# av-savchenko/fast-image-recognition

Hardware: AMD Instinct MI355X
Metric: query-vectors/sec brute-force L2 top-1, 1Mx512 gallery (higher is better)
Workload: dtype f32; 1 GPU; 1000000x512 f32 gallery, batched L2 top-1 through the library's default dispatch (the metric's 1Mx512 size; configs[1]'s kernel is the exact-scan loop under `roofline`, --full); query_batch=131072

## Files before the change

### fast-image-recognition_amd/csrc/fir_gemm.hip

```cpp
#include <hip/hip_runtime.h>
#include <stdint.h>

#include <algorithm>
#include <cstdio>
#include <cstdlib>
#include <cstring>
#include <string>
#include <vector>

#include "../../include/fir_amd.h"
#include "fir_internal.h"
#include "fir_common.h"

namespace {

using fir::kKeyNone;

#ifndef FIR_I8_AUTO_MIN_QUERIES
#define FIR_I8_AUTO_MIN_QUERIES 2048
#endif
#ifndef FIR_GEMM_BLOCK
#define FIR_GEMM_BLOCK 512
#endif
constexpr int kGemmBlock = FIR_GEMM_BLOCK;
constexpr int kGemmMinBlocks = kGemmBlock <= 512 ? 2 : 1;
constexpr int kQT = 64;
constexpr int kSlab8 = 64;
constexpr int kSlab16 = 32;
constexpr int kPasses = 128;
constexpr int kCand = 8;
constexpr int kRerankGroup = 8;
constexpr size_t kRerankLdsMax = 144 * 1024;
constexpr int kListCap = 4096;
constexpr int kClassSampleRows = 16384;
constexpr int kMinSampleRows = 8192;

typedef float f32x16 __attribute__((ext_vector_type(16)));


__global__ void __launch_bounds__(256) k_gemm_pack_gallery(const float4* __restrict__ gal4, int64_t n, int dp4, int dq8,
                                                            float4* __restrict__ gm, float* __restrict__ gnorm) {
    const int64_t o = (int64_t)blockIdx.x * 256 + threadIdx.x;
    const int64_t rblocks = (n + 31) / 32;
    if (o >= rblocks * dq8 * 64) return;
    const int l = (int)(o & 63);
    const int64_t t = o >> 6;
    const int kq = (int)(t % dq8);
    const int64_t rb = t / dq8;
    const int64_t row = rb * 32 + (l & 31);
    const int h = l >> 5;
    float v[4] = {0.f, 0.f, 0.f, 0.f};
    if (row < n) {
        const int64_t tile = row >> 6;
        const int r = (int)(row & 63);
#pragma unroll
        for (int i = 0; i < 4; ++i) {
            const int k = 8 * kq + 2 * i + h;
            if (k < dp4 * 4) {
                const float4 g = gal4[(tile * dp4 + (k >> 2)) * 64 + r];
                v[i] = (k & 3) == 0 ? g.x : (k & 3) == 1 ? g.y : (k & 3) == 2 ? g.z : g.w;
            }
        }
    }
    gm[o] = make_float4(v[0], v[1], v[2], v[3]);
    if (kq == 0 && h == 0 && row < n) {
        const int64_t tile = row >> 6;
        const int r = (int)(row & 63);
        float s = 0.f;
        for (int c = 0; c < dp4; ++c) {
            const float4 g = gal4[(tile * dp4 + c) * 64 + r];
            s += g.x * g.x + g.y * g.y + g.z * g.z + g.w * g.w;
        }
        gnorm[row] = s;
    }
}

__global__ void __launch_bounds__(256) k_gemm_pack_queries(const float* q, int nq, int d, int dq8, float4* qm) {
    q += (size_t)blockIdx.y * kQT * d;
    nq -= (int)blockIdx.y * kQT;
    qm += (size_t)blockIdx.y * (kQT / 32) * dq8 * 64;
    const int o = blockIdx.x * 256 + threadIdx.x;
    if (o < (kQT / 32) * dq8 * 64) {
        const int l = o & 63;
        const int t = o >> 6;
        const int kq = t % dq8, jb = t / dq8;
        const int qi = jb * 32 + (l & 31), h = l >> 5;
        float v[4] = {0.f, 0.f, 0.f, 0.f};
        if (qi < nq) {
#pragma unroll
            for (int i = 0; i < 4; ++i) {
                const int k = 8 * kq + 2 * i + h;
                if (k < d) v[i] = q[(size_t)qi * d + k];
            }
        }
        qm[o] = make_float4(v[0], v[1], v[2], v[3]);
    }
}

__global__ void __launch_bounds__(64) k_gemm_qnorm(const float* __restrict__ q, int nq, int d, float* __restrict__ qnorm) {
    const int qi = blockIdx.x;
    float s = 0.f;
    if (qi < nq)
        for (int k = threadIdx.x; k < d; k += 64) s += q[(size_t)qi * d + k] * q[(size_t)qi * d + k];
#pragma unroll
    for (int off = 32; off >= 1; off >>= 1) s += __shfl_xor(s, off, 64);
    if (threadIdx.x == 0) qnorm[qi] = s;
}

template <int MODE>
__global__ void __launch_bounds__(kGemmBlock, kGemmMinBlocks) k_gemm_proxy(const float4* __restrict__ gm, const float* __restrict__ gnorm,
                                                               const float4* qm, int64_t n, int64_t row_begin,
                                                               int64_t row_end, int dq8, const float* tau, unsigned long long* lists, int* counts, float* sample,
                                                               int sample_rows) {
    extern __shared__ __attribute__((aligned(16))) float4 lq[];
    __shared__ float tau_s[kQT];
    {
        const size_t ps = blockIdx.y;
        qm += ps * (kQT / 32) * dq8 * 64;
        tau += ps * kQT;
        lists += ps * kQT * kListCap;
        counts += ps * kQT;
        sample += ps * kQT * sample_rows;
    }
    const int lane = threadIdx.x & 63, wave = threadIdx.x >> 6;
    const int wpb = blockDim.x >> 6;
    const int sq8 = dq8 < kSlab8 ? dq8 : kSlab8;
    const int nslab = (dq8 + sq8 - 1) / sq8;
    if (MODE == 1 && threadIdx.x < kQT) tau_s[threadIdx.x] = tau[threadIdx.x];
    const int64_t rb_begin = row_begin / 32, rb_end = (row_end + 31) / 32;
    const int64_t nrg = (rb_end - rb_begin + wpb - 1) / wpb;
    bool staged = false;
    for (int64_t rg = blockIdx.x; rg < nrg; rg += gridDim.x) {
        const int64_t rb = rb_begin + rg * wpb + wave;
        const bool active = rb < rb_end;
        f32x16 acc0 = {0.f}, acc1 = {0.f};
        for (int sl = 0; sl < nslab; ++sl) {
            const int k0 = sl * sq8;
            const int kw = dq8 - k0 < sq8 ? dq8 - k0 : sq8;
            if (nslab > 1 || !staged) {
                __syncthreads();
                for (int i = threadIdx.x; i < 2 * kw * 64; i += blockDim.x) {
                    const int jb = i / (kw * 64), r = i - jb * kw * 64;
                    lq[(size_t)jb * sq8 * 64 + r] = qm[((size_t)jb * dq8 + k0) * 64 + r];
                }
                __syncthreads();
                staged = true;
            }
            if (!active) continue;
            const float4* a = gm + ((size_t)rb * dq8 + k0) * 64 + lane;
            const int last = kw - 1;
            float4 a0 = a[0], a1 = a[(size_t)(1 < last ? 1 : last) * 64], a2 = a[(size_t)(2 < last ? 2 : last) * 64],
                   a3 = a[(size_t)(3 < last ? 3 : last) * 64], a4 = a[(size_t)(4 < last ? 4 : last) * 64],
                   a5 = a[(size_t)(5 < last ? 5 : last) * 64], a6 = a[(size_t)(6 < last ? 6 : last) * 64],
                   a7 = a[(size_t)(7 < last ? 7 : last) * 64];
            float4 b0 = lq[lane], b1 = lq[(size_t)sq8 * 64 + lane];
#define FIR_GEMM_STEP(AV, KQ)                                                              \
            {                                                                              \
                const int kn = (KQ) + 1 < kw ? (KQ) + 1 : (KQ);                            \
                const float4 n0 = lq[(size_t)kn * 64 + lane];                              \
                const float4 n1 = lq[(size_t)(sq8 + kn) * 64 + lane];                      \
                __builtin_amdgcn_sched_barrier(0);     \
                acc0 = __builtin_amdgcn_mfma_f32_32x32x2f32(AV.x, b0.x, acc0, 0, 0, 0);    \
                acc1 = __builtin_amdgcn_mfma_f32_32x32x2f32(AV.x, b1.x, acc1, 0, 0, 0);    \
                acc0 = __builtin_amdgcn_mfma_f32_32x32x2f32(AV.y, b0.y, acc0, 0, 0, 0);    \
                acc1 = __builtin_amdgcn_mfma_f32_32x32x2f32(AV.y, b1.y, acc1, 0, 0, 0);    \
                acc0 = __builtin_amdgcn_mfma_f32_32x32x2f32(AV.z, b0.z, acc0, 0, 0, 0);    \
                acc1 = __builtin_amdgcn_mfma_f32_32x32x2f32(AV.z, b1.z, acc1, 0, 0, 0);    \
                acc0 = __builtin_amdgcn_mfma_f32_32x32x2f32(AV.w, b0.w, acc0, 0, 0, 0);    \
                acc1 = __builtin_amdgcn_mfma_f32_32x32x2f32(AV.w, b1.w, acc1, 0, 0, 0);    \
                b0 = n0;                                                                   \
                b1 = n1;                                                                   \
            }
            for (int kq = 0; kq < kw; kq += 8) {
#define FIR_GEMM_NEXT(AV, OFF) AV = a[(size_t)(kq + (OFF) + 8 < kw ? kq + (OFF) + 8 : last) * 64];
                FIR_GEMM_STEP(a0, kq)
                FIR_GEMM_NEXT(a0, 0)
                FIR_GEMM_STEP(a1, kq + 1)
                FIR_GEMM_NEXT(a1, 1)
                FIR_GEMM_STEP(a2, kq + 2)
                FIR_GEMM_NEXT(a2, 2)
                FIR_GEMM_STEP(a3, kq + 3)
                FIR_GEMM_NEXT(a3, 3)
                if (kq + 4 < kw) {
                    FIR_GEMM_STEP(a4, kq + 4)
                    FIR_GEMM_NEXT(a4, 4)
                    FIR_GEMM_STEP(a5, kq + 5)
                    FIR_GEMM_NEXT(a5, 5)
                    FIR_GEMM_STEP(a6, kq + 6)
                    FIR_GEMM_NEXT(a6, 6)
                    FIR_GEMM_STEP(a7, kq + 7)
                    FIR_GEMM_NEXT(a7, 7)
                }
#undef FIR_GEMM_NEXT
            }
#undef FIR_GEMM_STEP
        }
        if (!active) continue;
        const int64_t nrow = rb * 32 + (lane & 31);
        const float gn_lane = nrow < n ? gnorm[nrow] : 0.0f;
#pragma unroll
        for (int jb = 0; jb < 2; ++jb) {
            const int q = jb * 32 + (lane & 31);
#pragma unroll
            for (int reg = 0; reg < 16; ++reg) {
                const int roff = (reg & 3) + 8 * (reg >> 2) + 4 * (lane >> 5);
                const int64_t row = rb * 32 + roff;
                const float gn = __shfl(gn_lane, roff, 64);
                if (row >= n || row < row_begin || row >= row_end) continue;
                const float dot = jb == 0 ? acc0[reg] : acc1[reg];
                const float p = gn - 2.0f * dot;
                if (MODE == 0) {
                    if (row < sample_rows) sample[(size_t)q * sample_rows + row] = p;
                } else if (p < tau_s[q]) {
                    const int slot = atomicAdd(&counts[q], 1);
                    if (slot < kListCap) lists[(size_t)q * kListCap + slot] = fir::key_pack(p, (uint32_t)row);
                }
            }
        }
    }
}

typedef __bf16 bf16x8 __attribute__((ext_vector_type(8)));

__device__ __forceinline__ void split_bf16(float x, unsigned short& hi, unsigned short& lo) {
    const __bf16 h = (__bf16)x;
    const __bf16 l = (__bf16)(x - (float)h);
    __builtin_memcpy(&hi, &h, 2);
    __builtin_memcpy(&lo, &l, 2);
}

__global__ void __launch_bounds__(256) k_gemm_pack_gallery_bf16(const float4* __restrict__ gal4, int64_t n, int dp4, int dk16,
                                                                 uint4* __restrict__ gb) {
    const int64_t o = (int64_t)blockIdx.x * 256 + threadIdx.x;
    const int64_t rblocks = (n + 31) / 32;
    if (o >= rblocks * dk16 * 64) return;
    const int l = (int)(o & 63);
    const int64_t t = o >> 6;
    const int kb = (int)(t % dk16);
    const int64_t rb = t / dk16;
    const int64_t row = rb * 32 + (l & 31);
    const int h = l >> 5;
    unsigned short hi[8], lo[8];
#pragma unroll
    for (int j = 0; j < 8; ++j) {
        const int k = 16 * kb + 8 * h + j;
        float x = 0.f;
        if (row < n && k < dp4 * 4) {
            const float4 g = gal4[((row >> 6) * dp4 + (k >> 2)) * 64 + (row & 63)];
            x = (k & 3) == 0 ? g.x : (k & 3) == 1 ? g.y : (k & 3) == 2 ? g.z : g.w;
        }
        split_bf16(x, hi[j], lo[j]);
    }
    uint4 vh, vl;
    __builtin_memcpy(&vh, hi, 16);
    __builtin_memcpy(&vl, lo, 16);
    gb[(size_t)(t * 2) * 64 + l] = vh;
    gb[(size_t)(t * 2 + 1) * 64 + l] = vl;
}

__global__ void __launch_bounds__(256) k_gemm_pack_queries_bf16(const float* q, int nq, int d, int dk16, uint4* qbf) {
    q += (size_t)blockIdx.y * kQT * d;
    nq -= (int)blockIdx.y * kQT;
    qbf += (size_t)blockIdx.y * (kQT / 32) * dk16 * 128;
    const int o = blockIdx.x * 256 + threadIdx.x;
    if (o >= (kQT / 32) * dk16 * 64) return;
    const int l = o & 63;
    const int t = o >> 6;
    const int kb = t % dk16, jb = t / dk16;
    const int qi = jb * 32 + (l & 31), h = l >> 5;
    unsigned short hi[8], lo[8];
#pragma unroll
    for (int j = 0; j < 8; ++j) {
        const int k = 16 * kb + 8 * h + j;
        const float x = (qi < nq && k < d) ? q[(size_t)qi * d + k] : 0.f;
        split_bf16(x, hi[j], lo[j]);
    }
    uint4 vh, vl;
    __builtin_memcpy(&vh, hi, 16);
    __builtin_memcpy(&vl, lo, 16);
    qbf[(size_t)(t * 2) * 64 + l] = vh;
    qbf[(size_t)(t * 2 + 1) * 64 + l] = vl;
}

__device__ __forceinline__ uint4 ld_nt(const uint4* p) {
    typedef unsigned v4u __attribute__((ext_vector_type(4)));
    const v4u v = __builtin_nontemporal_load((const v4u*)p);
    return make_uint4(v.x, v.y, v.z, v.w);
}
__device__ __forceinline__ bf16x8 as_bf16x8(const uint4 v) {
    bf16x8 r;
    __builtin_memcpy(&r, &v, 16);
    return r;
}

template <int MODE>
__global__ void __launch_bounds__(kGemmBlock, kGemmMinBlocks) k_gemm_proxy_bf16(const uint4* __restrict__ gb, const float* __restrict__ gnorm,
                                                                    const uint4* qbf, int64_t n, int64_t row_begin,
                                                                    int64_t row_end, int dk16, const float* tau, unsigned long long* lists, int* counts, float* sample,
                                                                    int sample_rows) {
    extern __shared__ __attribute__((aligned(16))) uint4 lqb[];
    __shared__ float tau_s[kQT];
    {
        const size_t ps = blockIdx.y;
        qbf += ps * (kQT / 32) * dk16 * 128;
        tau += ps * kQT;
        lists += ps * kQT * kListCap;
        counts += ps * kQT;
        sample += ps * kQT * sample_rows;
    }
    const int lane = threadIdx.x & 63, wave = threadIdx.x >> 6;
    const int wpb = blockDim.x >> 6;
    const int sk16 = MODE == 0 ? dk16 : (dk16 < kSlab16 ? dk16 : kSlab16);
    const int nslab = (dk16 + sk16 - 1) / sk16;
    const uint4* bsrc = MODE == 0 ? qbf : lqb;
    if (MODE == 1 && threadIdx.x < kQT) tau_s[threadIdx.x] = tau[threadIdx.x];
    const int64_t rb_begin = row_begin / 32, rb_end = (row_end + 31) / 32;
    const int64_t nrg = (rb_end - rb_begin + wpb - 1) / wpb;
    bool staged = MODE == 0;
    for (int64_t rg = blockIdx.x; rg < nrg; rg += gridDim.x) {
        const int64_t rb = rb_begin + rg * wpb + wave;
        const bool active = rb < rb_end;
        f32x16 acc0 = {0.f}, acc1 = {0.f};
        for (int sl = 0; sl < nslab; ++sl) {
            const int k0 = sl * sk16;
            const int kw = dk16 - k0 < sk16 ? dk16 - k0 : sk16;
            if (MODE == 1 && (nslab > 1 || !staged)) {
                __syncthreads();
                for (int i = threadIdx.x; i < 2 * kw * 128; i += blockDim.x) {
                    const int jb = i / (kw * 128), r = i - jb * kw * 128;
                    lqb[(size_t)jb * sk16 * 128 + r] = qbf[((size_t)jb * dk16 + k0) * 128 + r];
                }
                __syncthreads();
                staged = true;
            }
            if (!active) continue;
            const uint4* a = gb + ((size_t)rb * dk16 + k0) * 128 + lane;
            const int last = kw - 1;
#define FIR_BF_LD(IDX) ld_nt(a + (size_t)((IDX) < last ? (IDX) : last) * 128)
#define FIR_BF_LDL(IDX) ld_nt(a + (size_t)((IDX) < last ? (IDX) : last) * 128 + 64)
            uint4 h0 = FIR_BF_LD(0), l0 = FIR_BF_LDL(0), h1 = FIR_BF_LD(1), l1 = FIR_BF_LDL(1), h2 = FIR_BF_LD(2), l2 = FIR_BF_LDL(2),
                  h3 = FIR_BF_LD(3), l3 = FIR_BF_LDL(3), h4 = FIR_BF_LD(4), l4 = FIR_BF_LDL(4), h5 = FIR_BF_LD(5), l5 = FIR_BF_LDL(5),
                  h6 = FIR_BF_LD(6), l6 = FIR_BF_LDL(6), h7 = FIR_BF_LD(7), l7 = FIR_BF_LDL(7);
            const uint4* bq0 = bsrc + (size_t)(MODE == 0 ? k0 : 0) * 128 + lane;
            const uint4* bq1 = bq0 + (size_t)sk16 * 128;
            uint4 b0h = bq0[0], b0l = bq0[64], b1h = bq1[0], b1l = bq1[64];
#define FIR_BF_STEP(AH, AL, KB)                                                                                  \
            {                                                                                                    \
                const int kn = (KB) + 1 < kw ? (KB) + 1 : (KB);                                                  \
                const uint4 n0h = bq0[(size_t)kn * 128], n0l = bq0[(size_t)kn * 128 + 64];                       \
                const uint4 n1h = bq1[(size_t)kn * 128], n1l = bq1[(size_t)kn * 128 + 64];                       \
                __builtin_amdgcn_sched_barrier(0);                                                               \
                const bf16x8 ah = as_bf16x8(AH), al = as_bf16x8(AL);                                             \
                acc0 = __builtin_amdgcn_mfma_f32_32x32x16_bf16(ah, as_bf16x8(b0h), acc0, 0, 0, 0);               \
                acc1 = __builtin_amdgcn_mfma_f32_32x32x16_bf16(ah, as_bf16x8(b1h), acc1, 0, 0, 0);               \
                acc0 = __builtin_amdgcn_mfma_f32_32x32x16_bf16(ah, as_bf16x8(b0l), acc0, 0, 0, 0);               \
                acc1 = __builtin_amdgcn_mfma_f32_32x32x16_bf16(ah, as_bf16x8(b1l), acc1, 0, 0, 0);               \
                acc0 = __builtin_amdgcn_mfma_f32_32x32x16_bf16(al, as_bf16x8(b0h), acc0, 0, 0, 0);               \
                acc1 = __builtin_amdgcn_mfma_f32_32x32x16_bf16(al, as_bf16x8(b1h), acc1, 0, 0, 0);               \
                b0h = n0h; b0l = n0l; b1h = n1h; b1l = n1l;                                                      \
            }
#define FIR_BF_NEXT(AH, AL, OFF)                \
            {                                   \
                AH = FIR_BF_LD(kb + (OFF) + 8); \
                AL = FIR_BF_LDL(kb + (OFF) + 8);\
            }
            for (int kb = 0; kb < kw; kb += 8) {
                FIR_BF_STEP(h0, l0, kb)
                FIR_BF_NEXT(h0, l0, 0)
                FIR_BF_STEP(h1, l1, kb + 1)
                FIR_BF_NEXT(h1, l1, 1)
                FIR_BF_STEP(h2, l2, kb + 2)
                FIR_BF_NEXT(h2, l2, 2)
                FIR_BF_STEP(h3, l3, kb + 3)
                FIR_BF_NEXT(h3, l3, 3)
                if (kb + 4 < kw) {
                    FIR_BF_STEP(h4, l4, kb + 4)
                    FIR_BF_NEXT(h4, l4, 4)
                    FIR_BF_STEP(h5, l5, kb + 5)
                    FIR_BF_NEXT(h5, l5, 5)
                    FIR_BF_STEP(h6, l6, kb + 6)
                    FIR_BF_NEXT(h6, l6, 6)
                    FIR_BF_STEP(h7, l7, kb + 7)
                    FIR_BF_NEXT(h7, l7, 7)
                }
            }
#undef FIR_BF_NEXT
#undef FIR_BF_STEP
#undef FIR_BF_LD
#undef FIR_BF_LDL
        }
        if (!active) continue;
        const int64_t nrow = rb * 32 + (lane & 31);
        const float gn_lane = nrow < n ? gnorm[nrow] : 0.0f;
#pragma unroll
        for (int jb = 0; jb < 2; ++jb) {
            const int q = jb * 32 + (lane & 31);
#pragma unroll
            for (int reg = 0; reg < 16; ++reg) {
                const int roff = (reg & 3) + 8 * (reg >> 2) + 4 * (lane >> 5);
                const int64_t row = rb * 32 + roff;
                const float gn = __shfl(gn_lane, roff, 64);
                if (row >= n || row < row_begin || row >= row_end) continue;
                const float dot = jb == 0 ? acc0[reg] : acc1[reg];
                const float p = gn - 2.0f * dot;
                if (MODE == 0) {
                    if (row < sample_rows) sample[(size_t)q * sample_rows + row] = p;
                } else if (p < tau_s[q]) {
                    const int slot = atomicAdd(&counts[q], 1);
                    if (slot < kListCap) lists[(size_t)q * kListCap + slot] = fir::key_pack(p, (uint32_t)row);
                }
            }
        }
    }
}

constexpr int kSlabW = 16;
constexpr int kUnitW = kSlabW / 2;
constexpr int kWideLds = 4 * kSlabW * 128 * (int)sizeof(uint4);
__global__ void __launch_bounds__(kGemmBlock, 1) k_gemm_proxy_bf16_wide(const uint4* __restrict__ gb, const float* __restrict__ gnorm,
                                                                         const uint4* qbf, int64_t n, int dk16, const float* tau,
                                                                         unsigned long long* lists, int* counts) {
    extern __shared__ __attribute__((aligned(16))) uint4 lqb[];
    __shared__ float tau_s[2 * kQT];
    {
        const size_t pr = blockIdx.y;
        qbf += pr * 4 * dk16 * 128;
        tau += pr * 2 * kQT;
        lists += pr * 2 * kQT * kListCap;
        counts += pr * 2 * kQT;
    }
    const int lane = threadIdx.x & 63, wave = threadIdx.x >> 6;
    const int wpb = blockDim.x >> 6;
    if (threadIdx.x < 2 * kQT) tau_s[threadIdx.x] = tau[threadIdx.x];
    const int64_t rb_end = (n + 31) / 32;
    const int64_t nrg = (rb_end + wpb - 1) / wpb;
    const int units = dk16 / kUnitW;
    int64_t rg = blockIdx.x;
    if (rg >= nrg) return;
#define FIR_W_BLOCK(RG) (gb + (size_t)(((RG) * wpb + wave) < rb_end ? ((RG) * wpb + wave) : rb_end - 1) * dk16 * 128 + lane)
    const uint4* a_cur = FIR_W_BLOCK(rg);
    uint4 ch[kUnitW], cl[kUnitW], nh[kUnitW], nl[kUnitW];
#pragma unroll
    for (int u = 0; u < kUnitW; ++u) {
        ch[u] = ld_nt(a_cur + (size_t)u * 128);
        cl[u] = ld_nt(a_cur + (size_t)u * 128 + 64);
    }
    for (; rg < nrg; rg += gridDim.x) {
        const int64_t rb = rg * wpb + wave;
        const bool active = rb < rb_end;
        const int64_t rgn = rg + gridDim.x;
        const uint4* a_nxt = FIR_W_BLOCK(rgn < nrg ? rgn : rg);
        f32x16 acc0 = {0.f}, acc1 = {0.f}, acc2 = {0.f}, acc3 = {0.f};
        for (int h = 0; h < units; ++h) {
            const uint4* src = h + 1 < units ? a_cur + (size_t)(h + 1) * kUnitW * 128 : a_nxt;
#pragma unroll
            for (int u = 0; u < kUnitW; ++u) {
                nh[u] = ld_nt(src + (size_t)u * 128);
                nl[u] = ld_nt(src + (size_t)u * 128 + 64);
            }
            if ((h & 1) == 0) {
                const int k0 = h * kUnitW;
                const int kw = dk16 - k0 < kSlabW ? dk16 - k0 : kSlabW;
                __syncthreads();
                for (int i = threadIdx.x; i < 4 * kw * 128; i += blockDim.x) {
                    const int jb = i / (kw * 128), r = i - jb * kw * 128;
                    lqb[(size_t)jb * kSlabW * 128 + r] = qbf[((size_t)jb * dk16 + k0) * 128 + r];
                }
                __syncthreads();
            }
            const uint4* bq = lqb + lane + (size_t)(h & 1) * kUnitW * 128;
#pragma unroll
            for (int u = 0; u < kUnitW; ++u) {
                const uint4* bu = bq + (size_t)u * 128;
                const bf16x8 ah = as_bf16x8(ch[u]), al = as_bf16x8(cl[u]);
#pragma unroll
                for (int jb = 0; jb < 4; ++jb) {
                    const bf16x8 bh = as_bf16x8(bu[(size_t)jb * kSlabW * 128]), bl = as_bf16x8(bu[(size_t)jb * kSlabW * 128 + 64]);
                    f32x16& acc = jb == 0 ? acc0 : jb == 1 ? acc1 : jb == 2 ? acc2 : acc3;
                    acc = __builtin_amdgcn_mfma_f32_32x32x16_bf16(ah, bh, acc, 0, 0, 0);
                    acc = __builtin_amdgcn_mfma_f32_32x32x16_bf16(ah, bl, acc, 0, 0, 0);
                    acc = __builtin_amdgcn_mfma_f32_32x32x16_bf16(al, bh, acc, 0, 0, 0);
                }
            }
#pragma unroll
            for (int u = 0; u < kUnitW; ++u) { ch[u] = nh[u]; cl[u] = nl[u]; }
        }
        a_cur = a_nxt;
        if (!active) continue;
        const int64_t nrow = rb * 32 + (lane & 31);
        const float gn_lane = nrow < n ? gnorm[nrow] : 0.0f;
#pragma unroll
        for (int jb = 0; jb < 4; ++jb) {
            const int q = jb * 32 + (lane & 31);
#pragma unroll
            for (int reg = 0; reg < 16; ++reg) {
                const int roff = (reg & 3) + 8 * (reg >> 2) + 4 * (lane >> 5);
                const int64_t row = rb * 32 + roff;
                const float gn = __shfl(gn_lane, roff, 64);
                if (row >= n) continue;
                const float dot = jb == 0 ? acc0[reg] : jb == 1 ? acc1[reg] : jb == 2 ? acc2[reg] : acc3[reg];
                const float p = gn - 2.0f * dot;
                if (p < tau_s[q]) {
                    const int slot = atomicAdd(&counts[q], 1);
                    if (slot < kListCap) lists[(size_t)q * kListCap + slot] = fir::key_pack(p, (uint32_t)row);
                }
            }
        }
    }
#undef FIR_W_BLOCK
}

typedef _Float16 f16x8 __attribute__((ext_vector_type(8)));
__device__ __forceinline__ f16x8 as_f16x8(const uint4 v) {
    f16x8 r;
    __builtin_memcpy(&r, &v, 16);
    return r;
}
constexpr int kSlabH = 32;
constexpr int kHalfLds = 4 * kSlabH * 64 * (int)sizeof(uint4);
constexpr int kRing = 8;

#include "fir_gemm_rerank.h"

__global__ void __launch_bounds__(256) k_gemm_absmax(const float4* __restrict__ gal4, int64_t count4, float* __restrict__ out) {
    float m = 0.f;
    for (int64_t i = (int64_t)blockIdx.x * 256 + threadIdx.x; i < count4; i += (int64_t)gridDim.x * 256) {
        const float4 g = gal4[i];
        const float a = fmaxf(fmaxf(fabsf(g.x), fabsf(g.y)), fmaxf(fabsf(g.z), fabsf(g.w)));
        const bool bad = !(g.x == g.x && g.y == g.y && g.z == g.z && g.w == g.w);
        m = fmaxf(m, bad ? __builtin_huge_valf() : a);
    }
#pragma unroll
    for (int off = 32; off >= 1; off >>= 1) m = fmaxf(m, __shfl_xor(m, off, 64));
    if ((threadIdx.x & 63) == 0) atomicMax((unsigned int*)out, __float_as_uint(m));
}

__global__ void __launch_bounds__(64) k_gemm_qprep_f16(const float* __restrict__ q, int nq, int d, int gallery_exp, float* __restrict__ qnorm,
                                                        float* __restrict__ qmul, float* __restrict__ qinv, int qstride, int* __restrict__ counts = nullptr,
                                                        float* __restrict__ win = nullptr, unsigned int* __restrict__ t_bits = nullptr,
                                                        const float* __restrict__ gnorm_max_p = nullptr, float e_rel = 0.f, int nslot = 0,
                                                        unsigned int* __restrict__ smin_init = nullptr, int* __restrict__ fb_state = nullptr) {
    const int qi = blockIdx.x;
    if (threadIdx.x == 0) {
        if (smin_init) smin_init[qi] = 0xFF800000u;
        if (fb_state && qi == 0) { fb_state[0] = 0; fb_state[1] = 0; }
    }
    float s = 0.f, m = 0.f;
    bool bad = false;
    if (qi < nq)
        for (int k = threadIdx.x; k < d; k += 64) {
            const float x = q[(size_t)qi * qstride + k];
            s += x * x;
            m = fmaxf(m, fabsf(x));
            bad = bad || !(fabsf(x) < __builtin_huge_valf());
        }
#pragma unroll
    for (int off = 32; off >= 1; off >>= 1) {
        s += __shfl_xor(s, off, 64);
        m = fmaxf(m, __shfl_xor(m, off, 64));
    }
    bad = __any(bad);
    if (threadIdx.x == 0) {
        int ex = 0;
        if (m > 0.f) (void)frexpf(m, &ex);
        int sh = m > 0.f ? 14 - ex : 0;
        if (sh < -100 || sh > 100 || gallery_exp < -100 || gallery_exp > 100) bad = true;
        const float qn = (bad && qi < nq) ? __builtin_nanf("") : s;
        qnorm[qi] = qn;
        qmul[qi] = bad ? 0.f : ldexpf(1.0f, sh);
        qinv[qi] = qi >= nq ? 0.f : bad ? __builtin_nanf("") : ldexpf(1.0f, -sh - gallery_exp);
        if (counts) counts[qi] = 0;
        if (win) {
            const unsigned int start = qi >= nq ? 0u : 0x7F800000u;
            if (qi >= nq) win[qi] = 0.f;
            else {
                win[qi] = nudge_up_(rounding_window_(e_rel, qn, gnorm_max_p[0]));
            }
            if (nslot > 0) { for (int sl = 0; sl < 8; ++sl) atomicExch(&t_bits[(size_t)qi * 8 + sl], start); }
            else atomicExch(&t_bits[qi], start);
        }
    }
}

#include "fir_gemm_f16x.h"

__global__ void __launch_bounds__(256) k_gemm_tau(const float* __restrict__ sample, int sample_rows, float* __restrict__ tau,
                                                   int nq_valid, const float* __restrict__ qnorm, const float* __restrict__ gnorm_max_p, float e_rel,
                                                   int kth_window = 0) {
    __shared__ unsigned long long red[4];
    const int q = blockIdx.x;
    if (q >= nq_valid) {
        if (threadIdx.x == 0) tau[q] = -__builtin_huge_valf();
        return;
    }
    const float* s = sample + (size_t)q * sample_rows;
    unsigned long long best[kCand];
#pragma unroll
    for (int i = 0; i < kCand; ++i) best[i] = kKeyNone;
    for (int i = threadIdx.x; i < sample_rows; i += 256) {
        unsigned long long v = fir::key_pack(s[i], (uint32_t)i);
        if (v < best[kCand - 1]) {
#pragma unroll
            for (int j = 0; j < kCand; ++j) {
                const bool sw = v < best[j];
                const unsigned long long t = best[j];
                best[j] = sw ? v : t;
                v = sw ? t : v;
            }
        }
    }
    unsigned long long m = kKeyNone, smallest = kKeyNone;
    for (int r = 0; r < kCand; ++r) {
        unsigned long long c = fir::wave_min_u64(best[0]);
        __syncthreads();
        if ((threadIdx.x & 63) == 0) red[threadIdx.x >> 6] = c;
        __syncthreads();
        m = red[0];
        for (int i = 1; i < 4; ++i) m = red[i] < m ? red[i] : m;
        if (r == 0) smallest = m;
        if (m == kKeyNone) break;
        if (best[0] == m) {
#pragma unroll
            for (int j = 0; j + 1 < kCand; ++j) best[j] = best[j + 1];
            best[kCand - 1] = kKeyNone;
        }
    }
    if (threadIdx.x == 0) {
        float t = __builtin_huge_valf();
        if (m != kKeyNone) {
            float v = fir::f32_from_orderable((uint32_t)(m >> 32));
            const float v1 = fir::f32_from_orderable((uint32_t)(smallest >> 32));
            const float window = rounding_window_(e_rel, qnorm[q], gnorm_max_p[0]);
            v = kth_window ? v + window : fmaxf(v, v1 + window);
            t = nudge_up_(v);
        }
        tau[q] = t;
    }
}

#include "fir_gemm_fb.h"
#include "fir_gemm_i8.h"

template <int KMAX>
__global__ void __launch_bounds__(64) k_gemm_rerank(const unsigned long long* __restrict__ lists, const int* __restrict__ counts,
                                                     const float* __restrict__ tau, const float4* __restrict__ gal4,
                                                     const float* __restrict__ queries, const float* __restrict__ qnorm,
                                                     const float* __restrict__ gnorm_max_p, int64_t n, int d, int dp4, int64_t row_offset,
                                                     float e_rel, int ngroup, int k_arg, unsigned long long* __restrict__ out_key,
                                                     int* __restrict__ ok, int qstride, const float4* __restrict__ rowmajor, const RerankFb fb,
                                                     const float* __restrict__ eabs = nullptr) {
    const int k = KMAX == 1 ? 1 : k_arg;
    const int q = blockIdx.x, lane = threadIdx.x;
    int qo = q;
    if (fb.qmap) {
        if (q >= fb.state[0] - fb.live_off) return;
        qo = fb.qmap[q];
    }
    const int cnt = counts[q];
    const int have = cnt < kListCap ? cnt : kListCap;
    const unsigned long long* L = lists + (size_t)q * kListCap;
    int found;
    const unsigned long long kth = list_kth_smallest_(L, have, k, lane, found);
    const float qn = qnorm[q], gmax = gnorm_max_p[0];
    const float pk = found == k ? fir::f32_from_orderable((uint32_t)(kth >> 32)) : __builtin_huge_valf();
    const RerankWindow w = eabs ? rerank_window_(e_rel, qn, gmax, d, pk, eabs[q]) : rerank_window_(e_rel, qn, gmax, d, pk);
    extern __shared__ __attribute__((aligned(16))) float4 crow[];
    const RerankLds lds = rerank_lds_f32_(crow, ngroup, dp4, d, queries + (size_t)qo * qstride, lane);
    unsigned long long best[KMAX];
#pragma unroll
    for (int i = 0; i < KMAX; ++i) best[i] = kKeyNone;
    const RerankWalk walk = rerank_walk_(L, have, w.win, lane, [&](int base, unsigned long long v, bool, unsigned long long mask) {
        rerank_gather_f32_(mask, v, base, lane, ngroup, lds, gal4, rowmajor, dp4, d, [&](int, unsigned long long cv, float dist) {
            if (dist < fir::kNotFound) {
                const int64_t row = (int64_t)(uint32_t)(cv & 0xFFFFFFFFull);
                unsigned long long key = fir::key_pack(dist, (uint32_t)(row + row_offset));
#pragma unroll
                for (int j = 0; j < KMAX; ++j) {
                    const bool sw = key < best[j];
                    const unsigned long long t = best[j];
                    best[j] = sw ? key : t;
                    key = sw ? t : key;
                }
            }
        });
    });
    unsigned long long kth_exact = kKeyNone;
    for (int r = 0; r < k; ++r) {
        const unsigned long long m = fir::wave_min_u64(best[0]);
        if (lane == 0) out_key[(size_t)qo * k + r] = m;
        kth_exact = m;
        if (m != kKeyNone && best[0] == m) {
#pragma unroll
            for (int j = 0; j + 1 < KMAX; ++j) best[j] = best[j + 1];
            best[KMAX - 1] = kKeyNone;
        }
    }
    if (lane == 0) {
        const float t = tau[q];
        const bool certified = rerank_certified_<float>(cnt, t, walk.p_out, qn, d, w.E, kth_exact != kKeyNone,
                                                        fir::f32_from_orderable((uint32_t)(kth_exact >> 32)), n, walk.reranked);
        ok[qo] = certified ? 1 : 0;
        if (!certified && fb.list && !fb.qmap) rerank_hand_over_(fb, q, cnt, t, pk, qn, gmax, e_rel, eabs);
    }
}

__global__ void __launch_bounds__(256) k_gemm_select(const float* __restrict__ proxies, int64_t n, const float* __restrict__ tau,
                                                      unsigned long long* __restrict__ lists, int* __restrict__ counts) {
    const int q = blockIdx.y;
    const float tq = tau[q];
    const float* p = proxies + (size_t)q * n;
    for (int64_t row = (int64_t)blockIdx.x * 256 + threadIdx.x; row < n; row += (int64_t)gridDim.x * 256) {
        const float v = p[row];
        if (v < tq) {
            const int slot = atomicAdd(&counts[q], 1);
            if (slot < kListCap) lists[(size_t)q * kListCap + slot] = fir::key_pack(v, (uint32_t)row);
        }
    }
}

__global__ void __launch_bounds__(256) k_gemm_tau_class(float* __restrict__ tau, int nq_total, int nq_valid, int d, const float* __restrict__ qnorm,
                                                         const float* __restrict__ gnorm_max_p, float e_rel) {
    const int q = blockIdx.x * 256 + threadIdx.x;
    if (q >= nq_total) return;
    if (q >= nq_valid) { tau[q] = -__builtin_huge_valf(); return; }
    const float ds = tau[q];
    float t = __builtin_huge_valf();
    if (ds < fir::kNotFound) {
        const float v = (ds * (float)d - qnorm[q]) + rounding_window_(e_rel, qnorm[q], gnorm_max_p[0]);
        t = nudge_up_(v);
    }
    tau[q] = t;
}

__global__ void __launch_bounds__(64) k_gemm_rerank_classes(unsigned long long* lists, const int* __restrict__ counts, const float* __restrict__ tau,
                                                             const float4* __restrict__ gal4, const float* __restrict__ queries,
                                                             const float* __restrict__ qnorm, const float* __restrict__ gnorm_max_p,
                                                             const int32_t* __restrict__ cls, int num_classes, int64_t n, int d, int dp4,
                                                             int64_t row_offset, float e_rel, int ngroup, int k, unsigned long long* __restrict__ out_key,
                                                             int32_t* __restrict__ out_cls, int* __restrict__ ok, int qstride,
                                                             const float4* __restrict__ rowmajor) {
    __shared__ int32_t taken[32];
    const int q = blockIdx.x, lane = threadIdx.x;
    const int cnt = counts[q];
    if (cnt > kListCap) {
        if (lane == 0) ok[q] = 0;
        return;
    }
    const int have = cnt;
    unsigned long long* L = lists + (size_t)q * kListCap;
    auto pick = [&](int r, unsigned long long prev, int64_t roff, int32_t& c_out) -> unsigned long long {
        unsigned long long cand = kKeyNone;
        int32_t cc = -1;
        for (int i = lane; i < have; i += 64) {
            const unsigned long long v = L[i];
            if (v >= cand || (r > 0 && v <= prev)) continue;
            const int32_t c = cls[(int64_t)(uint32_t)(v & 0xFFFFFFFFull) - roff];
            bool skip = (uint32_t)c >= (uint32_t)num_classes;
            for (int j = 0; j < r; ++j) skip = skip || taken[j] == c;
            if (!skip) { cand = v; cc = c; }
        }
        const unsigned long long m = fir::wave_min_u64(cand);
        const unsigned long long who = __ballot(m != kKeyNone && cand == m);
        c_out = who ? __shfl(cc, __ffsll((long long)who) - 1, 64) : -1;
        return m;
    };
    unsigned long long prev = 0;
    int found = 0;
    for (int r = 0; r < k; ++r) {
        int32_t c;
        const unsigned long long m = pick(r, prev, 0, c);
        if (m == kKeyNone) break;
        if (lane == 0) taken[r] = c;
        __syncthreads();
        prev = m;
        ++found;
    }
    const float qn = qnorm[q], gmax = gnorm_max_p[0];
    const float pk = found == k ? fir::f32_from_orderable((uint32_t)(prev >> 32)) : __builtin_huge_valf();
    const RerankWindow w = rerank_window_(e_rel, qn, gmax, d, pk);
    extern __shared__ __attribute__((aligned(16))) float4 crow[];
    const RerankLds lds = rerank_lds_f32_(crow, ngroup, dp4, d, queries + (size_t)q * qstride, lane);
    const RerankWalk walk = rerank_walk_(L, have, w.win, lane, [&](int base, unsigned long long v, bool in, unsigned long long mask) {
        if (base + lane < have && !in) L[base + lane] = kKeyNone;
        rerank_gather_f32_(mask, v, base, lane, ngroup, lds, gal4, rowmajor, dp4, d, [&](int i, unsigned long long cv, float dist) {
            const int64_t row = (int64_t)(uint32_t)(cv & 0xFFFFFFFFull);
            const bool counted = (uint32_t)cls[row] < (uint32_t)num_classes && dist < fir::kNotFound;
            L[i] = counted ? fir::key_pack(dist, (uint32_t)(row + row_offset)) : kKeyNone;
        });
    });
    __threadfence_block();
    __syncthreads();
    unsigned long long kth_exact = kKeyNone;
    prev = 0;
    int r = 0;
    for (; r < k; ++r) {
        int32_t c;
        const unsigned long long m = pick(r, prev, row_offset, c);
        if (m == kKeyNone) break;
        if (lane == 0) {
            taken[r] = c;
            if (out_key) out_key[(size_t)q * k + r] = m;
            if (out_cls) out_cls[(size_t)q * k + r] = c;
        }
        __syncthreads();
        prev = m;
        if (r == k - 1) kth_exact = m;
    }
    for (int i = r + lane; i < k; i += 64) {
        if (out_key) out_key[(size_t)q * k + i] = kKeyNone;
        if (out_cls) out_cls[(size_t)q * k + i] = -1;
    }
    if (lane == 0)
        ok[q] = rerank_certified_<float>(cnt, tau[q], walk.p_out, qn, d, w.E, kth_exact != kKeyNone, fir::f32_from_orderable((uint32_t)(kth_exact >> 32)), n,
                                         walk.reranked) ? 1 : 0;
}

__global__ void k_gemm_fb_count(int* __restrict__ state, int count) {
    unsigned long long* tot = (unsigned long long*)(state + 4);
    tot[0] += (unsigned long long)count;
    tot[1] += (unsigned long long)count;
}

__global__ void __launch_bounds__(256) k_gemm_untile(const float4* __restrict__ gal4, int64_t n, int dp4, int d4, float4* __restrict__ rowmajor) {
    __shared__ float4 t[32][65];
    const int64_t tile = blockIdx.x;
    const int c0 = blockIdx.y * 32;
    for (int i = threadIdx.x; i < 32 * 64; i += 256) {
        const int c = i >> 6, r = i & 63;
        if (c0 + c < d4) t[c][r] = gal4[((size_t)tile * dp4 + c0 + c) * 64 + r];
    }
    __syncthreads();
    for (int i = threadIdx.x; i < 64 * 32; i += 256) {
        const int r = i >> 5, c = i & 31;
        const int64_t row = tile * 64 + r;
        if (row < n && c0 + c < d4) rowmajor[(size_t)row * d4 + c0 + c] = t[c][r];
    }
}

__global__ void __launch_bounds__(256) k_gemm_row_norms(const float4* __restrict__ gal4, int64_t n, int dp4, float* __restrict__ gnorm, int d4) {
    const int64_t row = (int64_t)blockIdx.x * 256 + threadIdx.x;
    if (row >= n) return;
    float s = 0.f;
    for (int c = 0; c < d4; ++c) {
        const float4 g = gal4[((row >> 6) * dp4 + c) * 64 + (row & 63)];
        s += g.x * g.x + g.y * g.y + g.z * g.z + g.w * g.w;
    }
    gnorm[row] = s;
}

__global__ void k_gemm_max(const float* __restrict__ gnorm, int64_t n, float* __restrict__ out) {
    __shared__ float red[4];
    float m = 0.f;
    for (int64_t i = threadIdx.x; i < n; i += 256) m = fmaxf(m, gnorm[i]);
#pragma unroll
    for (int off = 32; off >= 1; off >>= 1) m = fmaxf(m, __shfl_xor(m, off, 64));
    if ((threadIdx.x & 63) == 0) red[threadIdx.x >> 6] = m;
    __syncthreads();
    if (threadIdx.x == 0) out[0] = fmaxf(fmaxf(red[0], red[1]), fmaxf(red[2], red[3]));
}

__global__ void __launch_bounds__(256) k_gemm_adapt_init(float* __restrict__ win, unsigned int* __restrict__ t_bits, int nq_total, int nq_valid,
                                                          const float* __restrict__ qnorm, const float* __restrict__ gnorm_max_p, float e_rel) {
    const int q = blockIdx.x * 256 + threadIdx.x;
    if (q >= nq_total) return;
    if (q >= nq_valid) { win[q] = 0.f; t_bits[q] = 0u; return; }
    win[q] = nudge_up_(rounding_window_(e_rel, qnorm[q], gnorm_max_p[0]));
    t_bits[q] = 0x7F800000u;
}
__global__ void __launch_bounds__(256) k_gemm_adapt_final(unsigned int* __restrict__ t_bits, const float* __restrict__ qnorm, float* __restrict__ tau,
                                                           int nq_total, int nq_valid, int nslot = 0) {
    const int q = blockIdx.x * 256 + threadIdx.x;
    if (q >= nq_total) return;
    unsigned int t;
    if (nslot > 0) {
        unsigned int v[8];
        for (int sl = 0; sl < 8; ++sl) v[sl] = atomicMin(&t_bits[(size_t)q * 8 + sl], 0xFFFFFFFFu);
        t = 0xFFFFFFFFu;
        for (int i = 0; i < 8; ++i) {
            int rank = 0;
            for (int j = 0; j < 8; ++j) rank += (v[j] < v[i] || (v[j] == v[i] && j < i)) ? 1 : 0;
            if (rank == nslot - 1) t = v[i];
        }
    } else t = atomicMin(&t_bits[q], 0xFFFFFFFFu);
    tau[q] = q < nq_valid ? __uint_as_float(t) - qnorm[q] : -__builtin_huge_valf();
}

}

struct fir_gemm {
    fir_gallery* g = nullptr;
    fir_gallery_view v;
    const float4* gal4 = nullptr;
    int dp4 = 0, dq8 = 0;
    int feat = 0;
    int precision = 0;
    uint4* gh = nullptr;
    float* proxies = nullptr;
    int proxies_nq = 0;
    int lists_cap = 0;
    float4* rowmajor = nullptr;
    int gallery_exp = 0;
    float* qmul[2] = {nullptr, nullptr};
    float* qinv[2] = {nullptr, nullptr};
    int dk16 = 0;
    float4* gm = nullptr;
    uint4* gb = nullptr;
    uint4* qbf[2] = {nullptr, nullptr};
    float* gnorm = nullptr;
    float* gmax = nullptr;
    float4* qm[2] = {nullptr, nullptr};
    float* qnorm[2] = {nullptr, nullptr};
    float* tau[2] = {nullptr, nullptr};
    float* sample = nullptr;
    unsigned long long* lists[2] = {nullptr, nullptr};
    int* counts[2] = {nullptr, nullptr};
    hipStream_t side = nullptr;
    hipEvent_t main_done[2] = {nullptr, nullptr}, rerank_done[2] = {nullptr, nullptr}, prep_done[2] = {nullptr, nullptr};
    hipEvent_t queries_ready = nullptr;
    hipStream_t copy = nullptr;
    hipEvent_t copy_done[2] = {nullptr, nullptr};
    int* ok = nullptr; size_t ok_cap = 0;
    int sample_rows = 0;
    int* fb_state = nullptr;
    int* fb_list = nullptr;
    int* fb_list2 = nullptr;
    float* fb_tau2 = nullptr;
    float* sc_qnorm = nullptr; float* sc_qmul = nullptr; float* sc_qinv = nullptr; float* sc_tau = nullptr;
    int* sc_counts = nullptr;
    unsigned long long* sc_lists = nullptr;
    uint4* sc_qbf = nullptr;
    size_t fb_lds = 0;
    int fb_grid = 0;
    int64_t passes = 0;
    int rerank_group = kRerankGroup;
    bool wide = true;
    unsigned int* smin[2] = {nullptr, nullptr};
    int rt_sample_rows = 0;
    bool f64 = false;
    const double2* gal2 = nullptr; int dp2 = 0;
    int adaptive = 1;
    int class_sample_div = 64;
    int adaptive_topk = 1;
    float* awin[2] = {nullptr, nullptr};
    unsigned int* aT[2] = {nullptr, nullptr};
    float erel_scale = 1.0f;
    int dbg_block = kGemmBlock;
    int dbg_skip = 0;
    int adapt_dbg = 0;
    bool debug_counts = false;
    hipEvent_t phase_ev[4] = {nullptr, nullptr, nullptr, nullptr};
    std::string dump_phases;
    int last_kind = 0;
    int last_b = 0, last_nq = 0;
    int last_sc_rounds = 0;
    bool last_i8 = false;
    int i8_mode = 0;
    bool i8_built = false, i8_off = false;
    const char* i8_off_why = "";
    std::string i8_note;
    int dk8 = 0;
    uint4* g8 = nullptr;
    float* i8_mu = nullptr;
    float* i8_gnorm = nullptr;
    float* i8_par = nullptr;
    float* i8_eabs[2] = {nullptr, nullptr};
    float* sc_eabs = nullptr;
    float i8_R = 0.f, i8_G = 0.f;
    int* i8_pin = nullptr;
    hipEvent_t i8_ev = nullptr;
    bool i8_pending = false;
    int i8_pending_qb = 0;
};

static void gemm_read_knobs_(fir_gemm* m) {
    if (const char* w = fir_knob_("FIR_GEMM_ADAPTIVE")) m->adaptive = std::atoi(w);
    if (const char* w = fir_knob_("FIR_GEMM_ADAPTIVE_TOPK")) m->adaptive_topk = std::atoi(w) != 0;
    if (const char* w = fir_knob_("FIR_GEMM_CLASS_SAMPLE_DIV")) m->class_sample_div = std::max(1, std::atoi(w));
#ifdef FIR_AUDIT
    if (const char* w = fir_knob_("FIR_GEMM_DBG_SKIP")) m->dbg_skip = std::atoi(w) & 1023;
    if (const char* w = fir_knob_("FIR_GEMM_DBG_BLOCK")) m->dbg_block = std::atoi(w) == 256 ? 256 : kGemmBlock;
    if (const char* w = fir_knob_("FIR_GEMM_EREL_SCALE")) m->erel_scale = (float)std::atof(w);
    if (const char* w = fir_knob_("FIR_GEMM_ADAPT_DBG")) m->adapt_dbg = (std::atoi(w) & 3) << 2;
    if (fir_knob_("FIR_GEMM_DEBUG_COUNTS")) m->debug_counts = true;
    if (const char* w = fir_knob_("FIR_GEMM_DUMP_PHASES")) m->dump_phases = w;
#endif
}

struct RerankSlot {
    const unsigned long long* lists;
    const int* counts;
    const float* tau;
    const float* qnorm;
    const float* eabs = nullptr;
    const float* gmax = nullptr;
};
static size_t gemm_rerank_lds_(const fir_gemm* m) { return (size_t)(m->rerank_group + 1) * (m->dp4 + 1) * sizeof(float4); }
static void gemm_launch_rerank_(fir_gemm* m, hipStream_t st, int nq, const RerankSlot& s, const float* d_queries, float e_rel, int k, uint64_t* out_key, int* ok,
                                const RerankFb& fb) {
    hipLaunchKernelGGL(k == 1 ? k_gemm_rerank<1> : k_gemm_rerank<kTopKMax>, dim3(nq), dim3(64), gemm_rerank_lds_(m), st, s.lists, s.counts, s.tau, m->gal4, d_queries,
                       s.qnorm, s.gmax ? s.gmax : (const float*)m->gmax, m->v.n, m->feat, m->dp4, m->v.row_offset, e_rel, m->rerank_group, k, (unsigned long long*)out_key,
                       ok, m->v.d, (const float4*)m->rowmajor, fb, s.eabs);
}

constexpr int kShareMax = 16, kShareStreamed = 8;
static bool gemm_streamed_(const fir_gemm* m) { return m->dk16 > kSlabH; }
static int gemm_odd_(const fir_gemm* m) { return m->dk16 == kRing ? 2 : (m->dk16 / kRing) & 1; }
static int gemm_odd8_(const fir_gemm* m) { return m->dk8 == kRing ? 2 : (m->dk8 / kRing) & 1; }
static int launch_pairs_(int left, int cap) {
    int P = 1;
    while (P * 2 <= left && P * 2 <= cap) P *= 2;
    return P;
}

typedef void (*fir_x_fn)(const uint4*, const float*, const uint4*, const float*, int64_t, int64_t, int64_t, int, const float*, unsigned long long*, int*, float*,
                         int, int, int, int, unsigned int*, int);
struct fir_x_entry {
    int mode, streamed, odd, njb;
    fir_x_fn fn;
    const char* name;
};
#define FIR_X(M, S, O) {M, S, O, 8, k_gemm_proxy_f16x<M, S, O>, "fir::k_gemm_proxy_f16x<" #M ", " #S ", " #O ">"}
#define FIR_X_FEW(S, J) {3, S, 0, J, k_gemm_proxy_f16x<3, S, 0, 0, J>, "fir::k_gemm_proxy_f16x<3, " #S ", 0, 0, " #J ">"}
static const fir_x_entry kXTable[] = {
    FIR_X(1, 0, 0), FIR_X(1, 0, 1), FIR_X(1, 1, 0), FIR_X(1, 1, 1), FIR_X(2, 0, 0), FIR_X(2, 0, 1), FIR_X(2, 1, 0), FIR_X(2, 1, 1),
    FIR_X(3, 0, 0), FIR_X(3, 0, 1), FIR_X(3, 1, 0), FIR_X(3, 1, 1), FIR_X(4, 0, 0), FIR_X(4, 0, 1), FIR_X(4, 1, 0), FIR_X(4, 1, 1),
    FIR_X_FEW(0, 1), FIR_X_FEW(1, 1), FIR_X_FEW(0, 2), FIR_X_FEW(1, 2),
    FIR_X(1, 0, 2), FIR_X(2, 0, 2), FIR_X(3, 0, 2), FIR_X(4, 0, 2),
};
#undef FIR_X
#undef FIR_X_FEW
static const fir_x_entry* lookup_x(int mode, bool streamed, int odd, int njb) {
    for (const fir_x_entry& e : kXTable)
        if (e.mode == mode && e.streamed == (int)streamed && e.odd == odd && e.njb == njb) return &e;
    return nullptr;
}
static const fir_x_entry& find_x(int mode, bool streamed, int odd, int njb = 8) {
    if (!(mode == 3 && !odd && (njb == 1 || njb == 2))) njb = 8;
    if (const fir_x_entry* e = lookup_x(mode, streamed, odd, njb)) return *e;
    if (const fir_x_entry* e = lookup_x(2, streamed, odd, 8)) return *e;
    return *lookup_x(2, false, 0, 8);
}
static fir_x_fn pick_x(int mode, bool streamed, int odd, int dbg = 0, int njb = 8) {
#ifdef FIR_AUDIT
    if (dbg && mode == 3 && !streamed && !odd) {
        switch (dbg & 1023) {
            case 1: return k_gemm_proxy_f16x<3, 0, 0, 1>;
            case 2: return k_gemm_proxy_f16x<3, 0, 0, 2>;
            case 3: return k_gemm_proxy_f16x<3, 0, 0, 3>;
            case 5: return k_gemm_proxy_f16x<3, 0, 0, 5>;
            case 7: return k_gemm_proxy_f16x<3, 0, 0, 7>;
            case 512: return k_gemm_proxy_f16x<3, 0, 0, 512>;
            case 256: return k_gemm_proxy_f16x<3, 0, 0, 256>;
            case 128: return k_gemm_proxy_f16x<3, 0, 0, 128>;
            case 384: return k_gemm_proxy_f16x<3, 0, 0, 384>;
            case 64: return k_gemm_proxy_f16x<3, 0, 0, 64>;
            case 33: return k_gemm_proxy_f16x<3, 0, 0, 33>;
            case 37: return k_gemm_proxy_f16x<3, 0, 0, 37>;
            case 35: return k_gemm_proxy_f16x<3, 0, 0, 35>;
            case 16: return k_gemm_proxy_f16x<3, 0, 0, 16>;
            case 8: return k_gemm_proxy_f16x<3, 0, 0, 8>;
            default: break;
        }
    }
#endif
    return find_x(mode, streamed, odd, dbg ? 8 : njb).fn;
}
struct fir_x8_entry {
    int mode, odd;
    fir_x_fn fn;
    const char* name;
};
#define FIR_X8(M, O) {M, O, k_gemm_proxy_f16x<M, 0, O, 0, 8, 1>, "fir::k_gemm_proxy_i8x<" #M ", " #O ">"}
static const fir_x8_entry kX8Table[] = {FIR_X8(3, 0), FIR_X8(3, 1), FIR_X8(3, 2), FIR_X8(1, 0), FIR_X8(1, 1), FIR_X8(1, 2)};
#undef FIR_X8
static const fir_x8_entry& find_x8(int mode, int odd) {
    for (const fir_x8_entry& e : kX8Table)
        if (e.mode == mode && e.odd == odd) return e;
    return kX8Table[0];
}
static hipError_t gemm_x_lds_attr_() {
    for (const fir_x_entry& e : kXTable) {
        const hipError_t err = hipFuncSetAttribute((const void*)e.fn, hipFuncAttributeMaxDynamicSharedMemorySize, kHalfLds);
        if (err != hipSuccess) return err;
    }
    for (const fir_x8_entry& e : kX8Table) {
        const hipError_t err = hipFuncSetAttribute((const void*)e.fn, hipFuncAttributeMaxDynamicSharedMemorySize, kHalfLds);
        if (err != hipSuccess) return err;
    }
    return hipSuccess;
}

static void gemm_free_i8_(fir_gemm* m) {
    (void)hipFree(m->g8); (void)hipFree(m->i8_mu); (void)hipFree(m->i8_gnorm); (void)hipFree(m->i8_par); (void)hipFree(m->i8_eabs[0]); (void)hipFree(m->i8_eabs[1]);
    (void)hipFree(m->sc_eabs);
    if (m->i8_pin) (void)hipHostFree(m->i8_pin);
    if (m->i8_ev) (void)hipEventDestroy(m->i8_ev);
    m->g8 = nullptr; m->i8_mu = m->i8_gnorm = m->i8_par = m->i8_eabs[0] = m->i8_eabs[1] = m->sc_eabs = nullptr;
    m->i8_pin = nullptr; m->i8_ev = nullptr;
    m->i8_built = false;
}

extern "C" {

int fir_gemm_create(fir_gallery* g, fir_gemm** out) { return fir_gemm_create_range(g, FIR_GEMM_F16, 0, out); }

int fir_gemm_create_ex(fir_gallery* g, int32_t precision, fir_gemm** out) { return fir_gemm_create_range(g, precision, 0, out); }

int fir_gemm_create_range(fir_gallery* g, int32_t precision, int32_t end_pos, fir_gemm** out) { return fir_gemm_create_range_ex_(g, precision, end_pos, -1, out); }

void fir_gemm_memory_bytes_(const fir_gemm* m, int64_t* fragments, int64_t* rowmajor, int64_t* scratch) {
    const int64_t rblocks = (std::max<int64_t>(m->v.n, 1) + 31) / 32, np = std::max<int64_t>(m->v.n, 1);
    const int64_t fr = m->gh ? rblocks * m->dk16 * 1024 : m->gb ? rblocks * m->dk16 * 2048 : m->gm ? rblocks * m->dq8 * 1024 : 0;
    const int64_t rm = m->rowmajor ? m->v.n * (int64_t)((m->feat + 3) / 4) * 16 : 0;
    int64_t sc = np * 4 + 16;
    sc += 2 * ((int64_t)m->lists_cap * kListCap * 8 + (int64_t)m->lists_cap * 4);
    sc += 2 * (m->precision == FIR_GEMM_F32 ? (int64_t)kPasses * (kQT / 32) * m->dq8 * 1024
                                            : (int64_t)kPasses * (kQT / 32) * m->dk16 * (m->precision == FIR_GEMM_BF16_SPLIT ? 2048 : 1024));
    sc += 2 * (int64_t)kPasses * kQT * 4 * 4 + 2 * (int64_t)kRtSubsets * kPasses * kQT * 4;
    sc += (int64_t)m->ok_cap * 16 + 32;
    if (m->sc_lists) sc += (int64_t)kScQueries * kListCap * 8 + (int64_t)4 * m->dk16 * 1024 + (int64_t)kScQueries * 20;
    if (m->proxies) sc += (int64_t)m->proxies_nq * np * 4;
    int64_t fr8 = 0;
    if (m->g8) {
        fr8 = rblocks * m->dk8 * 1024;
        sc += np * 4 + (int64_t)((m->feat + 3) / 4) * 16 + 32 + 2 * (int64_t)kPasses * kQT * 4 + (int64_t)kScQueries * 4;
    }
    if (fragments) *fragments = fr + fr8;
    if (rowmajor) *rowmajor = rm;
    if (scratch) *scratch = sc;
}

int fir_gemm_create_range_ex_(fir_gallery* g, int32_t precision, int32_t end_pos, int32_t rowmajor_mode, fir_gemm** out) {
    if (!g || !out) return fir_fail_(FIR_ERR_ARG, "NULL argument");
    if (precision != FIR_GEMM_F32 && precision != FIR_GEMM_BF16_SPLIT && precision != FIR_GEMM_F16)
        return fir_fail_(FIR_ERR_ARG, "bad precision %d", precision);
    *out = nullptr;
    fir_gemm* m = new (std::nothrow) fir_gemm();
    if (!m) return fir_fail_(FIR_ERR_NOMEM, "host allocation failed");
    m->g = g;
    const void* gp = nullptr;
    if (fir_gallery_view_(g, &m->v) != FIR_OK || fir_gallery_tiled_(g, &gp, &m->dp4) != FIR_OK) { delete m; return fir_fail_(FIR_ERR_ARG, "bad gallery"); }
    m->gal4 = (const float4*)gp;
    m->precision = precision;
    if (precision == FIR_GEMM_F16 && !(m->v.cus >= 8 && (m->v.cus & 7) == 0)) {
        const int cus = m->v.cus;
        delete m;
        return fir_fail_(FIR_ERR_ARG, "the 16-row kernels want CUs in eights (%d)", cus);
    }
    m->feat = end_pos > 0 && end_pos < m->v.d ? end_pos : m->v.d;
    if (end_pos < 0 || end_pos > m->v.d || (m->feat != m->v.d && (m->feat % 16 != 0 || precision != FIR_GEMM_F16))) {
        const int dd = m->v.d;
        delete m;
        return fir_fail_(FIR_ERR_ARG, "feature prefix [0,%d) of %d: multiples of 16 inside the row, fp16 form only", end_pos, dd);
    }
    if (const char* w = fir_knob_("FIR_GEMM_WIDE")) m->wide = std::atoi(w) != 0;
    m->dq8 = (m->feat + 31) / 32 * 4;
    m->dk16 = (m->feat + 127) / 128 * 8;
    if (precision == FIR_GEMM_F16) m->dk16 = (m->feat + 16 * kRing - 1) / (16 * kRing) * kRing;
    hipError_t e = hipSetDevice(m->v.device);
    const int64_t rblocks = (std::max<int64_t>(m->v.n, 1) + 31) / 32;
    const int64_t np = std::max<int64_t>(m->v.n, 1);
    if (e == hipSuccess && precision == FIR_GEMM_F32) e = hipMalloc((void**)&m->gm, (size_t)rblocks * m->dq8 * 64 * sizeof(float4));
    if (e == hipSuccess && precision == FIR_GEMM_BF16_SPLIT) e = hipMalloc((void**)&m->gb, (size_t)rblocks * m->dk16 * 128 * sizeof(uint4));
    if (e == hipSuccess && precision == FIR_GEMM_F16) e = hipMalloc((void**)&m->gh, (size_t)rblocks * m->dk16 * 64 * sizeof(uint4));
    if (e == hipSuccess) e = hipMalloc((void**)&m->gnorm, (size_t)np * sizeof(float));
    if (e == hipSuccess) e = hipMalloc((void**)&m->gmax, 16);
    for (int b = 0; b < 2; ++b) {
        if (e == hipSuccess && precision == FIR_GEMM_F32) e = hipMalloc((void**)&m->qm[b], (size_t)kPasses * (kQT / 32) * m->dq8 * 64 * sizeof(float4));
        if (e == hipSuccess && precision != FIR_GEMM_F32)
            e = hipMalloc((void**)&m->qbf[b], (size_t)kPasses * (kQT / 32) * m->dk16 * (precision == FIR_GEMM_BF16_SPLIT ? 128 : 64) * sizeof(uint4));
        if (e == hipSuccess) e = hipMalloc((void**)&m->qnorm[b], kPasses * kQT * sizeof(float));
        if (e == hipSuccess) e = hipMalloc((void**)&m->qmul[b], kPasses * kQT * sizeof(float));
        if (e == hipSuccess) e = hipMalloc((void**)&m->qinv[b], kPasses * kQT * sizeof(float));
        if (e == hipSuccess) e = hipMalloc((void**)&m->smin[b], (size_t)kRtSubsets * kPasses * kQT * sizeof(unsigned int));
        if (e == hipSuccess) e = hipMalloc((void**)&m->tau[b], kPasses * kQT * sizeof(float));
        if (e == hipSuccess) e = hipMalloc((void**)&m->awin[b], kPasses * kQT * sizeof(float));
        if (e == hipSuccess) e = hipMalloc((void**)&m->aT[b], (size_t)8 * kPasses * kQT * sizeof(unsigned int));
        if (e == hipSuccess) e = hipEventCreateWithFlags(&m->main_done[b], hipEventDisableTiming);
        if (e == hipSuccess) e = hipEventCreateWithFlags(&m->rerank_done[b], hipEventDisableTiming);
        if (e == hipSuccess) e = hipEventCreateWithFlags(&m->prep_done[b], hipEventDisableTiming);
    }
    if (e == hipSuccess) e = hipEventCreateWithFlags(&m->queries_ready, hipEventDisableTiming);
    if (e == hipSuccess) e = hipStreamCreateWithFlags(&m->side, hipStreamNonBlocking);
    if (e == hipSuccess) e = hipStreamCreateWithFlags(&m->copy, hipStreamNonBlocking);
    for (int b = 0; b < 2 && e == hipSuccess; ++b) e = hipEventCreateWithFlags(&m->copy_done[b], hipEventDisableTiming);
    m->sample_rows = (int)std::min<int64_t>(np, std::max<int64_t>(kMinSampleRows, np / 64));
    m->rt_sample_rows = (int)std::min<int64_t>(np, std::max<int64_t>(kMinSampleRows, np / 32));
    if (const char* w = fir_knob_("FIR_GEMM_SAMPLE_DIV"))
        m->rt_sample_rows = (int)std::min<int64_t>(np, std::max<int64_t>(kMinSampleRows, np / std::max(1, std::atoi(w))));
    if (e == hipSuccess) e = hipMalloc((void**)&m->fb_state, kFbStateWords * sizeof(int));
    if (e == hipSuccess) e = hipMemset(m->fb_state, 0, kFbStateWords * sizeof(int));
    if (e == hipSuccess) e = hipMalloc((void**)&m->sc_qnorm, kScQueries * sizeof(float));
    if (e == hipSuccess) e = hipMalloc((void**)&m->sc_qmul, kScQueries * sizeof(float));
    if (e == hipSuccess) e = hipMalloc((void**)&m->sc_qinv, kScQueries * sizeof(float));
    if (e == hipSuccess) e = hipMalloc((void**)&m->sc_tau, kScQueries * sizeof(float));
    if (e == hipSuccess) e = hipMalloc((void**)&m->sc_counts, kScQueries * sizeof(int));
    if (e == hipSuccess && precision == FIR_GEMM_F16) e = hipMalloc((void**)&m->sc_lists, (size_t)kScQueries * kListCap * sizeof(unsigned long long));
    if (e == hipSuccess && precision == FIR_GEMM_F16) e = hipMalloc((void**)&m->sc_qbf, (size_t)4 * m->dk16 * 64 * sizeof(uint4));
    {
        m->fb_lds = (size_t)m->dp4 * 4 * 8 * sizeof(float);
        if (m->fb_lds > kRerankLdsMax) {
            const int dd = m->v.d;
            fir_gemm_destroy(m);
            return fir_fail_(FIR_ERR_ARG, "rows of %d features are too long for the matrix-core path's exact fallback", dd);
        }
        if (e == hipSuccess && m->fb_lds > 48 * 1024)
            e = hipFuncSetAttribute((const void*)k_gemm_exact_fb, hipFuncAttributeMaxDynamicSharedMemorySize, (int)kRerankLdsMax);
        const int per_cu = (int)std::max<size_t>(1, std::min<size_t>(4, (size_t)(160 * 1024) / std::max<size_t>(m->fb_lds, 1)));
        m->fb_grid = std::max(1, m->v.cus) * per_cu;
    }
    const int lds_bytes = precision == FIR_GEMM_F32 ? (kQT / 32) * std::min(m->dq8, kSlab8) * 64 * (int)sizeof(float4)
                                                    : (kQT / 32) * std::min(m->dk16, kSlab16) * 128 * (int)sizeof(uint4);
    if (e == hipSuccess) e = hipFuncSetAttribute((const void*)k_gemm_proxy<0>, hipFuncAttributeMaxDynamicSharedMemorySize, lds_bytes);
    if (e == hipSuccess) e = hipFuncSetAttribute((const void*)k_gemm_proxy<1>, hipFuncAttributeMaxDynamicSharedMemorySize, lds_bytes);
    if (e == hipSuccess) e = hipFuncSetAttribute((const void*)k_gemm_proxy_bf16<0>, hipFuncAttributeMaxDynamicSharedMemorySize, lds_bytes);
    if (e == hipSuccess) e = hipFuncSetAttribute((const void*)k_gemm_proxy_bf16<1>, hipFuncAttributeMaxDynamicSharedMemorySize, lds_bytes);
    if (e == hipSuccess) e = hipFuncSetAttribute((const void*)k_gemm_proxy_bf16_wide, hipFuncAttributeMaxDynamicSharedMemorySize, kWideLds);
    {
        const size_t row_bytes = (size_t)(m->dp4 + 1) * sizeof(float4);
        m->rerank_group = (int)std::min<size_t>(kRerankGroup, kRerankLdsMax / row_bytes > 1 ? kRerankLdsMax / row_bytes - 1 : 0);
        if (m->rerank_group < 1) { delete m; return fir_fail_(FIR_ERR_ARG, "rows of %d features are too long for the matrix-core path's re-rank", m->v.d); }
        if (gemm_rerank_lds_(m) > 48 * 1024)
            for (const void* fn : {(const void*)k_gemm_rerank<1>, (const void*)k_gemm_rerank<kTopKMax>, (const void*)k_gemm_rerank_classes})
                if (e == hipSuccess) e = hipFuncSetAttribute(fn, hipFuncAttributeMaxDynamicSharedMemorySize, (int)kRerankLdsMax);
    }
    if (e == hipSuccess && precision == FIR_GEMM_F16) e = gemm_x_lds_attr_();
    gemm_read_knobs_(m);
    if (e == hipSuccess && m->v.n > 0) {
        if (precision == FIR_GEMM_BF16_SPLIT) {
            const int64_t totalb = rblocks * m->dk16 * 64;
            hipLaunchKernelGGL(k_gemm_pack_gallery_bf16, dim3((unsigned)((totalb + 255) / 256)), dim3(256), 0, m->v.stream, m->gal4, m->v.n, m->dp4,
                               m->dk16, m->gb);
            hipLaunchKernelGGL(k_gemm_row_norms, dim3((unsigned)((m->v.n + 255) / 256)), dim3(256), 0, m->v.stream, m->gal4, m->v.n, m->dp4, m->gnorm, (m->feat + 3) / 4);
        }
        if (precision == FIR_GEMM_F16) {
            float h_max = 0.f;
            e = hipMemsetAsync(m->gmax, 0, 16, m->v.stream);
            const int64_t count4 = (int64_t)((m->v.n + 63) / 64) * m->dp4 * 64;
            hipLaunchKernelGGL(k_gemm_absmax, dim3((unsigned)std::min<int64_t>((count4 + 255) / 256, 4096)), dim3(256), 0, m->v.stream, m->gal4, count4, m->gmax);
            if (e == hipSuccess) e = hipMemcpyAsync(&h_max, m->gmax, sizeof(float), hipMemcpyDeviceToHost, m->v.stream);
            if (e == hipSuccess) e = hipStreamSynchronize(m->v.stream);
            int ex = 0;
            if (h_max > 0.f && h_max < __builtin_huge_valf()) { (void)std::frexp(h_max, &ex); m->gallery_exp = 14 - ex; }
            else m->gallery_exp = h_max > 0.f ? 1000 : 0;
            const float scale = (m->gallery_exp >= -100 && m->gallery_exp <= 100) ? std::ldexp(1.0f, m->gallery_exp) : 0.f;
            const int64_t totalh = rblocks * m->dk16 * 64;
            hipLaunchKernelGGL(k_gemm_pack_gallery_f16x, dim3((unsigned)((totalh + 255) / 256)), dim3(256), 0, m->v.stream, m->gal4, m->v.n, m->dp4,
                               m->dk16, scale, m->gh, m->feat == m->v.d ? m->dp4 * 4 : m->feat);
            hipLaunchKernelGGL(k_gemm_row_norms, dim3((unsigned)((m->v.n + 255) / 256)), dim3(256), 0, m->v.stream, m->gal4, m->v.n, m->dp4, m->gnorm, (m->feat + 3) / 4);
        }
        const int64_t total = precision == FIR_GEMM_F32 ? rblocks * m->dq8 * 64 : 0;
        if (total > 0)
        hipLaunchKernelGGL(k_gemm_pack_gallery, dim3((unsigned)((total + 255) / 256)), dim3(256), 0, m->v.stream, m->gal4, m->v.n, m->dp4, m->dq8,
                           m->gm, m->gnorm);
        hipLaunchKernelGGL(k_gemm_max, dim3(1), dim3(256), 0, m->v.stream, m->gnorm, m->v.n, m->gmax);
        {
            const int d4 = (m->feat + 3) / 4;
            const size_t want = (size_t)m->v.n * d4 * sizeof(float4);
            size_t free_b = 0, total_b = 0;
            int mode = rowmajor_mode;
            if (const char* w = fir_knob_("FIR_GEMM_ROWMAJOR")) { if (mode < 0) mode = std::atoi(w); }
            const bool room = hipMemGetInfo(&free_b, &total_b) == hipSuccess && free_b >= 4 * want;
            if (mode != 0 && (room || mode > 0) && hipMalloc((void**)&m->rowmajor, want) == hipSuccess) {
                const int64_t tiles = (m->v.n + 63) / 64;
                for (int64_t t0 = 0; t0 < tiles; t0 += 65535 * 16) {
                    const int64_t nt = std::min<int64_t>(tiles - t0, 65535 * 16);
                    hipLaunchKernelGGL(k_gemm_untile, dim3((unsigned)nt, (unsigned)((d4 + 31) / 32)), dim3(256), 0, m->v.stream, m->gal4 + (size_t)t0 * m->dp4 * 64,
                                       m->v.n - t0 * 64, m->dp4, d4, m->rowmajor + (size_t)t0 * 64 * d4);
                }
            } else {
                (void)hipGetLastError();
                m->rowmajor = nullptr;
            }
        }
        e = hipGetLastError();
        if (e == hipSuccess) e = hipStreamSynchronize(m->v.stream);
    }
    if (e != hipSuccess) {
        const int rc = fir_fail_(e == hipErrorOutOfMemory ? FIR_ERR_NOMEM : FIR_ERR_HIP, "GEMM-path setup: %s", hipGetErrorString(e));
        fir_gemm_destroy(m);
        return rc;
    }
    *out = m;
    return FIR_OK;
}

int fir_gemm_destroy(fir_gemm* m) {
    if (!m) return FIR_OK;
    (void)hipSetDevice(m->v.device);
    (void)fir_gallery_wait_calls_(m->g);
    if (m->v.stream || !m->f64) (void)hipStreamSynchronize(m->v.stream);
    if (m->side) { (void)hipStreamSynchronize(m->side); (void)hipStreamDestroy(m->side); }
    for (int b = 0; b < 2; ++b) {
        (void)hipFree(m->qm[b]); (void)hipFree(m->qbf[b]); (void)hipFree(m->qnorm[b]); (void)hipFree(m->qmul[b]); (void)hipFree(m->qinv[b]); (void)hipFree(m->smin[b]); (void)hipFree(m->tau[b]); (void)hipFree(m->awin[b]); (void)hipFree(m->aT[b]); (void)hipFree(m->lists[b]); (void)hipFree(m->counts[b]);
        if (m->main_done[b]) (void)hipEventDestroy(m->main_done[b]);
        if (m->rerank_done[b]) (void)hipEventDestroy(m->rerank_done[b]);
        if (m->prep_done[b]) (void)hipEventDestroy(m->prep_done[b]);
    }
    if (m->queries_ready) (void)hipEventDestroy(m->queries_ready);
    for (hipEvent_t ev : m->phase_ev) if (ev) (void)hipEventDestroy(ev);
    (void)hipFree(m->gm); (void)hipFree(m->gb); (void)hipFree(m->gh); (void)hipFree(m->rowmajor); (void)hipFree(m->proxies); (void)hipFree(m->gnorm); (void)hipFree(m->gmax); (void)hipFree(m->sample); (void)hipFree(m->ok);
    (void)hipFree(m->fb_state); (void)hipFree(m->fb_list); (void)hipFree(m->fb_list2); (void)hipFree(m->fb_tau2);
    (void)hipFree(m->sc_qnorm); (void)hipFree(m->sc_qmul); (void)hipFree(m->sc_qinv); (void)hipFree(m->sc_tau); (void)hipFree(m->sc_counts);
    (void)hipFree(m->sc_lists); (void)hipFree(m->sc_qbf);
    gemm_free_i8_(m);
        if (m->copy) { (void)hipStreamSynchronize(m->copy); (void)hipStreamDestroy(m->copy); }
    for (int b = 0; b < 2; ++b) if (m->copy_done[b]) (void)hipEventDestroy(m->copy_done[b]);
    delete m;
    return FIR_OK;
}

int fir_gemm_stats_ex(const fir_gemm* m, int64_t out[3]) {
    if (!m || !out) return fir_fail_(FIR_ERR_ARG, "NULL argument");
    FIR_HIP(hipSetDevice(m->v.device));
    FIR_HIP(hipDeviceSynchronize());
    unsigned long long tot[2] = {0, 0};
    FIR_HIP(hipMemcpy(tot, m->fb_state + 4, sizeof tot, hipMemcpyDeviceToHost));
    out[0] = m->passes;
    out[1] = (int64_t)tot[0];
    out[2] = (int64_t)tot[1];
    return FIR_OK;
}

int fir_gemm_uncertified_notes(const fir_gemm* m, float out[32], int32_t* count) {
    if (!m || !out || !count) return fir_fail_(FIR_ERR_ARG, "NULL argument");
    FIR_HIP(hipSetDevice(m->v.device));
    FIR_HIP(hipDeviceSynchronize());
    int h[kFbStateWords];
    FIR_HIP(hipMemcpy(h, m->fb_state, sizeof h, hipMemcpyDeviceToHost));
    *count = h[2] < 8 ? h[2] : 8;
    std::memcpy(out, h + 8, 32 * sizeof(float));
    return FIR_OK;
}

int fir_gemm_stats(const fir_gemm* m, int64_t* passes, int64_t* fallback_queries) {
    int64_t o[3];
    const int rc = fir_gemm_stats_ex(m, o);
    if (rc) return rc;
    if (passes) *passes = o[0];
    if (fallback_queries) *fallback_queries = o[2];
    return FIR_OK;
}

}

static int gemm_finish_(fir_gemm* m, const float* d_queries, int k, uint64_t* d_keys, hipStream_t st, float e_rel, int sc_rounds, bool streamed, bool i8 = false) {
    const int d = m->feat, qs = m->v.d;
    const int64_t n = m->v.n;
    for (int r = 0; r < sc_rounds; ++r) {
        const int off = r * kScQueries;
        if (i8) {
            hipLaunchKernelGGL(k_gemm_qprep_i8, dim3(kScQueries), dim3(64), 0, st, d_queries, kScQueries, d, qs, (const float*)m->i8_mu, (const float*)m->i8_par, e_rel,
                               m->erel_scale, m->sc_qnorm, m->sc_qmul, m->sc_qinv, m->sc_eabs, m->sc_counts, (float*)nullptr, (unsigned int*)nullptr, (int*)nullptr,
                               (const int*)m->fb_state, (const int*)m->fb_list, off, (const float*)m->fb_tau2, m->sc_tau);
            hipLaunchKernelGGL(k_gemm_pack_queries_i8, dim3((4 * m->dk8 * 64 + 255) / 256, 1), dim3(256), 0, st, d_queries, kScQueries, d, m->dk8, (const float*)m->i8_mu,
                               (const float*)m->sc_qmul, m->sc_qbf, qs, (const int*)m->fb_list + off, (const int*)m->fb_state, off);
            hipLaunchKernelGGL(find_x8(1, gemm_odd8_(m)).fn, dim3(m->v.cus, 1), dim3(kGemmBlock), kHalfLds, st, m->g8, m->i8_gnorm, m->sc_qbf, (const float*)m->sc_qinv, n,
                               (int64_t)0, n, m->dk8, (const float*)m->sc_tau, m->sc_lists, m->sc_counts, (float*)nullptr, 0, 1, 1, 1,
                               (unsigned int*)m->fb_state, off);
            gemm_launch_rerank_(m, st, kScQueries, {m->sc_lists, m->sc_counts, m->sc_tau, m->sc_qnorm, m->sc_eabs, m->i8_par + 2}, d_queries, e_rel, k, d_keys, m->ok,
                                {m->fb_state, nullptr, nullptr, 0, (const int*)m->fb_list + off, off});
            continue;
        }
        hipLaunchKernelGGL(k_gemm_sc_prep, dim3(kScQueries), dim3(64), 0, st, d_queries, d, qs, m->gallery_exp, (const int*)m->fb_state, (const int*)m->fb_list, off,
                           (const float*)m->fb_tau2, m->sc_qnorm, m->sc_qmul, m->sc_qinv, m->sc_tau, m->sc_counts);
        hipLaunchKernelGGL(k_gemm_pack_queries_f16x, dim3((4 * m->dk16 * 64 + 255) / 256, 1), dim3(256), 0, st, d_queries, kScQueries, d, m->dk16, (const float*)m->sc_qmul,
                           m->sc_qbf, qs, (const int*)m->fb_list + off, (const int*)m->fb_state, off);
        hipLaunchKernelGGL(pick_x(1, streamed, gemm_odd_(m)), dim3(m->v.cus, 1), dim3(kGemmBlock), kHalfLds, st, m->gh, m->gnorm, m->sc_qbf, (const float*)m->sc_qinv, n,
                           (int64_t)0, n, m->dk16, (const float*)m->sc_tau, m->sc_lists, m->sc_counts, (float*)nullptr, 0, 1, 1, 1,
                           (unsigned int*)m->fb_state, off);
        gemm_launch_rerank_(m, st, kScQueries, {m->sc_lists, m->sc_counts, m->sc_tau, m->sc_qnorm}, d_queries, e_rel, k, d_keys, m->ok,
                            {m->fb_state, nullptr, nullptr, 0, (const int*)m->fb_list + off, off});
    }
    hipLaunchKernelGGL(k_gemm_fb_collect, dim3(1), dim3(256), 0, st, m->fb_state, (const int*)m->fb_list, (const int*)m->ok, m->fb_list2, (unsigned long long*)d_keys, k);
    for (int r = 0; r < k; ++r)
        hipLaunchKernelGGL(k_gemm_exact_fb, dim3(m->fb_grid), dim3(256), m->fb_lds, st, m->gal4, n, m->dp4, d, m->v.row_offset, d_queries, qs, (const int*)m->fb_state,
                           (const int*)m->fb_list2, (unsigned long long*)d_keys, k, r);
    FIR_HIP(hipGetLastError());
    return FIR_OK;
}

struct GemmCall {
    const float* d_queries;
    const float* h_queries;
    int32_t qb;
    int k;
    uint64_t* d_keys;
    int32_t num_classes;
    int32_t* d_classes;
    hipStream_t st;
    int d, qs;
    int64_t n;
    float e_rel;
    int grid;
    int sbq, nsb;
    bool serial_prep;
    bool one_stream;
    bool streamed;
    int odd;
    size_t lds;
    bool i8 = false;
    bool i8_went_back = false;

    int sb_queries(int sb) const { return std::min(sbq, qb - sb * sbq); }
    const float* sb_first(int sb) const { return d_queries + (size_t)sb * sbq * qs; }
};

constexpr int kI8AutoMinQueries = FIR_I8_AUTO_MIN_QUERIES;
constexpr float kI8AutoMaxRG = 0.0125f;
static int gemm_build_i8_(fir_gemm* m, hipStream_t st) {
    const int64_t n = m->v.n, rblocks = (std::max<int64_t>(n, 1) + 31) / 32, tiles = (n + 63) / 64;
    const int d4 = (m->feat + 3) / 4;
    m->dk8 = (m->feat + 32 * kRing - 1) / (32 * kRing) * kRing;
    double* partial = nullptr;
    FIR_HIP(hipMalloc((void**)&m->g8, (size_t)rblocks * m->dk8 * 64 * sizeof(uint4)));
    FIR_HIP(hipMalloc((void**)&m->i8_mu, (size_t)d4 * 4 * sizeof(float)));
    FIR_HIP(hipMalloc((void**)&m->i8_gnorm, (size_t)std::max<int64_t>(n, 1) * sizeof(float)));
    FIR_HIP(hipMalloc((void**)&m->i8_par, 8 * sizeof(float)));
    for (int b = 0; b < 2; ++b) FIR_HIP(hipMalloc((void**)&m->i8_eabs[b], kPasses * kQT * sizeof(float)));
    FIR_HIP(hipMalloc((void**)&m->sc_eabs, kScQueries * sizeof(float)));
    FIR_HIP(hipHostMalloc((void**)&m->i8_pin, 64, hipHostMallocDefault));
    FIR_HIP(hipEventCreateWithFlags(&m->i8_ev, hipEventDisableTiming));
    FIR_HIP(hipMalloc((void**)&partial, (size_t)kI8Slices * d4 * 4 * sizeof(double)));
    hipLaunchKernelGGL(k_i8_colsum, dim3(d4, kI8Slices), dim3(256), 0, st, m->gal4, tiles, m->dp4, partial);
    hipLaunchKernelGGL(k_i8_mean, dim3((d4 * 4 + 255) / 256), dim3(256), 0, st, (const double*)partial, d4, m->feat, n, m->i8_mu, m->i8_par);
    hipLaunchKernelGGL(k_i8_rows<0>, dim3((unsigned)((n + 255) / 256)), dim3(256), 0, st, m->gal4, n, m->dp4, m->feat, (const float*)m->i8_mu, m->i8_gnorm, m->i8_par);
    hipLaunchKernelGGL(k_i8_scale, dim3(1), dim3(1), 0, st, m->i8_par);
    hipLaunchKernelGGL(k_i8_rows<1>, dim3((unsigned)((n + 255) / 256)), dim3(256), 0, st, m->gal4, n, m->dp4, m->feat, (const float*)m->i8_mu, m->i8_gnorm, m->i8_par);
    const int64_t total = rblocks * m->dk8 * 64;
    hipLaunchKernelGGL(k_i8_pack_gallery, dim3((unsigned)((total + 255) / 256)), dim3(256), 0, st, m->gal4, n, m->dp4, m->dk8, m->feat, (const float*)m->i8_mu,
                       (const float*)m->i8_par, m->g8);
    float h[4] = {0.f, 0.f, 0.f, 0.f};
    hipError_t e = hipGetLastError();
    if (e == hipSuccess) e = hipMemcpyAsync(h, m->i8_par, sizeof h, hipMemcpyDeviceToHost, st);
    if (e == hipSuccess) e = hipStreamSynchronize(st);
    (void)hipFree(partial);
    FIR_HIP(e);
    m->i8_G = std::sqrt(h[2]);
    m->i8_R = h[3];
    m->i8_built = true;
    return FIR_OK;
}
static int gemm_wants_i8_(fir_gemm* m, GemmCall& c, bool* out) {
    *out = false;
    if (m->i8_pending) {
        const hipError_t eq = hipEventQuery(m->i8_ev);
        if (eq == hipSuccess) {
            m->i8_pending = false;
            if ((int64_t)m->i8_pin[0] * 16 > (int64_t)m->i8_pending_qb) { m->i8_off = true; m->i8_off_why = "second passes"; }
        } else if (eq == hipErrorNotReady) (void)hipGetLastError();
    }
    if (m->i8_mode == 0 || m->precision != FIR_GEMM_F16 || m->f64 || c.k != 1 || c.num_classes > 0 || m->feat != m->v.d || m->feat > 1024 || m->feat < 8 ||
        c.qb <= 32 || m->dbg_skip)
        return FIR_OK;
    if (m->i8_mode < 0 && (kI8AutoMinQueries <= 0 || c.qb < kI8AutoMinQueries)) return FIR_OK;
    if (m->i8_mode < 0 && m->i8_off) { c.i8_went_back = true; return FIR_OK; }
    if (!m->i8_built && m->i8_off) { c.i8_went_back = true; return FIR_OK; }
    if (!m->i8_built) {
        const int rc = gemm_build_i8_(m, c.st);
        if (rc) {
            (void)hipGetLastError();
            gemm_free_i8_(m);
            if (rc != FIR_ERR_NOMEM) return rc;
            m->i8_off = true; m->i8_off_why = "no memory";
            c.i8_went_back = true;
            return FIR_OK;
        }
        if (!(m->i8_R <= kI8AutoMaxRG * m->i8_G)) { m->i8_off = true; m->i8_off_why = "R / G"; }
    }
    if (m->i8_mode < 0 && m->i8_off) { c.i8_went_back = true; return FIR_OK; }
    if (!m->i8_built) return FIR_OK;
    *out = true;
    return FIR_OK;
}

static bool adaptive_for_(const fir_gemm* m, const GemmCall& c, int nq_sb) {
    if (m->precision != FIR_GEMM_F16 || m->adaptive <= 0 || (c.k > 1 && !m->adaptive_topk)) return false;
    if (c.num_classes > 0) return false;
    if (m->adaptive > 1 || c.k == 1) return true;
    const int pairs_sb = ((nq_sb + kQT - 1) / kQT + 1) / 2;
    const int P = launch_pairs_(pairs_sb, c.streamed ? kShareStreamed : kShareMax);
    const int64_t row_groups = ((c.n + 31) / 32 + kGemmBlock / 64 - 1) / (kGemmBlock / 64);
    return P >= 8 || c.n <= 65536 || row_groups * P / std::max(c.grid, 1) >= 100;
}

static int gemm_fb_reserve_(fir_gemm* m, int32_t qb) {
    if ((size_t)qb <= m->ok_cap) return FIR_OK;
    FIR_HIP(hipDeviceSynchronize());
    (void)hipFree(m->ok); (void)hipFree(m->fb_list); (void)hipFree(m->fb_list2); (void)hipFree(m->fb_tau2);
    m->ok = nullptr; m->fb_list = nullptr; m->fb_list2 = nullptr; m->fb_tau2 = nullptr;
    m->ok_cap = 0;
    const size_t cap = (size_t)std::max(qb, 1024);
    FIR_HIP(hipMalloc((void**)&m->ok, cap * sizeof(int)));
    FIR_HIP(hipMalloc((void**)&m->fb_list, cap * sizeof(int)));
    FIR_HIP(hipMalloc((void**)&m->fb_list2, cap * sizeof(int)));
    FIR_HIP(hipMalloc((void**)&m->fb_tau2, cap * sizeof(float)));
    m->ok_cap = cap;
    return FIR_OK;
}

static int gemm_reserve_(fir_gemm* m, const GemmCall& c) {
    const int rcr = gemm_fb_reserve_(m, c.qb);
    if (rcr) return rcr;
    const int need = (std::min(c.sbq, c.qb) + 2 * kQT - 1) / (2 * kQT) * (2 * kQT);
    if (need > m->lists_cap) {
        FIR_HIP(hipStreamSynchronize(c.st));
        FIR_HIP(hipStreamSynchronize(m->side));
        for (int b = 0; b < 2; ++b) {
            (void)hipFree(m->lists[b]); (void)hipFree(m->counts[b]);
            m->lists[b] = nullptr; m->counts[b] = nullptr;
        }
        m->lists_cap = 0;
        for (int b = 0; b < 2; ++b) {
            FIR_HIP(hipMalloc((void**)&m->lists[b], (size_t)need * kListCap * sizeof(unsigned long long)));
            FIR_HIP(hipMalloc((void**)&m->counts[b], (size_t)need * sizeof(int)));
        }
        m->lists_cap = need;
    }
    if (m->precision != FIR_GEMM_F16 && !m->sample)
        FIR_HIP(hipMalloc((void**)&m->sample, (size_t)kPasses * kQT * m->sample_rows * sizeof(float)));
    return FIR_OK;
}

static int gemm_prep_f16_(fir_gemm* m, const GemmCall& c, hipStream_t ps, int sb) {
    const int b = sb & 1, nq = c.sb_queries(sb), k = c.k;
    const int pairs = ((nq + kQT - 1) / kQT + 1) / 2;
    const float* dq = c.sb_first(sb);
    if (c.i8) {
        hipLaunchKernelGGL(k_gemm_qprep_i8, dim3(pairs * 2 * kQT), dim3(64), 0, ps, dq, nq, c.d, c.qs, (const float*)m->i8_mu, (const float*)m->i8_par, c.e_rel,
                           m->erel_scale, m->qnorm[b], m->qmul[b], m->qinv[b], m->i8_eabs[b], m->counts[b], m->awin[b], m->aT[b], sb == 0 ? m->fb_state : (int*)nullptr,
                           (const int*)nullptr, (const int*)nullptr, 0, (const float*)nullptr, (float*)nullptr);
        hipLaunchKernelGGL(k_gemm_pack_queries_i8, dim3((4 * m->dk8 * 64 + 255) / 256, pairs), dim3(256), 0, ps, dq, nq, c.d, m->dk8, (const float*)m->i8_mu,
                           (const float*)m->qmul[b], m->qbf[b], c.qs);
        return FIR_OK;
    }
    const bool adaptive = adaptive_for_(m, c, nq);
    hipLaunchKernelGGL(k_gemm_qprep_f16, dim3(pairs * 2 * kQT), dim3(64), 0, ps, dq, nq, c.d, m->gallery_exp, m->qnorm[b], m->qmul[b], m->qinv[b], c.qs,
                       m->counts[b], adaptive ? m->awin[b] : (float*)nullptr, adaptive ? m->aT[b] : (unsigned int*)nullptr,
                       (const float*)m->gmax, c.e_rel, k > 1 ? k : 0, (unsigned int*)nullptr, sb == 0 ? m->fb_state : (int*)nullptr);
    hipLaunchKernelGGL(k_gemm_pack_queries_f16x, dim3((4 * m->dk16 * 64 + 255) / 256, pairs), dim3(256), 0, ps, dq, nq, c.d, m->dk16, m->qmul[b],
                       m->qbf[b], c.qs);
    if (adaptive) return FIR_OK;
    if (c.num_classes > 0) {
        const int64_t rows = std::min<int64_t>(c.n, std::max<int64_t>(kClassSampleRows, c.n * k / m->class_sample_div));
        const int rc = fir_class_scan_dev_(m->g, dq, nq, c.d, c.num_classes, k, rows, nullptr, nullptr, m->tau[b], ps);
        if (rc) return rc;
        hipLaunchKernelGGL(k_gemm_tau_class, dim3((pairs * 2 * kQT + 255) / 256), dim3(256), 0, ps, m->tau[b], pairs * 2 * kQT, nq, c.d, m->qnorm[b], m->gmax, c.e_rel);
        return FIR_OK;
    }
    const int sub_stride = k > 1 ? kPasses * kQT : 0;
    FIR_HIP(hipMemsetD32Async((hipDeviceptr_t)m->smin[b], (int)0xFF800000u, sub_stride ? (size_t)kRtSubsets * sub_stride : (size_t)pairs * 2 * kQT, ps));
    const int64_t sample_blocks = ((int64_t)m->rt_sample_rows + 31) / 32;
    const int rb_stride = (int)std::max<int64_t>(1, ((c.n + 31) / 32) / sample_blocks);
    for (int p0 = 0; p0 < pairs;) {
        const int P = launch_pairs_(pairs - p0, kShareMax);
        const size_t qo = (size_t)p0;
        hipLaunchKernelGGL(pick_x(2, c.streamed, c.odd), dim3(c.grid), dim3(kGemmBlock), kHalfLds, ps, m->gh, m->gnorm, m->qbf[b] + qo * 4 * m->dk16 * 64,
                           m->qinv[b] + qo * 2 * kQT, c.n, (int64_t)0, sample_blocks * 32, m->dk16, m->tau[b], m->lists[b], m->counts[b], (float*)nullptr,
                           0, P, P <= 1 ? 1 : 0, rb_stride, m->smin[b] + qo * 2 * kQT, sub_stride);
        p0 += P;
    }
    if (sub_stride)
        hipLaunchKernelGGL(k_gemm_tau_kmin, dim3((pairs * 2 * kQT + 255) / 256), dim3(256), 0, ps, m->smin[b], sub_stride, k, m->tau[b], pairs * 2 * kQT, nq,
                           m->qnorm[b], m->gmax, c.e_rel);
    else
        hipLaunchKernelGGL(k_gemm_tau_min, dim3((pairs * 2 * kQT + 255) / 256), dim3(256), 0, ps, m->smin[b], m->tau[b], pairs * 2 * kQT, nq, m->qnorm[b], m->gmax, c.e_rel);
    return FIR_OK;
}

static int gemm_prep_f32_bf16_(fir_gemm* m, const GemmCall& c, hipStream_t ps, int sb) {
    const int b = sb & 1, nq = c.sb_queries(sb), np = (nq + kQT - 1) / kQT;
    const float* dq = c.sb_first(sb);
    const int sample_rows = m->sample_rows, sample_grid = (sample_rows + 63) / 64;
    hipLaunchKernelGGL(k_gemm_qnorm, dim3(np * kQT), dim3(64), 0, ps, dq, nq, c.d, m->qnorm[b]);
    FIR_HIP(hipMemsetAsync(m->counts[b], 0, (size_t)np * kQT * sizeof(int), ps));
    if (m->precision == FIR_GEMM_F32) {
        hipLaunchKernelGGL(k_gemm_pack_queries, dim3(((kQT / 32) * m->dq8 * 64 + 255) / 256, np), dim3(256), 0, ps, dq, nq, c.d, m->dq8, m->qm[b]);
        hipLaunchKernelGGL(k_gemm_proxy<0>, dim3(sample_grid, np), dim3(128), c.lds, ps, m->gm, m->gnorm, m->qm[b], c.n, (int64_t)0,
                           (int64_t)sample_rows, m->dq8, m->tau[b], m->lists[b], m->counts[b], m->sample, sample_rows);
    } else {
        hipLaunchKernelGGL(k_gemm_pack_queries_bf16, dim3(((kQT / 32) * m->dk16 * 64 + 255) / 256, np), dim3(256), 0, ps, dq, nq, c.d, m->dk16,
                           m->qbf[b]);
        hipLaunchKernelGGL(k_gemm_proxy_bf16<0>, dim3(sample_grid, np), dim3(128), 0, ps, m->gb, m->gnorm, m->qbf[b], c.n, (int64_t)0,
                           (int64_t)sample_rows, m->dk16, m->tau[b], m->lists[b], m->counts[b], m->sample, sample_rows);
    }
    hipLaunchKernelGGL(k_gemm_tau, dim3(np * kQT), dim3(256), 0, ps, m->sample, sample_rows, m->tau[b], 0x7FFFFFFF, m->qnorm[b], m->gmax, c.e_rel,
                       c.k > 1 ? 1 : 0);
    return FIR_OK;
}

static void gemm_audit_mark_(fir_gemm* m, int i, hipStream_t s) {
#ifdef FIR_AUDIT
    if (!m->debug_counts) return;
    if (!m->phase_ev[i]) (void)hipEventCreate(&m->phase_ev[i]);
    if (m->phase_ev[i]) (void)hipEventRecord(m->phase_ev[i], s);
#else
    (void)m; (void)i; (void)s;
#endif
}

static int gemm_prep_(fir_gemm* m, const GemmCall& c, int sb) {
    hipStream_t ps = c.serial_prep ? c.st : m->side;
    const int b = sb & 1;
    if (c.serial_prep && sb >= 2) FIR_HIP(hipStreamWaitEvent(c.st, m->rerank_done[b], 0));
    if (c.h_queries) {
        const size_t off = (size_t)sb * c.sbq * c.qs;
        FIR_HIP(hipMemcpyAsync((void*)(c.d_queries + off), c.h_queries + off, (size_t)c.sb_queries(sb) * c.qs * sizeof(float), hipMemcpyHostToDevice, m->copy));
        FIR_HIP(hipEventRecord(m->copy_done[b], m->copy));
        FIR_HIP(hipStreamWaitEvent(ps, m->copy_done[b], 0));
    }
    gemm_audit_mark_(m, 0, ps);
    const int rc = m->precision == FIR_GEMM_F16 ? gemm_prep_f16_(m, c, ps, sb) : gemm_prep_f32_bf16_(m, c, ps, sb);
    if (rc) return rc;
    FIR_HIP(hipGetLastError());
    gemm_audit_mark_(m, 1, ps);
    FIR_HIP(hipEventRecord(m->prep_done[b], ps));
    return FIR_OK;
}

static int gemm_pass_f16_(fir_gemm* m, const GemmCall& c, int sb) {
    const int b = sb & 1, nq = c.sb_queries(sb), k = c.k;
    const int pairs = ((nq + kQT - 1) / kQT + 1) / 2;
    const int64_t n = c.n;
    if (c.i8) {
        auto bytes8 = [&](int P) { return (double)((n + 31) / 32) * m->dk8 * 1024.0 + P * (4.0 * m->dk8 * 1024.0 + 128.0 * 8.0); };
        const fir_x8_entry& ran8 = find_x8(3, c.odd);
        int nl = 0, pf = 1, rc8 = FIR_OK;
        for (int p0 = 0; p0 < pairs; ++nl) {
            const int P = launch_pairs_(pairs - p0, kShareMax);
            if (p0 == 0) pf = P;
            const size_t qo = (size_t)p0;
            if ((rc8 = fir_gallery_profile_begin_(m->g, c.st))) return rc8;
            hipLaunchKernelGGL(ran8.fn, dim3(c.grid, 1), dim3(kGemmBlock), kHalfLds, c.st, m->g8, m->i8_gnorm, m->qbf[b] + qo * 4 * m->dk8 * 64, m->qinv[b] + qo * 2 * kQT,
                               n, (int64_t)0, n, m->dk8, m->awin[b] + qo * 2 * kQT, m->lists[b] + qo * 2 * kQT * kListCap, m->counts[b] + qo * 2 * kQT,
                               m->qnorm[b] + qo * 2 * kQT, m->sample_rows, P, (P <= 1 ? 1 : 0) | m->adapt_dbg, 1, m->aT[b] + qo * 2 * kQT, 0);
            if ((rc8 = fir_gallery_profile_end_(m->g, c.st, bytes8(P)))) return rc8;
            p0 += P;
        }
        fir_gallery_note_dispatch_(m->g, (const void*)ran8.fn, ran8.name, sb == 0, c.grid, nl, kGemmBlock, kHalfLds, 128 * pf, bytes8(pf), 2.0 * (double)n * c.d * 128.0 * pf);
        hipLaunchKernelGGL(k_gemm_adapt_final, dim3((pairs * 2 * kQT + 255) / 256), dim3(256), 0, c.st, m->aT[b], m->qnorm[b], m->tau[b], pairs * 2 * kQT, nq, 0);
        return FIR_OK;
    }
    const bool adaptive = adaptive_for_(m, c, nq);
    const bool njb_shape = c.streamed ? !c.odd : (m->dk16 % (4 * kRing)) == 0;
    const int njb = (k == 1 && adaptive && !m->dbg_skip && njb_shape) ? (nq <= 16 ? 1 : nq <= 32 ? 2 : 8) : 8;
    const int mode = adaptive ? (k > 1 ? 4 : 3) : 1;
    auto launch_bytes = [&](int P) { return (double)((n + 31) / 32) * m->dk16 * 1024.0 + P * (4.0 * m->dk16 * 1024.0 + 128.0 * 8.0); };
    int nlaunch = 0, p_first = 1, rc = FIR_OK;
    for (int p0 = 0; p0 < pairs; ++nlaunch) {
        const int P = launch_pairs_(pairs - p0, c.streamed ? kShareStreamed : kShareMax);
        if (p0 == 0) p_first = P;
        const int nt = P <= 1 ? 1 : 0;
        const size_t qo = (size_t)p0;
        if ((rc = fir_gallery_profile_begin_(m->g, c.st))) return rc;
        if (adaptive)
            hipLaunchKernelGGL(pick_x(mode, c.streamed, c.odd, k > 1 ? 0 : m->dbg_skip, njb), dim3(c.grid, 1), dim3(c.streamed ? kGemmBlock : m->dbg_block), kHalfLds, c.st,
                               m->gh, m->gnorm, m->qbf[b] + qo * 4 * m->dk16 * 64, m->qinv[b] + qo * 2 * kQT, n, (int64_t)0, n, m->dk16, m->awin[b] + qo * 2 * kQT,
                               m->lists[b] + qo * 2 * kQT * kListCap, m->counts[b] + qo * 2 * kQT, m->qnorm[b] + qo * 2 * kQT, m->sample_rows, P, nt | m->adapt_dbg, 1,
                               m->aT[b] + qo * 2 * kQT * (k > 1 ? 8 : 1), k > 1 ? k : 0);
        else
            hipLaunchKernelGGL(pick_x(mode, c.streamed, c.odd), dim3(c.grid, 1), dim3(kGemmBlock), kHalfLds, c.st, m->gh, m->gnorm, m->qbf[b] + qo * 4 * m->dk16 * 64,
                               m->qinv[b] + qo * 2 * kQT, n, (int64_t)0, n, m->dk16, m->tau[b] + qo * 2 * kQT, m->lists[b] + qo * 2 * kQT * kListCap,
                               m->counts[b] + qo * 2 * kQT, (float*)nullptr, m->sample_rows, P, nt, 1, (unsigned int*)nullptr, 0);
        if ((rc = fir_gallery_profile_end_(m->g, c.st, launch_bytes(P)))) return rc;
        p0 += P;
    }
    const fir_x_entry& ran = find_x(mode, c.streamed, c.odd, njb);
    const char* ran_name = ran.name;
    if (c.i8_went_back) {
        if (sb == 0) m->i8_note = std::string(ran.name) + " (int8 nomination off for this gallery: " + m->i8_off_why + ")";
        ran_name = m->i8_note.c_str();
    }
    fir_gallery_note_dispatch_(m->g, (const void*)ran.fn, ran_name, sb == 0, c.grid, nlaunch, kGemmBlock, kHalfLds, 128 * p_first, launch_bytes(p_first),
                               2.0 * (double)n * c.d * 128.0 * p_first);
    if (adaptive)
        hipLaunchKernelGGL(k_gemm_adapt_final, dim3((pairs * 2 * kQT + 255) / 256), dim3(256), 0, c.st, m->aT[b], m->qnorm[b], m->tau[b], pairs * 2 * kQT, nq, k > 1 ? k : 0);
    return FIR_OK;
}

static void gemm_pass_f32_bf16_(fir_gemm* m, const GemmCall& c, int sb) {
    const int b = sb & 1, np = (c.sb_queries(sb) + kQT - 1) / kQT, grid = c.grid, sample_rows = m->sample_rows;
    const int64_t n = c.n;
    if (m->precision == FIR_GEMM_F32) {
        hipLaunchKernelGGL(k_gemm_proxy<1>, dim3(grid, np), dim3(kGemmBlock), c.lds, c.st, m->gm, m->gnorm, m->qm[b], n, (int64_t)0, n, m->dq8,
                           m->tau[b], m->lists[b], m->counts[b], m->sample, sample_rows);
        fir_gallery_note_dispatch_(m->g, (const void*)k_gemm_proxy<1>, "fir::k_gemm_proxy<1>", sb == 0, grid, np, kGemmBlock, c.lds, 64,
                                   np * ((double)((n + 31) / 32) * m->dq8 * 1024.0), 2.0 * (double)n * c.d * 64.0 * np);
        return;
    }
    const int pairs = m->wide ? np / 2 : 0;
    if (pairs > 0)
        hipLaunchKernelGGL(k_gemm_proxy_bf16_wide, dim3(grid, pairs), dim3(kGemmBlock), kWideLds, c.st, m->gb, m->gnorm, m->qbf[b], n, m->dk16,
                           m->tau[b], m->lists[b], m->counts[b]);
    if (np > 2 * pairs) {
        const size_t p0 = (size_t)2 * pairs;
        hipLaunchKernelGGL(k_gemm_proxy_bf16<1>, dim3(grid, np - 2 * pairs), dim3(kGemmBlock), c.lds, c.st, m->gb, m->gnorm,
                           m->qbf[b] + p0 * (kQT / 32) * m->dk16 * 128, n, (int64_t)0, n, m->dk16, m->tau[b] + p0 * kQT,
                           m->lists[b] + p0 * kQT * kListCap, m->counts[b] + p0 * kQT, m->sample + p0 * kQT * sample_rows, sample_rows);
    }
    fir_gallery_note_dispatch_(m->g, (const void*)k_gemm_proxy_bf16_wide, pairs > 0 ? "fir::k_gemm_proxy_bf16_wide" : "fir::k_gemm_proxy_bf16<1>", sb == 0,
                               grid, pairs > 0 ? pairs : np, kGemmBlock, pairs > 0 ? (size_t)kWideLds : c.lds, pairs > 0 ? 128 : 64,
                               (pairs + (np - 2 * pairs)) * ((double)((n + 31) / 32) * m->dk16 * 2048.0), 2.0 * (double)n * c.d * 64.0 * np);
}

static void gemm_rerank_(fir_gemm* m, const GemmCall& c, int sb, hipStream_t rs) {
    const int b = sb & 1, q0 = sb * c.sbq, nq = c.sb_queries(sb);
    if (c.num_classes > 0)
        hipLaunchKernelGGL(k_gemm_rerank_classes, dim3(nq), dim3(64), gemm_rerank_lds_(m), rs, m->lists[b], m->counts[b], m->tau[b], m->gal4, c.sb_first(sb), m->qnorm[b], m->gmax,
                           m->v.cls, c.num_classes, c.n, c.d, m->dp4, m->v.row_offset, c.e_rel, m->rerank_group, c.k,
                           c.d_keys ? (unsigned long long*)c.d_keys + (size_t)q0 * c.k : nullptr, c.d_classes ? c.d_classes + (size_t)q0 * c.k : nullptr, m->ok + q0,
                           c.qs, m->rowmajor);
    else
        gemm_launch_rerank_(m, rs, nq, {m->lists[b], m->counts[b], m->tau[b], m->qnorm[b], c.i8 ? m->i8_eabs[b] : nullptr, c.i8 ? m->i8_par + 2 : nullptr}, c.sb_first(sb),
                            c.e_rel, c.k, c.d_keys + (size_t)q0 * c.k, m->ok + q0, {m->fb_state, m->fb_list, m->fb_tau2, q0, nullptr, 0});
}

#ifdef FIR_AUDIT
static int gemm_audit_report_(fir_gemm* m, const GemmCall& c) {
    const int last = c.nsb - 1, b = last & 1;
    if (!m->dump_phases.empty()) {
        FIR_HIP(hipStreamSynchronize(c.st));
        std::vector<unsigned long long> h(8 * 256);
        FIR_HIP(hipMemcpy(h.data(), m->lists[b] + (size_t)(2 * kQT - 1) * kListCap + 2048, h.size() * 8, hipMemcpyDeviceToHost));
        if (FILE* f = std::fopen(m->dump_phases.c_str(), "w")) {
            for (int w = 0; w < 8; ++w)
                for (int u = 0; u < 240; ++u) std::fprintf(f, "%d %d %llu %llu\n", w, u, h[(size_t)w * 256 + u] >> 20, h[(size_t)w * 256 + u] & 0xFFFFFull);
            for (int w = 0; w < 8; ++w)
                std::fprintf(f, "# end %d %llu %llu %llu %llu\n", w, h[(size_t)w * 256 + 240], h[(size_t)w * 256 + 241], h[(size_t)w * 256 + 242], h[(size_t)w * 256 + 243]);
            std::fclose(f);
        }
    }
    if (m->debug_counts) {
        FIR_HIP(hipStreamSynchronize(c.st));
        const int nql = c.sb_queries(last);
        std::vector<int> hc((size_t)nql), h_ok((size_t)nql);
        FIR_HIP(hipMemcpy(hc.data(), m->counts[b], (size_t)nql * sizeof(int), hipMemcpyDeviceToHost));
        FIR_HIP(hipMemcpy(h_ok.data(), m->ok + (size_t)last * c.sbq, (size_t)nql * sizeof(int), hipMemcpyDeviceToHost));
        long long sum = 0;
        int mx = 0, bad = 0, over = 0;
        for (int v : hc) { sum += v; mx = std::max(mx, v); over += v > kListCap ? 1 : 0; }
        for (int v : h_ok) bad += v ? 0 : 1;
        std::vector<float> ht((size_t)nql);
        FIR_HIP(hipMemcpy(ht.data(), m->tau[b], (size_t)nql * sizeof(float), hipMemcpyDeviceToHost));
        double ts = 0;
        int ninf = 0;
        for (float v : ht) { if (v < 1e30f) ts += v; else ++ninf; }
        float ms[3] = {0.f, 0.f, 0.f};
        if (c.serial_prep && m->phase_ev[3])
            for (int i = 0; i < 3; ++i) (void)hipEventElapsedTime(&ms[i], m->phase_ev[i], m->phase_ev[i + 1]);
        std::fprintf(stderr, "fir_gemm: appended rows per query (last super-batch of %d): mean %.1f, max %d; tau: mean %.6f, %d not finite; %d uncertified; "
                     "%d lists overflowed; preparation %.3f ms, full passes %.3f ms, re-rank %.3f ms\n", nql,
                     (double)sum / nql, mx, ts / std::max(1, nql - ninf), ninf, bad, over, ms[0], ms[1], ms[2]);
    }
    return FIR_OK;
}
#endif

static int gemm_finish_classes_(fir_gemm* m, const GemmCall& c) {
    std::vector<int> h_ok((size_t)c.qb);
    FIR_HIP(hipMemcpyAsync(h_ok.data(), m->ok, (size_t)c.qb * sizeof(int), hipMemcpyDeviceToHost, c.st));
    FIR_HIP(hipStreamSynchronize(c.st));
    int uncertified = 0;
    for (int q0 = 0; q0 < c.qb;) {
        int q1 = q0;
        while (q1 < c.qb && !h_ok[q1]) ++q1;
        if (q1 == q0) { ++q0; continue; }
        const int rc = fir_class_scan_dev_(m->g, c.d_queries + (size_t)q0 * c.qs, q1 - q0, c.d, c.num_classes, c.k, 0, c.d_keys ? c.d_keys + (size_t)q0 * c.k : nullptr,
                                           c.d_classes ? c.d_classes + (size_t)q0 * c.k : nullptr, nullptr, c.st);
        if (rc) return rc;
        uncertified += q1 - q0;
        q0 = q1;
    }
    if (uncertified) hipLaunchKernelGGL(k_gemm_fb_count, dim3(1), dim3(1), 0, c.st, m->fb_state, uncertified);
    FIR_HIP(hipGetLastError());
    return FIR_OK;
}

static int gemm_search(fir_gemm* m, const float* d_queries, int32_t qb, int k, uint64_t* d_keys, void* stream, const float* h_queries = nullptr,
                       int32_t num_classes = 0, int32_t* d_classes = nullptr) {
    if (!m || (!d_keys && !(num_classes > 0 && d_classes)) || (qb > 0 && !d_queries)) return fir_fail_(FIR_ERR_ARG, "NULL argument");
    if (qb < 0) return fir_fail_(FIR_ERR_ARG, "qb < 0");
    if (k < 1 || k > (num_classes > 0 ? 32 : kTopKMax)) return fir_fail_(FIR_ERR_ARG, "k=%d outside [1,%d]", k, num_classes > 0 ? 32 : kTopKMax);
    if (qb == 0) return FIR_OK;
    FIR_HIP(hipSetDevice(m->v.device));
    hipStream_t st = stream ? (hipStream_t)stream : m->v.stream;
    FirCallOrder order(m->g, st);
    if (order.rc) return order.rc;
    GemmCall c;
    c.d_queries = d_queries; c.h_queries = h_queries; c.qb = qb; c.k = k; c.d_keys = d_keys; c.st = st;
    c.num_classes = num_classes; c.d_classes = d_classes;
    c.d = m->feat; c.qs = m->v.d; c.n = m->v.n; c.grid = m->v.cus;
    if (c.n == 0 && h_queries) FIR_HIP(hipMemcpyAsync((void*)d_queries, h_queries, (size_t)qb * c.qs * sizeof(float), hipMemcpyHostToDevice, st));
    if (c.n == 0 && num_classes > 0) return fir_class_scan_dev_(m->g, d_queries, qb, c.d, num_classes, k, 0, d_keys, d_classes, nullptr, st);
    if (c.n == 0)
        return k == 1 ? fir_search_top1_exact_keys_dev_(m->g, d_queries, qb, 0, c.d, d_keys, st)
                      : fir_search_topk_exact_keys_dev_(m->g, d_queries, qb, c.d, k, d_keys, st);
    c.streamed = gemm_streamed_(m);
    c.odd = gemm_odd_(m);
    {
        const int rc8 = gemm_wants_i8_(m, c, &c.i8);
        if (rc8) return rc8;
    }
    if (c.i8) { c.streamed = false; c.odd = gemm_odd8_(m); }
    c.lds = m->precision == FIR_GEMM_F32 ? (size_t)(kQT / 32) * std::min(m->dq8, kSlab8) * 64 * sizeof(float4)
                                         : (size_t)(kQT / 32) * std::min(m->dk16, kSlab16) * 128 * sizeof(uint4);
    c.e_rel = m->erel_scale * (8.0f * (float)c.d * 5.9604645e-8f +
              (m->precision == FIR_GEMM_BF16_SPLIT ? 6.1035156e-5f : m->precision == FIR_GEMM_F16 ? 9.765625e-4f * 1.0625f : 0.0f));
    if (c.i8) c.e_rel = m->erel_scale * (8.0f * (float)c.d * 5.9604645e-8f);
    const bool short_launches = (double)c.n * (double)c.d <= 1.5e8;
    c.sbq = std::min(kPasses * kQT, std::max(1024, ((short_launches ? qb : qb / 4) + 1023) / 1024 * 1024));
    c.nsb = (qb + c.sbq - 1) / c.sbq;
    c.serial_prep = !h_queries;
    c.one_stream = c.nsb == 1 && c.serial_prep;
    int rc = gemm_reserve_(m, c);
    if (rc) return rc;
    if (m->precision != FIR_GEMM_F16) FIR_HIP(hipMemsetAsync(m->fb_state, 0, 2 * sizeof(int), st));
    if (!c.one_stream) {
        FIR_HIP(hipEventRecord(m->queries_ready, st));
        FIR_HIP(hipStreamWaitEvent(m->side, m->queries_ready, 0));
    }
    if ((rc = gemm_prep_(m, c, 0))) return rc;
    for (int sb = 0; sb < c.nsb; ++sb) {
        const int b = sb & 1;
        if (c.serial_prep) { if (sb >= 1 && (rc = gemm_prep_(m, c, sb))) return rc; }
        else if (sb + 1 < c.nsb && (rc = gemm_prep_(m, c, sb + 1))) return rc;
        FIR_HIP(hipStreamWaitEvent(st, m->prep_done[b], 0));
        if (m->precision == FIR_GEMM_F16) { if ((rc = gemm_pass_f16_(m, c, sb))) return rc; }
        else gemm_pass_f32_bf16_(m, c, sb);
        FIR_HIP(hipEventRecord(m->main_done[b], st));
        gemm_audit_mark_(m, 2, st);
        hipStream_t rs = c.one_stream ? st : m->side;
        if (!c.one_stream) FIR_HIP(hipStreamWaitEvent(m->side, m->main_done[b], 0));
        gemm_rerank_(m, c, sb, rs);
        gemm_audit_mark_(m, 3, rs);
        FIR_HIP(hipEventRecord(m->rerank_done[b], rs));
        m->passes += (c.sb_queries(sb) + kQT - 1) / kQT;
    }
    if (!c.one_stream) FIR_HIP(hipStreamWaitEvent(st, m->rerank_done[(c.nsb - 1) & 1], 0));
    FIR_HIP(hipGetLastError());
    m->last_kind = 1; m->last_b = (c.nsb - 1) & 1; m->last_nq = c.sb_queries(c.nsb - 1); m->last_sc_rounds = 0; m->last_i8 = c.i8;
#ifdef FIR_AUDIT
    if ((rc = gemm_audit_report_(m, c))) return rc;
#endif
    if (num_classes > 0) return gemm_finish_classes_(m, c);
    const int sc_rounds = m->precision == FIR_GEMM_F16 && qb > 32 ? std::min(kScRounds, (qb + kScQueries - 1) / kScQueries) : 0;
    m->last_sc_rounds = sc_rounds;
    if ((rc = gemm_finish_(m, d_queries, k, d_keys, st, c.e_rel, sc_rounds, c.streamed, c.i8))) return rc;
    if (c.i8 && m->i8_mode < 0 && !m->i8_pending) {
        FIR_HIP(hipMemcpyAsync(m->i8_pin, m->fb_state, sizeof(int), hipMemcpyDeviceToHost, st));
        FIR_HIP(hipEventRecord(m->i8_ev, st));
        m->i8_pending = true;
        m->i8_pending_qb = qb;
    }
    return FIR_OK;
}

extern "C" {

void fir_gemm_set_int8_(fir_gemm* m, int32_t mode) { if (m) m->i8_mode = mode > 0 ? 1 : mode < 0 ? -1 : 0; }

int fir_gemm_search_top1_keys_dev(fir_gemm* m, const float* d_queries, int32_t qb, uint64_t* d_keys, void* stream) {
    return gemm_search(m, d_queries, qb, 1, d_keys, stream);
}

int fir_gemm_search_topk_keys_dev(fir_gemm* m, const float* d_queries, int32_t qb, int32_t k, uint64_t* d_keys, void* stream) {
    return gemm_search(m, d_queries, qb, k, d_keys, stream);
}

int fir_gemm_search_top_classes_keys_dev(fir_gemm* m, const float* d_queries, int32_t qb, int32_t num_classes, int32_t k, uint64_t* d_keys,
                                         int32_t* d_classes, void* stream) {
    if (!m || (qb > 0 && !d_queries)) return fir_fail_(FIR_ERR_ARG, "NULL argument");
    if (m->precision != FIR_GEMM_F16 || m->f64) return fir_fail_(FIR_ERR_ARG, "the distinct-class form needs a FIR_GEMM_F16 state");
    if (qb < 0) return fir_fail_(FIR_ERR_ARG, "qb < 0");
    if (k < 1 || k > 32) return fir_fail_(FIR_ERR_ARG, "k=%d outside [1,32]", k);
    if (num_classes < 1 || num_classes > (1 << 24)) return fir_fail_(FIR_ERR_ARG, "num_classes=%d outside [1,%d]", num_classes, 1 << 24);
    if (!m->v.cls && m->v.n > 0) return fir_fail_(FIR_ERR_STATE, "gallery was created without class labels");
    if (qb > 0 && !d_keys && !d_classes) return fir_fail_(FIR_ERR_ARG, "d_keys and d_classes are both NULL");
    if (qb == 0) return FIR_OK;
    return gemm_search(m, d_queries, qb, k, d_keys, stream, nullptr, num_classes, d_classes);
}

int fir_gemm_search_few_keys_dev(fir_gemm* m, const float* d_queries, int32_t qb, uint64_t* d_keys, void* stream) {
    if (!m || !d_keys || !d_queries) return fir_fail_(FIR_ERR_ARG, "NULL argument");
    if (qb < 1 || qb > 8) return fir_fail_(FIR_ERR_ARG, "qb=%d outside [1,8]", qb);
    if (m->precision != FIR_GEMM_F16) return fir_fail_(FIR_ERR_ARG, "the few-query form needs the fp16 copy");
    FIR_HIP(hipSetDevice(m->v.device));
    hipStream_t st = stream ? (hipStream_t)stream : m->v.stream;
    FirCallOrder order(m->g, st);
    if (order.rc) return order.rc;
    const int d = m->feat, qs = m->v.d;
    const int64_t n = m->v.n;
    if (n == 0) return fir_search_top1_exact_keys_dev_(m->g, d_queries, qb, 0, d, d_keys, st);
    const int nqt = qb <= 1 ? 1 : qb <= 2 ? 2 : qb <= 4 ? 4 : 8;
    if (nqt > m->proxies_nq) {
        if (m->proxies) FIR_HIP(hipFree(m->proxies));
        m->proxies = nullptr;
        m->proxies_nq = 0;
        FIR_HIP(hipMalloc((void**)&m->proxies, (size_t)nqt * n * sizeof(float)));
        m->proxies_nq = nqt;
    }
    if (m->lists_cap < 2 * kQT) {
        for (int bb = 0; bb < 2; ++bb) {
            (void)hipFree(m->lists[bb]); (void)hipFree(m->counts[bb]);
            m->lists[bb] = nullptr; m->counts[bb] = nullptr;
        }
        m->lists_cap = 0;
        for (int bb = 0; bb < 2; ++bb) {
            FIR_HIP(hipMalloc((void**)&m->lists[bb], (size_t)2 * kQT * kListCap * sizeof(unsigned long long)));
            FIR_HIP(hipMalloc((void**)&m->counts[bb], (size_t)2 * kQT * sizeof(int)));
        }
        m->lists_cap = 2 * kQT;
    }
    {
        const int rcr = gemm_fb_reserve_(m, qb);
        if (rcr) return rcr;
    }
    const float e_rel = m->erel_scale * (8.0f * (float)d * 5.9604645e-8f + 9.765625e-4f * 1.0625f);
    const int b = 0;
    hipLaunchKernelGGL(k_gemm_qprep_f16, dim3(2 * kQT), dim3(64), 0, st, d_queries, qb, d, m->gallery_exp, m->qnorm[b], m->qmul[b], m->qinv[b], qs, m->counts[b],
                       (float*)nullptr, (unsigned int*)nullptr, (const float*)nullptr, 0.f, 0, m->smin[b], m->fb_state);
    hipLaunchKernelGGL(k_gemm_pack_queries_f16x, dim3((4 * m->dk16 * 64 + 255) / 256, 1), dim3(256), 0, st, d_queries, qb, d, m->dk16, m->qmul[b], m->qbf[b], qs);
    const dim3 grid((unsigned)std::min<int64_t>((int64_t)m->v.cus * 8, ((n + 31) / 32 + 3) / 4));
    const size_t lds = (size_t)m->dk16 * 2 * nqt * sizeof(uint4);
    typedef void (*scan_fn)(const uint4*, const float*, const uint4*, const float*, int64_t, int, float*, unsigned int*);
    const scan_fn scan = nqt == 1 ? k_gemm_scan_f16x<1> : nqt == 2 ? k_gemm_scan_f16x<2> : nqt == 4 ? k_gemm_scan_f16x<4> : k_gemm_scan_f16x<8>;
    const double bytes = (double)((n + 31) / 32) * m->dk16 * 1024.0 + (double)nqt * n * 4.0;
    {
        int rcp = fir_gallery_profile_begin_(m->g, st);
        if (rcp) return rcp;
        hipLaunchKernelGGL(scan, grid, dim3(256), lds, st, m->gh, m->gnorm, m->qbf[b], m->qinv[b], n, m->dk16, m->proxies, m->smin[b]);
        if ((rcp = fir_gallery_profile_end_(m->g, st, bytes))) return rcp;
    }
    fir_gallery_note_dispatch_(m->g, (const void*)scan, "fir::k_gemm_scan_f16x", 1, (int)grid.x, 1, 256, lds, nqt, bytes, 2.0 * (double)n * d * nqt);
    hipLaunchKernelGGL(k_gemm_tau_min, dim3(1), dim3(256), 0, st, m->smin[b], m->tau[b], 2 * kQT, qb, m->qnorm[b], m->gmax, e_rel);
    hipLaunchKernelGGL(k_gemm_select, dim3((unsigned)std::min<int64_t>(1024, (n + 255) / 256), qb), dim3(256), 0, st, m->proxies, n, m->tau[b], m->lists[b], m->counts[b]);
    gemm_launch_rerank_(m, st, qb, {m->lists[b], m->counts[b], m->tau[b], m->qnorm[b]}, d_queries, e_rel, 1, d_keys, m->ok,
                        {m->fb_state, m->fb_list, m->fb_tau2, 0, nullptr, 0});
    FIR_HIP(hipGetLastError());
    m->passes += 1;
    m->last_kind = 2; m->last_b = b; m->last_nq = qb; m->last_sc_rounds = 0; m->last_i8 = false;
    return gemm_finish_(m, d_queries, 1, d_keys, st, e_rel, 0, gemm_streamed_(m));
}

int fir_gemm_nominations_(fir_gemm* m, int32_t which, int32_t q0, int32_t nq, int32_t max_entries, int32_t* counts, float* tau, float* qnorm,
                          uint64_t* lists, float* proxies, float* gmax, int32_t* qmap, int32_t* live) {
    if (!m || (m->f64 && which != 0)) return fir_fail_(FIR_ERR_ARG, "not a fir_gemm nomination state");
    if (which < 0 || which > 1 || q0 < 0 || nq < 0 || max_entries < 0 || max_entries > kListCap) return fir_fail_(FIR_ERR_ARG, "bad range");
    if (!m->last_kind) return fir_fail_(FIR_ERR_STATE, "no call has run on this state yet");
    FIR_HIP(hipSetDevice(m->v.device));
    FIR_HIP(hipDeviceSynchronize());
    const int b = m->last_b;
    int have = m->last_nq, off = 0;
    if (which == 1) {
        int cnt = 0;
        FIR_HIP(hipMemcpy(&cnt, m->fb_state, sizeof(int), hipMemcpyDeviceToHost));
        const int rounds = std::min(m->last_sc_rounds, (cnt + kScQueries - 1) / kScQueries);
        if (m->last_kind != 1 || rounds <= 0 || !m->sc_lists) have = 0;
        else { off = (rounds - 1) * kScQueries; have = std::min(kScQueries, cnt - off); }
    }
    if (live) *live = have;
    if (gmax) FIR_HIP(hipMemcpy(gmax, m->last_i8 ? m->i8_par + 2 : m->gmax, sizeof(float), hipMemcpyDeviceToHost));
    if (nq == 0) return FIR_OK;
    if (q0 + nq > have) return fir_fail_(FIR_ERR_ARG, "slots [%d,%d) of %d", q0, q0 + nq, have);
    const int* d_counts = which ? m->sc_counts : m->counts[b];
    const float* d_tau = which ? m->sc_tau : m->tau[b];
    const float* d_qnorm = which ? m->sc_qnorm : m->qnorm[b];
    const unsigned long long* d_lists = which ? m->sc_lists : m->lists[b];
    if (counts) FIR_HIP(hipMemcpy(counts, d_counts + q0, (size_t)nq * sizeof(int), hipMemcpyDeviceToHost));
    if (tau) FIR_HIP(hipMemcpy(tau, d_tau + q0, (size_t)nq * sizeof(float), hipMemcpyDeviceToHost));
    if (qnorm) FIR_HIP(hipMemcpy(qnorm, d_qnorm + q0, (size_t)nq * sizeof(float), hipMemcpyDeviceToHost));
    if (lists && max_entries > 0)
        FIR_HIP(hipMemcpy2D(lists, (size_t)max_entries * 8, d_lists + (size_t)q0 * kListCap, (size_t)kListCap * 8, (size_t)max_entries * 8, (size_t)nq,
                            hipMemcpyDeviceToHost));
    if (qmap) {
        if (which) FIR_HIP(hipMemcpy(qmap, m->fb_list + off + q0, (size_t)nq * sizeof(int), hipMemcpyDeviceToHost));
        else for (int i = 0; i < nq; ++i) qmap[i] = q0 + i;
    }
    if (proxies) {
        if (m->last_kind != 2 || !m->proxies) return fir_fail_(FIR_ERR_STATE, "the most recent call was not the few-query scan");
        FIR_HIP(hipMemcpy(proxies, m->proxies + (size_t)q0 * m->v.n, (size_t)nq * m->v.n * sizeof(float), hipMemcpyDeviceToHost));
    }
    return FIR_OK;
}

int fir_gemm_search_staged_(fir_gemm* m, const float* h_queries, float* d_stage, int32_t qb, int32_t k, uint64_t* d_keys, void* stream) {
    if (!h_queries || !d_stage) return fir_fail_(FIR_ERR_ARG, "NULL argument");
    return gemm_search(m, d_stage, qb, k, d_keys, stream, h_queries);
}

}

#include "fir_gemm_f64.h"
```

### fast-image-recognition_amd/csrc/fir_gemm_f16x.h

```cpp
#pragma once
#include <type_traits>

typedef float f32x4 __attribute__((ext_vector_type(4)));
typedef int i32x4 __attribute__((ext_vector_type(4)));

__global__ void __launch_bounds__(256) k_gemm_pack_gallery_f16x(const float4* __restrict__ gal4, int64_t n, int dp4, int dk16, float scale,
                                                                 uint4* __restrict__ gh, int kmax) {
    const int64_t o = (int64_t)blockIdx.x * 256 + threadIdx.x;
    const int64_t rblocks = (n + 31) / 32;
    if (o >= rblocks * dk16 * 64) return;
    const int l = (int)(o & 63);
    const int64_t t = o >> 6;
    const int piece = (int)(t % dk16);
    const int64_t rb = t / dk16;
    const int kk = piece >> 1, s = piece & 1;
    const int64_t row = rb * 32 + 16 * s + (l & 15);
    f16x8 v;
#pragma unroll
    for (int j = 0; j < 8; ++j) {
        const int k = 32 * kk + 8 * (l >> 4) + j;
        float x = 0.f;
        if (row < n && k < kmax) {
            const float4 g = gal4[((row >> 6) * dp4 + (k >> 2)) * 64 + (row & 63)];
            x = (k & 3) == 0 ? g.x : (k & 3) == 1 ? g.y : (k & 3) == 2 ? g.z : g.w;
        }
        v[j] = (_Float16)(x * scale);
    }
    uint4 u;
    __builtin_memcpy(&u, &v, 16);
    gh[o] = u;
}

__global__ void __launch_bounds__(256) k_gemm_pack_queries_f16x(const float* q, int nq, int d, int dk16, const float* __restrict__ qmul, uint4* qh,
                                                                 int qstride, const int* __restrict__ qmap = nullptr, const int* __restrict__ state = nullptr,
                                                                 int live_off = 0) {
    if (qmap) {
        nq = state[0] - live_off;
        if (nq <= 0) return;
        nq = nq < 2 * kQT ? nq : 2 * kQT;
    }
    const int dk32 = dk16 >> 1;
    const int q_base = (int)blockIdx.y * 2 * kQT;
    qh += (size_t)blockIdx.y * 8 * dk32 * 64;
    const int o = blockIdx.x * 256 + threadIdx.x;
    if (o >= 8 * dk32 * 64) return;
    const int l = o & 63;
    const int t = o >> 6;
    const int kk = t % dk32, jb = t / dk32;
    const int qi = q_base + jb * 16 + (l & 15);
    const float mul = qi < nq ? qmul[qi] : 0.f;
    f16x8 v;
#pragma unroll
    for (int j = 0; j < 8; ++j) {
        const int k = 32 * kk + 8 * (l >> 4) + j;
        const float x = (qi < nq && k < d) ? q[(size_t)(qmap ? qmap[qi] : qi) * qstride + k] : 0.f;
        v[j] = (_Float16)(x * mul);
    }
    uint4 u;
    __builtin_memcpy(&u, &v, 16);
    qh[o] = u;
}

__device__ __forceinline__ f32x4 mfma_x_(const f16x8 a, const f16x8 b, const f32x4 c) { return __builtin_amdgcn_mfma_f32_16x16x32_f16(a, b, c, 0, 0, 0); }
__device__ __forceinline__ i32x4 mfma_x_(const f16x8 a, const f16x8 b, const i32x4 c) {
    i32x4 ai, bi;
    __builtin_memcpy(&ai, &a, 16);
    __builtin_memcpy(&bi, &b, 16);
    return __builtin_amdgcn_mfma_i32_16x16x64_i8(ai, bi, c, 0, 0, 0);
}

constexpr int kXStage = 16;
template <int MODE, int STREAMED, int ODD, int DBG = 0, int NJB = 8, int I8 = 0>
__global__ void __launch_bounds__(kGemmBlock, 1) k_gemm_proxy_f16x(const uint4* __restrict__ gh, const float* __restrict__ gnorm, const uint4* qh,
                                                                    const float* __restrict__ qinv, int64_t n, int64_t row_begin, int64_t row_end,
                                                                    int dk16, const float* tau, unsigned long long* lists, int* counts,
                                                                    float* sample, int sample_rows, int share, int nt_flags,
                                                                    int rb_stride, unsigned int* smin, int sub_stride) {
    extern __shared__ __attribute__((aligned(16))) uint4 lqx[];
    if (MODE == 1 && smin != nullptr && (int)smin[0] - sub_stride <= 0) return;
    const int nt = nt_flags & 1;
    __shared__ float tau_s[2 * kQT], qinv_s[2 * kQT];
    constexpr bool kAdapt = MODE == 3 || MODE == 4;
    constexpr bool kSlots = MODE == 4;
    const int kth = kSlots ? sub_stride : 1;
    auto kth_of_slots = [&](const unsigned int* sl) -> unsigned int {
        const uint4 lo = *(const uint4*)sl, hi = *(const uint4*)(sl + 4);
        const unsigned int v[8] = {lo.x, lo.y, lo.z, lo.w, hi.x, hi.y, hi.z, hi.w};
        unsigned int res = 0xFFFFFFFFu;
#pragma unroll
        for (int i = 0; i < 8; ++i) {
            int rank = 0;
#pragma unroll
            for (int j = 0; j < 8; ++j) rank += (v[j] < v[i] || (v[j] == v[i] && j < i)) ? 1 : 0;
            res = rank == kth - 1 ? v[i] : res;
        }
        return res;
    };
    constexpr bool kAppend = MODE == 1 || kAdapt;
    __shared__ unsigned long long skeys[kAppend ? 2 * kQT * kXStage : 1];
    __shared__ int scnt[kAppend ? 2 * kQT : 1];
    __shared__ float qn_s[kAdapt ? 2 * kQT : 1], win_s[kAdapt ? 2 * kQT : 1];
    __shared__ __attribute__((aligned(16))) unsigned int slot_s[kSlots ? 2 * kQT * 8 : 8];
    __shared__ float tq_s[kAdapt ? 2 * kQT : 1];
    constexpr bool kDynForm = !STREAMED && kAdapt && !(DBG & 128);
    if (kDynForm && share <= 0) share = 1;
    __shared__ int next_blk;
    unsigned long long t_entry = 0;
    if (DBG & 256) t_entry = __builtin_amdgcn_s_memtime();
    int pair_of_wg = (int)blockIdx.y;
    int64_t rg_first = blockIdx.x, rg_step = gridDim.x, rg_last = -1;
    int range = (int)blockIdx.x;
    if (share > 0) {
        const int w = (int)blockIdx.x, xcd = w & 7, slot = w >> 3;
        const int ranges = ((int)gridDim.x >> 3) / share * 8;
        range = xcd + 8 * (slot / share);
        if (range >= ranges) return;
        pair_of_wg = slot % share;
        const int64_t nrg_all = (((row_end + 31) / 32 - row_begin / 32) + (blockDim.x >> 6) - 1) / (blockDim.x >> 6);
        rg_first = nrg_all * range / ranges;
        rg_last = nrg_all * (range + 1) / ranges;
        rg_step = 1;
    }
    const int dk32 = dk16 >> 1;
    {
        const size_t pr = (size_t)pair_of_wg;
        qh += pr * 8 * dk32 * 64;
        qinv += pr * 2 * kQT;
        tau += pr * 2 * kQT;
        lists += pr * 2 * kQT * kListCap;
        counts += pr * 2 * kQT;
        if (MODE == 0) sample += pr * 2 * kQT * ((sample_rows + 31) / 32);
        if (MODE == 2 || MODE == 3) smin += pr * 2 * kQT;
        if (MODE == 4) smin += pr * 2 * kQT * 8;
        if (kAdapt) sample += pr * 2 * kQT;
    }
    const int64_t rbs = MODE == 2 ? rb_stride : 1;
    const int lane = threadIdx.x & 63, wave = __builtin_amdgcn_readfirstlane(threadIdx.x >> 6);
    const int wpb = blockDim.x >> 6;
    if (threadIdx.x < 2 * kQT) {
        if (kSlots) {
            unsigned int v8[8];
#pragma unroll
            for (int sl = 0; sl < 8; ++sl) v8[sl] = atomicMin(&smin[threadIdx.x * 8 + sl], 0xFFFFFFFFu);
#pragma unroll
            for (int sl = 0; sl < 8; ++sl) slot_s[threadIdx.x * 8 + sl] = v8[sl];
            tau_s[threadIdx.x] = __uint_as_float(kth_of_slots(&slot_s[threadIdx.x * 8]));
        } else
        tau_s[threadIdx.x] = MODE == 1 ? tau[threadIdx.x] : MODE == 3 ? __uint_as_float(atomicMin(&smin[threadIdx.x], 0xFFFFFFFFu)) : 0.f;
        qinv_s[threadIdx.x] = qinv[threadIdx.x];
        if (kAppend) scnt[threadIdx.x] = 0;
        if (kDynForm && threadIdx.x == 0) next_blk = wpb;
        if (kAdapt) {
            qn_s[threadIdx.x] = sample[threadIdx.x];
            win_s[threadIdx.x] = tau[threadIdx.x];
            tq_s[threadIdx.x] = tau_s[threadIdx.x] - qn_s[threadIdx.x];
        }
    }
    const int64_t rb_begin = row_begin / 32, rb_end = (row_end + 31) / 32;
    const int64_t nrg = (rb_end - rb_begin + wpb - 1) / wpb;
    constexpr int RING = (!STREAMED && NJB < 8) ? 2 * kRing : kRing;
    const int units = dk16 / RING;
    int64_t rg_end = rg_last >= 0 ? rg_last : nrg;
    int64_t rg = rg_first;
    if (rg >= rg_end) return;
    const int64_t blk0 = rb_begin + rg_first * wpb;
    if (kDynForm) {
        rg = blk0 + wave;
        rg_end = rb_begin + rg_end * wpb;
    }
#define FIR_X_LD(P) (nt ? ld_nt(P) : *(P))
#define FIR_X_RBP(RG) (kDynForm ? (RG) : rb_begin + (RG) * wpb + wave)
#define FIR_X_BLOCK(RG) (gh + (size_t)((FIR_X_RBP(RG) < rb_end ? FIR_X_RBP(RG) : rb_end - 1) * rbs) * dk16 * 64)
    const uint4* a_cur = FIR_X_BLOCK(rg);
    uint4 cur[RING], nxt[RING];
#pragma unroll
    for (int u = 0; u < RING; ++u) cur[u] = FIR_X_LD(a_cur + (size_t)u * 64 + lane);
    constexpr int kUnitsPerSlab = kSlabH / RING;
    const uint32_t lds_base = (uint32_t)(uintptr_t)(void __attribute__((address_space(3)))*)lqx;
    auto request_piece = [&](int hq, int slot, int i) {
        const uint4* src = qh + ((size_t)wave * dk32 + (size_t)hq * 4 + i) * 64 + lane;
        const uint32_t dst = __builtin_amdgcn_readfirstlane(lds_base + (uint32_t)slot * (4 * RING * 1024) + (uint32_t)(i * 8 + wave) * 1024);
        asm volatile("s_mov_b32 m0, %0\n\tglobal_load_lds_dwordx4 %1, off" ::"s"(dst), "v"(src) : "memory");
    };
    int ring_c = 0, hq3 = 0;
    if (STREAMED) {
        int hq = 0;
        for (int cc = 0; cc < 3; ++cc) {
#pragma unroll
            for (int i = 0; i < 4; ++i) request_piece(hq, cc, i);
            hq = hq + 1 == units ? 0 : hq + 1;
        }
        hq3 = hq;
        asm volatile("s_waitcnt vmcnt(0)" ::: "memory");
        __syncthreads();
    } else {
        for (int i = threadIdx.x; i < NJB * dk32 * 64; i += blockDim.x) {
            const int jb = i / (dk32 * 64), r = i - jb * dk32 * 64;
            lqx[(size_t)((r >> 6) * 8 + jb) * 64 + (r & 63)] = qh[(size_t)jb * dk32 * 64 + r];
        }
        __syncthreads();
    }
    float smallest[NJB];
#pragma unroll
    for (int j = 0; j < NJB; ++j) smallest[j] = __builtin_huge_valf();
    uint4 B[NJB];
#pragma unroll
    for (int j = 0; j < NJB; ++j) B[j] = lqx[lane + j * 64];
    constexpr bool kDefer = kAppend && !(DBG & 8) && !(DBG & 1);
    using acc_t = typename std::conditional<I8 != 0, i32x4, f32x4>::type;
    acc_t acc[2][NJB];
    if (kDefer) {
#pragma unroll
        for (int j = 0; j < NJB; ++j) acc[0][j] = acc[1][j] = acc_t{0, 0, 0, 0};
    }
    bool pend = false;
    int64_t p_rb = 0;
    float4 pg[2] = {};
    float p_gmin = __builtin_huge_valf();
    float m2r[kDefer ? NJB : 1], tqr[kDefer ? NJB : 1];
    if (kDefer) {
#pragma unroll
        for (int jb = 0; jb < NJB; ++jb) {
            m2r[jb] = 2.0f * qinv_s[jb * 16 + (lane & 15)];
            tqr[jb] = kAdapt ? tq_s[jb * 16 + (lane & 15)] : tau_s[jb * 16 + (lane & 15)];
        }
    }
    bool warm = kAdapt;
    auto slots_to_T = [&](int q) {
        const unsigned int tk = kth_of_slots(&slot_s[q * 8]);
        if (tk < atomicMin((unsigned int*)&tau_s[q], tk)) tq_s[q] = __uint_as_float(tk) - qn_s[q];
    };
    auto lower_T = [&](int q, const float (&pv)[8], float mn) {
        if (!kSlots) {
            const float tn = fmaxf((mn + qn_s[q]) + win_s[q], 0.f);
            if (tn < tau_s[q]) {
                if (__float_as_uint(tn) < atomicMin((unsigned int*)&tau_s[q], __float_as_uint(tn))) tq_s[q] = tn - qn_s[q];
                atomicMin(&smin[q], __float_as_uint(tn));
            }
        } else {
            const uint4 s_lo = *(const uint4*)&slot_s[q * 8], s_hi = *(const uint4*)&slot_s[q * 8 + 4];
            const unsigned int have[8] = {s_lo.x, s_lo.y, s_lo.z, s_lo.w, s_hi.x, s_hi.y, s_hi.z, s_hi.w};
            const float qn = qn_s[q], win = win_s[q];
            bool fell = false;
#pragma unroll
            for (int i = 0; i < 8; ++i) {
                const float tn = fmaxf((pv[i] + qn) + win, 0.f);
                if (pv[i] == pv[i] && tn < __uint_as_float(have[i])) {
                    atomicMin(&slot_s[q * 8 + i], __float_as_uint(tn));
                    atomicMin(&smin[q * 8 + i], __float_as_uint(tn));
                    fell = true;
                }
            }
            if (fell) slots_to_T(q);
        }
    };
    auto exchange_T = [&]() {
        __syncthreads();
        if (threadIdx.x < 2 * kQT) {
            if (kSlots) {
                unsigned int mine[8], old[8];
#pragma unroll
                for (int sl = 0; sl < 8; ++sl) mine[sl] = slot_s[threadIdx.x * 8 + sl];
#pragma unroll
                for (int sl = 0; sl < 8; ++sl) old[sl] = (nt_flags & 8) ? mine[sl] : atomicMin(&smin[threadIdx.x * 8 + sl], mine[sl]);
#pragma unroll
                for (int sl = 0; sl < 8; ++sl) slot_s[threadIdx.x * 8 + sl] = old[sl] < mine[sl] ? old[sl] : mine[sl];
                tau_s[threadIdx.x] = __uint_as_float(kth_of_slots(&slot_s[threadIdx.x * 8]));
            } else {
            const unsigned int mine = __float_as_uint(tau_s[threadIdx.x]);
            const unsigned int old = (nt_flags & 8) ? mine : atomicMin(&smin[threadIdx.x], mine);
            tau_s[threadIdx.x] = __uint_as_float(old < mine ? old : mine);
            }
            tq_s[threadIdx.x] = tau_s[threadIdx.x] - qn_s[threadIdx.x];
        }
        __syncthreads();
    };
    int blk_no = 0;
    int dbg_units = 0;
    int touch_e = 0, touch_o = 0;
    int64_t rg_next = rg;
    for (; rg < rg_end; rg = rg_next) {
        const bool warm_it = warm;
        warm = false;
        rg_next = rg + rg_step;
        int tk = 0;
        if (kDynForm && lane == 0) tk = (int)atomicInc((unsigned int*)&next_blk, 0xFFFFFFFFu);
        const int64_t rbp = FIR_X_RBP(rg);
        const int64_t rb = rbp * rbs;
        const bool active = rbp < rb_end;
        const uint4* a_nxt = a_cur;
        auto next_block = [&]() {
            if (kDynForm) rg_next = blk0 + __builtin_amdgcn_readfirstlane(tk);
            const int64_t rgn = rg_next;
            a_nxt = FIR_X_BLOCK(rgn < rg_end ? rgn : rg);
        };
        constexpr bool kNextLate = kDynForm && !(DBG & 512);
        if (!kNextLate) next_block();
        if (kAdapt) {
            if (!warm_it && wave < NJB && !(nt_flags & 4)) {
                const int v = blk_no >> __builtin_ctz((unsigned)blk_no | 0x40000000u);
                if ((v == 1 || v == 3) && lane < 16) {
                    int zl;
                    asm volatile("v_mbcnt_lo_u32_b32 %0, -1, 0\n\tv_mbcnt_hi_u32_b32 %0, -1, %0" : "=v"(zl));
                    const int ql = 16 * wave + zl;
                    if (kSlots) {
                        unsigned int mine[8], old[8];
#pragma unroll
                        for (int sl = 0; sl < 8; ++sl) mine[sl] = slot_s[ql * 8 + sl];
#pragma unroll
                        for (int sl = 0; sl < 8; ++sl) old[sl] = atomicMin(&smin[ql * 8 + sl], mine[sl]);
                        bool fell = false;
#pragma unroll
                        for (int sl = 0; sl < 8; ++sl)
                            if (old[sl] < mine[sl]) { atomicMin(&slot_s[ql * 8 + sl], old[sl]); fell = true; }
                        if (fell) slots_to_T(ql);
                    } else {
                    const unsigned int mine = __float_as_uint(tau_s[ql]);
                    const unsigned int old = atomicMin(&smin[ql], mine);
                    if (old < mine && old < atomicMin((unsigned int*)&tau_s[ql], old)) tq_s[ql] = __uint_as_float(old) - qn_s[ql];
                    }
                }
            }
            ++blk_no;
        }
        float4 gns[2];
        const float* gn_blk = n >= 32 ? gnorm + (rb * 32 < ((n - 32) & ~(int64_t)3) ? rb * 32 : ((n - 32) & ~(int64_t)3)) : (const float*)gh;
        const bool full_block = active && rbp * 32 >= row_begin && rbp * 32 + 32 <= row_end && rb * 32 + 32 <= n && (MODE != 0 || rb * 32 + 32 <= sample_rows);
        unsigned int* smin_blk = MODE == 2 ? smin + (size_t)(wave & 7) * sub_stride : nullptr;
        auto check_jb = [&](int jb, int64_t rbq, const float4 g0, const float4 g1, float gminq) {
            const int q = jb * 16 + (lane & 15);
            const float m2 = kDefer ? m2r[jb] : 2.0f * qinv_s[q];
            const float tq = kDefer ? tqr[jb] : kAdapt ? tq_s[q] : tau_s[q];
            float amax;
            if (I8) {
                int imax;
                asm("v_max3_i32 %0, %1, %2, %3\n\tv_max3_i32 %0, %0, %4, %5\n\tv_max3_i32 %0, %0, %6, %7\n\tv_max_i32 %0, %0, %8"
                    : "=&v"(imax)
                    : "v"(acc[0][jb][0]), "v"(acc[0][jb][1]), "v"(acc[0][jb][2]), "v"(acc[0][jb][3]), "v"(acc[1][jb][0]), "v"(acc[1][jb][1]),
                      "v"(acc[1][jb][2]), "v"(acc[1][jb][3]));
                amax = (float)imax;
            } else
            asm("v_max3_f32 %0, %1, %2, %3\n\tv_max3_f32 %0, %0, %4, %5\n\tv_max3_f32 %0, %0, %6, %7\n\tv_max_f32 %0, %0, %8"
                : "=&v"(amax)
                : "v"(acc[0][jb][0]), "v"(acc[0][jb][1]), "v"(acc[0][jb][2]), "v"(acc[0][jb][3]), "v"(acc[1][jb][0]), "v"(acc[1][jb][1]),
                  "v"(acc[1][jb][2]), "v"(acc[1][jb][3]));
            if (__builtin_expect(!(__builtin_fmaf(-m2, amax, gminq) < tq), 1)) return;
            const float gnv[8] = {g0.x, g0.y, g0.z, g0.w, g1.x, g1.y, g1.z, g1.w};
            float pv[8];
            float mn = __builtin_huge_valf();
#pragma unroll
            for (int i = 0; i < 8; ++i) {
                pv[i] = __builtin_fmaf(-m2, (float)acc[i >> 2][jb][i & 3], gnv[i]);
                mn = fminf(mn, pv[i]);
            }
            if (mn < tq) {
                int lz;
                asm volatile("v_mbcnt_lo_u32_b32 %0, -1, 0\n\tv_mbcnt_hi_u32_b32 %0, -1, %0" : "=v"(lz));
                const int qr = jb * 16 + (lz & 15);
#pragma unroll
                for (int i = 0; i < 8; ++i) {
                    if (pv[i] < tq) {
                        const int64_t row = rbq * 32 + 16 * (i >> 2) + 4 * (lz >> 4) + (i & 3);
                        const unsigned long long key = fir::key_pack(pv[i], (uint32_t)row);
                        const int st = atomicAdd(&scnt[qr], 1);
                        if (st < kXStage) {
                            skeys[qr * kXStage + st] = key;
                        } else {
                            const int slot = atomicAdd(&counts[qr], 1);
                            if (slot < kListCap) lists[(size_t)qr * kListCap + slot] = key;
                            else if (kAdapt) tq_s[qr] = -__builtin_huge_valf();
                        }
                    }
                }
                if (kAdapt) lower_T(qr, pv, mn);
            }
        };
        auto unit = [&](uint4 (&C)[RING], uint4 (&N)[RING], int h, auto first_tag, auto last_tag) {
            constexpr bool kFirst = decltype(first_tag)::value;
            constexpr bool kLast = decltype(last_tag)::value;
            if (kLast && !kFirst && kDefer && kAdapt) {
#pragma unroll
                for (int jb = 0; jb < NJB; ++jb) tqr[jb] = tq_s[jb * 16 + (lane & 15)];
            }
            if (kLast && kNextLate) next_block();
            const uint4* src = kLast ? a_nxt : a_cur + (size_t)(h + 1) * RING * 64;
            const uint4* bq = STREAMED ? lqx + lane + (size_t)(ring_c & 3) * 4 * RING * 64 : lqx + lane + (size_t)(h % kUnitsPerSlab) * RING * 4 * 64;
            unsigned long long t_burst0 = 0;
            if (DBG & 256) t_burst0 = __builtin_amdgcn_s_memtime();
            if (!(DBG & 16) && !(DBG & 2) && !(DBG & 64)) {
                if (nt) {
#pragma unroll
                    for (int u = 0; u < RING; ++u) N[u] = ld_nt(src + (size_t)u * 64 + lane);
                } else {
#pragma unroll
                    for (int u = 0; u < RING; ++u) N[u] = src[(size_t)u * 64 + lane];
                }
            }
            if ((DBG & 512) && pair_of_wg == 0) {
                const uint4* tgt = h + 2 < units ? a_cur + (size_t)(h + 2) * RING * 64 : a_nxt + (size_t)(h + 2 - units) * RING * 64;
                int& tch = (h & 1) ? touch_o : touch_e;
                asm volatile("" ::"v"(tch));
                tch = *(const int*)(tgt + (size_t)lane * 8);
            }
            if (DBG & 256) {
                const unsigned long long t_burst1 = __builtin_amdgcn_s_memtime();
                if (blockIdx.x == 0 && dbg_units < 240 && lane == 0) {
                    unsigned long long* dst = lists + (size_t)(2 * kQT - 1) * kListCap + 2048 + (size_t)wave * 256;
                    dst[dbg_units] = (t_burst0 << 20) | ((t_burst1 - t_burst0) & 0xFFFFFull);
                }
                ++dbg_units;
            }
            if (kLast) {
                unsigned int zl;
                asm volatile("v_mov_b32 %0, 0" : "=v"(zl));
                const float* gb = gn_blk;
                const unsigned int off = 4u * ((unsigned int)lane >> 4) + zl;
                gns[0] = *(const float4*)(gb + off);
                gns[1] = *(const float4*)(gb + off + 16);
            }
            __builtin_amdgcn_sched_barrier(0);
            const uint4* bq_after = STREAMED ? lqx + lane + (size_t)((ring_c + 1) & 3) * 4 * RING * 64
                                             : lqx + lane + (size_t)((kLast ? 0 : h + 1) % kUnitsPerSlab) * RING * 4 * 64;
#pragma unroll
            for (int t = 0; t < RING / 2; ++t) {
                const uint4* bn = t + 1 < RING / 2 ? bq + (size_t)(t + 1) * 8 * 64 : bq_after;
                const f16x8 a0 = as_f16x8(C[2 * t]), a1 = as_f16x8(C[2 * t + 1]);
#pragma unroll
                for (int j = 0; j < NJB; ++j) {
                    if (kDefer && kFirst && t == 0) {
                        check_jb(j, p_rb, pg[0], pg[1], p_gmin);
                    }
                    const f16x8 b = as_f16x8(B[j]);
                    const acc_t zero = {0, 0, 0, 0};
                    if (!(DBG & 32)) {
                        acc[0][j] = mfma_x_(a0, b, kFirst && t == 0 ? zero : acc[0][j]);
                        acc[1][j] = mfma_x_(a1, b, kFirst && t == 0 ? zero : acc[1][j]);
                    } else {
                        asm volatile("" ::"v"(a0), "v"(a1), "v"(b));
                        if (kFirst && t == 0) { acc[0][j] = zero; acc[1][j] = zero; }
                    }
                    if (!(DBG & 4)) B[j] = bn[j * 64];
                    if ((DBG & 64) && t == 0 && RING == 8) {
                        N[j] = nt ? ld_nt(src + (size_t)j * 64 + lane) : src[(size_t)j * 64 + lane];
                    }
                    if ((DBG & 16) && !(DBG & 2) && (j == 3 || j == 7)) {
                        const int u = 2 * t + (j == 7 ? 1 : 0);
                        N[u] = nt ? ld_nt(src + (size_t)u * 64 + lane) : src[(size_t)u * 64 + lane];
                    }
                    __builtin_amdgcn_sched_barrier(0);
                }
                if (STREAMED) request_piece(hq3, (ring_c + 3) & 3, t);
            }
            if (STREAMED) {
                asm volatile("s_waitcnt vmcnt(12)" ::: "memory");
                __builtin_amdgcn_s_barrier();
                ++ring_c;
                hq3 = hq3 + 1 == units ? 0 : hq3 + 1;
            }
            if (kLast && kFirst && kDefer && kAdapt) {
#pragma unroll
                for (int jb = 0; jb < NJB; ++jb) tqr[jb] = tq_s[jb * 16 + (lane & 15)];
            }
            if (kFirst) {
                pend = false;
                p_gmin = __builtin_huge_valf();
            }
        };
        const std::true_type yes;
        const std::false_type no;
        if (!ODD) {
            unit(cur, nxt, 0, yes, no);
            for (int h = 1; h + 1 < units; h += 2) {
                unit(nxt, cur, h, no, no);
                unit(cur, nxt, h + 1, no, no);
            }
            unit(nxt, cur, units - 1, no, yes);
        } else {
            if (ODD == 2) {
                unit(cur, nxt, 0, yes, yes);
            } else {
                unit(cur, nxt, 0, yes, no);
                for (int h = 1; h + 2 < units; h += 2) {
                    unit(nxt, cur, h, no, no);
                    unit(cur, nxt, h + 1, no, no);
                }
                unit(nxt, cur, units - 2, no, no);
                unit(cur, nxt, units - 1, no, yes);
            }
#pragma unroll
            for (int u = 0; u < RING; ++u) cur[u] = nxt[u];
        }
        a_cur = a_nxt;
        if (ODD == 2 || !full_block) asm volatile("" ::"v"(gns[0].x), "v"(gns[0].y), "v"(gns[0].z), "v"(gns[0].w), "v"(gns[1].x), "v"(gns[1].y), "v"(gns[1].z), "v"(gns[1].w));
        if (DBG & 1) {
#pragma unroll
            for (int jb = 0; jb < NJB; ++jb) asm volatile("" ::"v"(acc[0][jb]), "v"(acc[1][jb]));
            continue;
        }
        if (kAdapt && warm_it) {
            if (active && full_block) {
                int lw;
                asm volatile("v_mbcnt_lo_u32_b32 %0, -1, 0\n\tv_mbcnt_hi_u32_b32 %0, -1, %0" : "=v"(lw));
#pragma unroll
                for (int jb = 0; jb < NJB; ++jb) {
                    const int q = jb * 16 + (lw & 15);
                    const float m2 = 2.0f * qinv_s[q];
                    float pv[8];
                    float mn = __builtin_huge_valf();
#pragma unroll
                    for (int s = 0; s < 2; ++s) {
                        const float gnv[4] = {gns[s].x, gns[s].y, gns[s].z, gns[s].w};
#pragma unroll
                        for (int reg = 0; reg < 4; ++reg) {
                            pv[4 * s + reg] = __builtin_fmaf(-m2, (float)acc[s][jb][reg], gnv[reg]);
                            mn = fminf(mn, pv[4 * s + reg]);
                        }
                    }
                    if (kSlots) {
#pragma unroll
                        for (int i = 0; i < 8; ++i) {
                            const float tn = fmaxf((pv[i] + qn_s[q]) + win_s[q], 0.f);
                            if (pv[i] == pv[i] && tn < __uint_as_float(slot_s[q * 8 + i])) atomicMin(&slot_s[q * 8 + i], __float_as_uint(tn));
                        }
                    } else {
                        float o = __shfl_xor(mn, 16, 64);
                        mn = o < mn ? o : mn;
                        o = __shfl_xor(mn, 32, 64);
                        mn = o < mn ? o : mn;
                        const float tn = fmaxf((mn + qn_s[q]) + win_s[q], 0.f);
                        if (lw < 16 && tn < tau_s[q]) atomicMin((unsigned int*)&tau_s[q], __float_as_uint(tn));
                    }
                }
            }
            exchange_T();
            if (kDefer) {
#pragma unroll
                for (int jb = 0; jb < NJB; ++jb) tqr[jb] = tq_s[jb * 16 + (lane & 15)];
#pragma unroll
                for (int jb = 0; jb < NJB; ++jb) asm volatile("" ::"v"(tqr[jb]));
            }
        }
        if (!active) continue;
        if (full_block) {
            const float gmin = fminf(fminf(fminf(gns[0].x, gns[0].y), fminf(gns[0].z, gns[0].w)), fminf(fminf(gns[1].x, gns[1].y), fminf(gns[1].z, gns[1].w)));
            if (kAppend) {
                if (kDefer) {
                    pend = true;
                    p_rb = rb;
                    pg[0] = gns[0];
                    pg[1] = gns[1];
                    p_gmin = gmin;
                } else {
#pragma unroll
                    for (int jb = 0; jb < NJB; ++jb) check_jb(jb, rb, gns[0], gns[1], gmin);
                }
                continue;
            }
#pragma unroll
            for (int jb = 0; jb < NJB; ++jb) {
                const int q = jb * 16 + (lane & 15);
                const float m2 = 2.0f * qinv_s[q];
                float pv[8];
                float mn = __builtin_huge_valf();
#pragma unroll
                for (int s = 0; s < 2; ++s) {
                    const float gnv[4] = {gns[s].x, gns[s].y, gns[s].z, gns[s].w};
#pragma unroll
                    for (int reg = 0; reg < 4; ++reg) {
                        pv[4 * s + reg] = __builtin_fmaf(-m2, (float)acc[s][jb][reg], gnv[reg]);
                        mn = fminf(mn, pv[4 * s + reg]);
                    }
                }
                if (MODE == 2 && !sub_stride) {
                    smallest[jb] = fminf(smallest[jb], mn);
                } else if (MODE == 2) {
#pragma unroll
                    for (int i = 0; i < 8; ++i) {
                        float v = pv[i] == pv[i] ? pv[i] : __builtin_huge_valf();
                        float o = __shfl_xor(v, 16, 64);
                        v = o < v ? o : v;
                        o = __shfl_xor(v, 32, 64);
                        v = o < v ? o : v;
                        if (lane < 16 && v < __builtin_huge_valf()) atomicMin(&smin[(size_t)(i * 8 + (wave & 7)) * sub_stride + q], fir::f32_orderable(v));
                    }
                } else {
                    float o = __shfl_xor(mn, 16, 64);
                    mn = o < mn ? o : mn;
                    o = __shfl_xor(mn, 32, 64);
                    mn = o < mn ? o : mn;
                    if (MODE == 0) { if (lane < 16) sample[(size_t)(rb - rb_begin) * (2 * kQT) + q] = mn; }
                }
            }
            continue;
        }
        int ls;
        asm volatile("v_mbcnt_lo_u32_b32 %0, -1, 0\n\tv_mbcnt_hi_u32_b32 %0, -1, %0" : "=v"(ls));
#pragma unroll
        for (int jb = 0; jb < NJB; ++jb) {
            const int q = jb * 16 + (ls & 15);
            const float m2 = 2.0f * qinv_s[q];
            const float tq = kAdapt ? tq_s[q] : tau_s[q];
            float mn = __builtin_huge_valf();
#pragma unroll
            for (int i = 0; i < 8; ++i) {
                const int64_t row = rb * 32 + 16 * (i >> 2) + 4 * (ls >> 4) + (i & 3);
                if (row >= n || (MODE != 2 && (row < row_begin || row >= row_end))) continue;
                const float p = __builtin_fmaf(-m2, (float)acc[i >> 2][jb][i & 3], gnorm[row]);
                if (MODE == 0) {
                    if (row < sample_rows) mn = p < mn ? p : mn;
                } else if (MODE == 2) {
                    mn = p < mn ? p : mn;
                } else if (p < tq) {
                    const int slot = atomicAdd(&counts[q], 1);
                    if (slot < kListCap) lists[(size_t)q * kListCap + slot] = fir::key_pack(p, (uint32_t)row);
                }
            }
            asm volatile("" ::"v"(tq), "v"(m2));
            if (MODE == 2 && !sub_stride) {
                smallest[jb] = fminf(smallest[jb], mn);
            } else if (MODE != 1 && !kAdapt) {
                float o = __shfl_xor(mn, 16, 64);
                mn = o < mn ? o : mn;
                o = __shfl_xor(mn, 32, 64);
                mn = o < mn ? o : mn;
                if (MODE == 0) { if (lane < 16) sample[(size_t)(rb - rb_begin) * (2 * kQT) + q] = mn; }
                else if (lane < 16 && mn < __builtin_huge_valf()) atomicMin(&smin_blk[q], fir::f32_orderable(mn));
            }
        }
    }
    if ((DBG & 256) && blockIdx.x == 0 && lane == 0) {
        unsigned long long* dst = lists + (size_t)(2 * kQT - 1) * kListCap + 2048 + (size_t)wave * 256;
        dst[240] = (unsigned long long)dbg_units;
        dst[241] = t_entry;
        dst[242] = __builtin_amdgcn_s_memtime();
    }
    if (kDefer && pend) {
        int lt;
        asm volatile("v_mbcnt_lo_u32_b32 %0, -1, 0\n\tv_mbcnt_hi_u32_b32 %0, -1, %0" : "=v"(lt));
        auto last_jb = [&](int jb) {
            const int q = jb * 16 + (lt & 15);
            const float m2 = 2.0f * qinv_s[q];
            const float tq = kAdapt ? tq_s[q] : tau_s[q];
            const float gnv[8] = {pg[0].x, pg[0].y, pg[0].z, pg[0].w, pg[1].x, pg[1].y, pg[1].z, pg[1].w};
            float pv[8];
            float mn = __builtin_huge_valf();
#pragma unroll
            for (int i = 0; i < 8; ++i) {
                pv[i] = __builtin_fmaf(-m2, (float)acc[i >> 2][jb][i & 3], gnv[i]);
                mn = fminf(mn, pv[i]);
            }
            if (mn < tq) {
#pragma unroll
                for (int i = 0; i < 8; ++i) {
                    if (pv[i] < tq) {
                        const int64_t row = p_rb * 32 + 16 * (i >> 2) + 4 * (lt >> 4) + (i & 3);
                        const unsigned long long key = fir::key_pack(pv[i], (uint32_t)row);
                        const int st = atomicAdd(&scnt[q], 1);
                        if (st < kXStage) {
                            skeys[q * kXStage + st] = key;
                        } else {
                            const int slot = atomicAdd(&counts[q], 1);
                            if (slot < kListCap) lists[(size_t)q * kListCap + slot] = key;
                        }
                    }
                }
                if (kAdapt) lower_T(q, pv, mn);
            }
        };
#pragma unroll
        for (int jb = 0; jb < NJB; ++jb) last_jb(jb);
    }
    if (kAppend) {
        __syncthreads();
        if (threadIdx.x < 2 * kQT) {
            const int q = threadIdx.x;
            const int cnt = scnt[q] < kXStage ? scnt[q] : kXStage;
            if (cnt > 0) {
                const int base = atomicAdd(&counts[q], cnt);
                for (int st = 0; st < cnt; ++st)
                    if (base + st < kListCap) lists[(size_t)q * kListCap + base + st] = skeys[q * kXStage + st];
            }
        }
    }
    if ((DBG & 256) && blockIdx.x == 0 && lane == 0)
        lists[(size_t)(2 * kQT - 1) * kListCap + 2048 + (size_t)wave * 256 + 243] = __builtin_amdgcn_s_memtime();
    if (MODE == 2 && !sub_stride) {
#pragma unroll
        for (int jb = 0; jb < NJB; ++jb) {
            float v = smallest[jb];
            v = fminf(v, __shfl_xor(v, 16, 64));
            v = fminf(v, __shfl_xor(v, 32, 64));
            if (lane < 16 && v < __builtin_huge_valf()) atomicMin(&smin[jb * 16 + lane], fir::f32_orderable(v));
        }
    }
#undef FIR_X_BLOCK
#undef FIR_X_RBP
#undef FIR_X_LD
}

constexpr int kRtSubsets = 64;
__global__ void __launch_bounds__(256) k_gemm_tau_kmin(const unsigned int* __restrict__ smin, int sub_stride, int k, float* __restrict__ tau,
                                                        int nq_total, int nq_valid, const float* __restrict__ qnorm,
                                                        const float* __restrict__ gnorm_max_p, float e_rel) {
    const int q = blockIdx.x * 256 + threadIdx.x;
    if (q >= nq_total) return;
    if (q >= nq_valid) { tau[q] = -__builtin_huge_valf(); return; }
    unsigned int best[8];
#pragma unroll
    for (int i = 0; i < 8; ++i) best[i] = 0xFFFFFFFFu;
    for (int s = 0; s < kRtSubsets; ++s) {
        unsigned int v = smin[(size_t)s * sub_stride + q];
        if (v == 0xFF800000u) continue;
#pragma unroll
        for (int i = 0; i < 8; ++i) {
            const bool sw = v < best[i];
            const unsigned int t = best[i];
            best[i] = sw ? v : t;
            v = sw ? t : v;
        }
    }
    unsigned int kth = 0xFFFFFFFFu;
#pragma unroll
    for (int i = 0; i < 8; ++i) kth = i == k - 1 ? best[i] : kth;
    float t = __builtin_huge_valf();
    if (kth != 0xFFFFFFFFu) {
        const float v = fir::f32_from_orderable(kth) + rounding_window_(e_rel, qnorm[q], gnorm_max_p[0]);
        t = nudge_up_(v);
    }
    tau[q] = t;
}

__global__ void __launch_bounds__(256) k_gemm_tau_min(const unsigned int* __restrict__ smin, float* __restrict__ tau, int nq_total, int nq_valid,
                                                       const float* __restrict__ qnorm, const float* __restrict__ gnorm_max_p, float e_rel) {
    const int q = blockIdx.x * 256 + threadIdx.x;
    if (q >= nq_total) return;
    if (q >= nq_valid) { tau[q] = -__builtin_huge_valf(); return; }
    const unsigned int o = smin[q];
    float t = __builtin_huge_valf();
    if (o != 0xFF800000u) {
        const float v1 = fir::f32_from_orderable(o);
        const float v = v1 + rounding_window_(e_rel, qnorm[q], gnorm_max_p[0]);
        t = nudge_up_(v);
    }
    tau[q] = t;
}

typedef _Float16 f16x2x __attribute__((ext_vector_type(2)));
template <int NQ>
__global__ void __launch_bounds__(256) k_gemm_scan_f16x(const uint4* __restrict__ gh, const float* __restrict__ gnorm, const uint4* __restrict__ qh,
                                                         const float* __restrict__ qinv, int64_t n, int dk16, float* __restrict__ proxies,
                                                         unsigned int* __restrict__ smin) {
    extern __shared__ __attribute__((aligned(16))) uint4 qsx[];
    const int dk32 = dk16 >> 1;
    for (int idx = threadIdx.x; idx < dk32 * 4 * NQ; idx += blockDim.x) {
        const int i = idx % NQ, qt = (idx / NQ) & 3, kk = idx / (4 * NQ);
        qsx[idx] = qh[(size_t)kk * 64 + 16 * qt + i];
    }
    __syncthreads();
    const int lane = threadIdx.x & 63, qt = lane >> 4;
    const int64_t gw = (int64_t)blockIdx.x * (blockDim.x >> 6) + (threadIdx.x >> 6), nw = (int64_t)gridDim.x * (blockDim.x >> 6);
    const int64_t nrb = (n + 31) / 32;
    float m2[NQ], smallest[NQ];
#pragma unroll
    for (int i = 0; i < NQ; ++i) { m2[i] = 2.0f * qinv[i]; smallest[i] = __builtin_huge_valf(); }
    for (int64_t rb = gw; rb < nrb; rb += nw) {
        const uint4* a = gh + (size_t)rb * dk16 * 64 + lane;
        float acc[2][NQ];
#pragma unroll
        for (int i = 0; i < NQ; ++i) acc[0][i] = acc[1][i] = 0.f;
        for (int kb0 = 0; kb0 < dk16; kb0 += 8) {
            uint4 g[8];
#pragma unroll
            for (int u = 0; u < 8; ++u) g[u] = ld_nt(a + (size_t)(kb0 + u) * 64);
#pragma unroll
            for (int u = 0; u < 8; ++u) {
                f16x2x gv[4];
                __builtin_memcpy(gv, &g[u], 16);
#pragma unroll
                for (int i = 0; i < NQ; ++i) {
                    const uint4 qq = qsx[(((kb0 + u) >> 1) * 4 + qt) * NQ + i];
                    f16x2x qv[4];
                    __builtin_memcpy(qv, &qq, 16);
#pragma unroll
                    for (int t = 0; t < 4; ++t) acc[u & 1][i] = __builtin_amdgcn_fdot2(gv[t], qv[t], acc[u & 1][i], false);
                }
            }
        }
#pragma unroll
        for (int s = 0; s < 2; ++s) {
            const int64_t row = rb * 32 + 16 * s + (lane & 15);
            const float gn = row < n ? gnorm[row] : 0.f;
#pragma unroll
            for (int i = 0; i < NQ; ++i) {
                float dot = acc[s][i] + __shfl_xor(acc[s][i], 16, 64);
                dot += __shfl_xor(dot, 32, 64);
                if (lane < 16 && row < n) {
                    const float p = __builtin_fmaf(-m2[i], dot, gn);
                    proxies[(size_t)i * n + row] = p;
                    smallest[i] = fminf(smallest[i], p);
                }
            }
        }
    }
#pragma unroll
    for (int i = 0; i < NQ; ++i) {
        float v = smallest[i];
#pragma unroll
        for (int off = 8; off >= 1; off >>= 1) v = fminf(v, __shfl_xor(v, off, 64));
        if (lane == 0 && v < __builtin_huge_valf()) atomicMin(&smin[i], fir::f32_orderable(v));
    }
}
```

### fast-image-recognition_amd/csrc/fir_internal.h

```cpp
#pragma once
#include <hip/hip_runtime.h>
#include <stdint.h>

#include "../../include/fir_amd.h"

struct fir_gallery;

extern "C" int fir_fail_(int code, const char* fmt, ...) __attribute__((format(printf, 2, 3)));
#define FIR_HIP(expr)                                                                                                  \
    do {                                                                                                               \
        hipError_t e_ = (expr);                                                                                        \
        if (e_ != hipSuccess) return fir_fail_(e_ == hipErrorOutOfMemory ? FIR_ERR_NOMEM : FIR_ERR_HIP,               \
                                               "%s failed: %s (%s:%d)", #expr, hipGetErrorString(e_), __FILE__, __LINE__); \
    } while (0)

struct fir_gallery_view {
    int device;
    int cus;
    int64_t n;
    int d;
    int metric;
    int64_t row_offset;
    const int32_t* cls;
    hipStream_t stream;
};
extern "C" int fir_gallery_view_(fir_gallery* g, fir_gallery_view* out);

extern "C" int fir_gallery_call_begin_(fir_gallery* g, hipStream_t st);
extern "C" void fir_gallery_call_end_(fir_gallery* g, hipStream_t st, int finished);
extern "C" int fir_gallery_wait_calls_(fir_gallery* g);
struct FirCallOrder {
    fir_gallery* g;
    hipStream_t st;
    int rc;
    bool finished = false;
    FirCallOrder(fir_gallery* g_, hipStream_t st_) : g(g_), st(st_) { rc = fir_gallery_call_begin_(g, st); }
    ~FirCallOrder() { fir_gallery_call_end_(g, st, finished); }
    void done() { finished = true; }
    FirCallOrder(const FirCallOrder&) = delete;
    FirCallOrder& operator=(const FirCallOrder&) = delete;
};
template <typename F>
struct FirOnExit {
    F f;
    ~FirOnExit() { f(); }
};
template <typename F>
FirOnExit<F> fir_on_exit(F f) { return FirOnExit<F>{f}; }
struct FirBuf {
    void* p = nullptr;
    size_t cap = 0;
    FirBuf() = default;
    FirBuf(const FirBuf&) = delete;
    FirBuf& operator=(const FirBuf&) = delete;
    ~FirBuf() { release(); }
    void release() { if (p) (void)hipFree(p); p = nullptr; cap = 0; }
    hipError_t reserve(size_t bytes) {
        if (p && bytes <= cap) return hipSuccess;
        release();
        const hipError_t e = hipMalloc(&p, bytes < 16 ? 16 : bytes);
        if (e == hipSuccess) cap = bytes < 16 ? 16 : bytes; else p = nullptr;
        return e;
    }
    template <typename T> T* as() const { return (T*)p; }
};
inline int fir_reserve_(FirBuf& b, size_t bytes, const char* what, const char* file, int line) {
    const hipError_t e = b.reserve(bytes);
    if (e == hipSuccess) return FIR_OK;
    return fir_fail_(e == hipErrorOutOfMemory ? FIR_ERR_NOMEM : FIR_ERR_HIP, "%s.reserve(%zu) failed: %s (%s:%d)", what, bytes, hipGetErrorString(e), file, line);
}
#define FIR_RESERVE(buf, bytes) fir_reserve_(buf, bytes, #buf, __FILE__, __LINE__)
extern "C" void fir_set_last_error_(const char* msg);
extern "C" const char* fir_knob_(const char* name);
extern "C" int fir_gallery_tiled_(fir_gallery* g, const void** gal4, int* dp4);

extern "C" int fir_gallery_scratch_(fir_gallery* g, int slot, size_t bytes, void** out);
extern "C" uint64_t fir_gallery_next_counter_(fir_gallery* g, int slot);
extern "C" fir_twd_dispatch_info* fir_gallery_twd_record_(fir_gallery* g);

extern "C" int fir_subrange_distances_dev_(fir_gallery* g, const float* d_queries, int32_t qb, int32_t start, int32_t end, int32_t step,
                                           float* d_out, void* stream);

extern "C" int fir_split_distances_dev_(fir_gallery* g, const float* d_queries, int32_t qb, int32_t split, int32_t end, float* d_out, void* stream);

extern "C" int fir_runtime_init_(int device);

extern "C" int fir_wait_ticket_(hipStream_t st, volatile uint64_t* flag, uint64_t ticket);
extern "C" int fir_gallery_pin_(fir_gallery* g, void** base, size_t* query_bytes, uint64_t** results);
extern "C" uint64_t fir_gallery_next_ticket_(fir_gallery* g);

extern "C" int fir_search_top1_exact_keys_dev_(fir_gallery* g, const float* d_queries, int32_t qb, int32_t start_pos, int32_t end_pos,
                                               uint64_t* d_keys, void* stream);

extern "C" int fir_search_topk_exact_keys_dev_(fir_gallery* g, const float* d_queries, int32_t qb, int32_t end_pos, int32_t k, uint64_t* d_keys, void* stream);

extern "C" int fir_class_scan_dev_(fir_gallery* g, const float* d_queries, int32_t qb, int32_t end_pos, int32_t num_classes, int32_t k,
                                   int64_t sample_rows, uint64_t* d_keys, int32_t* d_classes, float* d_bound, void* stream);

extern "C" int fir_twd_wants_mfma_(fir_gallery* g, int32_t qb, int32_t end_pos);
extern "C" int fir_twd_mfma_classes_(fir_gallery* g, const float* d_queries, int32_t qb, int32_t end_pos, int32_t num_classes, int32_t k,
                                     uint64_t* d_keys, int32_t* d_classes, void* stream, int64_t* exact_answered);
extern "C" int fir_twd_mfma_topk_(fir_gallery* g, const float* d_queries, int32_t qb, int32_t qb_call, int32_t end_pos, int32_t k, uint64_t* d_keys,
                                  void* stream);
extern "C" int fir_gallery_label_range_(fir_gallery* g, int32_t* lo, int32_t* hi);
extern "C" int64_t* fir_gallery_twd_mfma_record_(fir_gallery* g);

extern "C" int fir_gallery_profile_begin_(fir_gallery* g, void* st);
extern "C" int fir_gallery_profile_end_(fir_gallery* g, void* st, double bytes_alg);
extern "C" void fir_gallery_note_dispatch_(fir_gallery* g, const void* fn, const char* name, int first, int gx, int gy, int block, size_t dyn_lds,
                                           int qpp, double bytes, double flops);

struct fir_gemm;
extern "C" int fir_gemm_search_staged_(fir_gemm* m, const float* h_queries, float* d_stage, int32_t qb, int32_t k, uint64_t* d_keys, void* stream);

extern "C" int fir_gemm_create_range_ex_(fir_gallery* g, int32_t precision, int32_t end_pos, int32_t rowmajor_mode, fir_gemm** out);
extern "C" int fir_gemm_nominations_(fir_gemm* m, int32_t which, int32_t q0, int32_t nq, int32_t max_entries, int32_t* counts, float* tau, float* qnorm,
                                     uint64_t* lists, float* proxies, float* gmax, int32_t* qmap, int32_t* live);
extern "C" void fir_gemm_set_int8_(fir_gemm* m, int32_t mode);
extern "C" void fir_gemm_memory_bytes_(const fir_gemm* m, int64_t* fragments, int64_t* rowmajor, int64_t* scratch);

struct fir_cls;
extern "C" int fir_cls_pnn_scores_dev_(fir_cls* c, const double* queries, int32_t qb, double var, double** d_scores, void** stream, int32_t* max_batch);
extern "C" int fir_cls_knn_nearest_dev_(fir_cls* c, const double* queries, int32_t qb, int32_t k, double** d_lists, void** stream, int32_t* max_batch);

extern "C" int fir_gemm_create_f64_(int device, int cus, void* stream, const void* gal2, int64_t nt, int d, int dp2, fir_gemm** out);
extern "C" int fir_gemm_knn_f64_(fir_gemm* m, const double* d_qc, int32_t qb, int32_t kp, int32_t* d_rows, double* d_dist, int32_t* d_ok, void* stream,
                                 const char** kernel_name, double* flops_per_launch, hipEvent_t* ev_pair);
extern "C" int fir_gemm_destroy(fir_gemm* m);
extern "C" int fir_cls_knn_rows_(fir_cls* c, const double* queries, int32_t qb, int32_t kp, int32_t* rows, double* dist, int32_t* ok);
extern "C" fir_gemm* fir_cls_knn_state_(fir_cls* c);
```

Before: 2.490 million queries/s.

## Add 256-query tile variant of int8 top-1 proxy kernel sharing each gallery block

Adds a QH=2 instantiation of the int8 proxy GEMM kernel in which one workgroup holds two 128-query tiles in LDS and runs each loaded gallery block against both halves before moving on. The aim is to halve gallery reads and block-scheduling overhead per query, improving arithmetic intensity in the bandwidth-bound scan. In exchange it uses more LDS and registers, halves the per-query staging buffer, and adds more complex per-half threshold handling. It is enabled by default (i8_tile=-1) when the depth matches 2*kRing and there are at least two query pairs.

```diff
diff --git a/fast-image-recognition_amd/csrc/fir_gemm.hip b/fast-image-recognition_amd/csrc/fir_gemm.hip
--- a/fast-image-recognition_amd/csrc/fir_gemm.hip
+++ b/fast-image-recognition_amd/csrc/fir_gemm.hip
@@ -954,6 +954,7 @@
     int last_b = 0, last_nq = 0;
     int last_sc_rounds = 0;
     bool last_i8 = false;
+    int i8_tile = -1;
     int i8_mode = 0;
     bool i8_built = false, i8_off = false;
     const char* i8_off_why = "";
@@ -1073,11 +1074,45 @@
 #define FIR_X8(M, O) {M, O, k_gemm_proxy_f16x<M, 0, O, 0, 8, 1>, "fir::k_gemm_proxy_i8x<" #M ", " #O ">"}
 static const fir_x8_entry kX8Table[] = {FIR_X8(3, 0), FIR_X8(3, 1), FIR_X8(3, 2), FIR_X8(1, 0), FIR_X8(1, 1), FIR_X8(1, 2)};
 #undef FIR_X8
+static const fir_x8_entry kX8Tile256 = {3, 0, k_gemm_proxy_f16x<3, 0, 0, 0, 8, 1, 2>, "fir::k_gemm_proxy_i8x<3, 0> (256-query tile)"};
 static const fir_x8_entry& find_x8(int mode, int odd) {
     for (const fir_x8_entry& e : kX8Table)
         if (e.mode == mode && e.odd == odd) return e;
     return kX8Table[0];
 }
+static fir_x_fn pick_x8(int mode, int odd, int dbg = 0) {
+#ifdef FIR_AUDIT
+    if (dbg && mode == 3 && !odd) {
+        switch (dbg & 1023) {
+            case 1: return k_gemm_proxy_f16x<3, 0, 0, 1, 8, 1>;
+            case 3: return k_gemm_proxy_f16x<3, 0, 0, 3, 8, 1>;
+            case 5: return k_gemm_proxy_f16x<3, 0, 0, 5, 8, 1>;
+            case 7: return k_gemm_proxy_f16x<3, 0, 0, 7, 8, 1>;
+            case 33: return k_gemm_proxy_f16x<3, 0, 0, 33, 8, 1>;
+            case 35: return k_gemm_proxy_f16x<3, 0, 0, 35, 8, 1>;
+            case 37: return k_gemm_proxy_f16x<3, 0, 0, 37, 8, 1>;
+            default: break;
+        }
+    }
+#endif
+    return find_x8(mode, odd).fn;
+}
+static fir_x_fn pick_x8_tile256(int dbg = 0) {
+#ifdef FIR_AUDIT
+    switch (dbg & 1023) {
+        case 1: return k_gemm_proxy_f16x<3, 0, 0, 1, 8, 1, 2>;
+        case 3: return k_gemm_proxy_f16x<3, 0, 0, 3, 8, 1, 2>;
+        case 5: return k_gemm_proxy_f16x<3, 0, 0, 5, 8, 1, 2>;
+        case 7: return k_gemm_proxy_f16x<3, 0, 0, 7, 8, 1, 2>;
+        case 33: return k_gemm_proxy_f16x<3, 0, 0, 33, 8, 1, 2>;
+        case 35: return k_gemm_proxy_f16x<3, 0, 0, 35, 8, 1, 2>;
+        case 37: return k_gemm_proxy_f16x<3, 0, 0, 37, 8, 1, 2>;
+        default: break;
+    }
+#endif
+    (void)dbg;
+    return kX8Tile256.fn;
+}
 static hipError_t gemm_x_lds_attr_() {
     for (const fir_x_entry& e : kXTable) {
         const hipError_t err = hipFuncSetAttribute((const void*)e.fn, hipFuncAttributeMaxDynamicSharedMemorySize, kHalfLds);
@@ -1087,7 +1122,7 @@
         const hipError_t err = hipFuncSetAttribute((const void*)e.fn, hipFuncAttributeMaxDynamicSharedMemorySize, kHalfLds);
         if (err != hipSuccess) return err;
     }
-    return hipSuccess;
+    return hipFuncSetAttribute((const void*)kX8Tile256.fn, hipFuncAttributeMaxDynamicSharedMemorySize, kHalfLds);
 }
 
 static void gemm_free_i8_(fir_gemm* m) {
@@ -1451,7 +1486,7 @@
         } else if (eq == hipErrorNotReady) (void)hipGetLastError();
     }
     if (m->i8_mode == 0 || m->precision != FIR_GEMM_F16 || m->f64 || c.k != 1 || c.num_classes > 0 || m->feat != m->v.d || m->feat > 1024 || m->feat < 8 ||
-        c.qb <= 32 || m->dbg_skip)
+        c.qb <= 32 || (m->dbg_skip && m->i8_mode != 1))
         return FIR_OK;
     if (m->i8_mode < 0 && (kI8AutoMinQueries <= 0 || c.qb < kI8AutoMinQueries)) return FIR_OK;
     if (m->i8_mode < 0 && m->i8_off) { c.i8_went_back = true; return FIR_OK; }
@@ -1624,16 +1659,18 @@
     const int64_t n = c.n;
     if (c.i8) {
         auto bytes8 = [&](int P) { return (double)((n + 31) / 32) * m->dk8 * 1024.0 + P * (4.0 * m->dk8 * 1024.0 + 128.0 * 8.0); };
-        const fir_x8_entry& ran8 = find_x8(3, c.odd);
+        const bool tile256 = m->i8_tile != 0 && m->dk8 == 2 * kRing && pairs >= 2;
+        const fir_x8_entry& ran8 = tile256 ? kX8Tile256 : find_x8(3, c.odd);
         int nl = 0, pf = 1, rc8 = FIR_OK;
         for (int p0 = 0; p0 < pairs; ++nl) {
-            const int P = launch_pairs_(pairs - p0, kShareMax);
+            const int P = launch_pairs_(pairs - p0, tile256 ? 2 * kShareMax : kShareMax);
             if (p0 == 0) pf = P;
             const size_t qo = (size_t)p0;
+            const bool tile = tile256 && P >= 2;
             if ((rc8 = fir_gallery_profile_begin_(m->g, c.st))) return rc8;
-            hipLaunchKernelGGL(ran8.fn, dim3(c.grid, 1), dim3(kGemmBlock), kHalfLds, c.st, m->g8, m->i8_gnorm, m->qbf[b] + qo * 4 * m->dk8 * 64, m->qinv[b] + qo * 2 * kQT,
+            hipLaunchKernelGGL(tile ? pick_x8_tile256(m->dbg_skip) : pick_x8(3, c.odd, m->dbg_skip), dim3(c.grid, 1), dim3(kGemmBlock), kHalfLds, c.st, m->g8, m->i8_gnorm, m->qbf[b] + qo * 4 * m->dk8 * 64, m->qinv[b] + qo * 2 * kQT,
                                n, (int64_t)0, n, m->dk8, m->awin[b] + qo * 2 * kQT, m->lists[b] + qo * 2 * kQT * kListCap, m->counts[b] + qo * 2 * kQT,
-                               m->qnorm[b] + qo * 2 * kQT, m->sample_rows, P, (P <= 1 ? 1 : 0) | m->adapt_dbg, 1, m->aT[b] + qo * 2 * kQT, 0);
+                               m->qnorm[b] + qo * 2 * kQT, m->sample_rows, tile ? P / 2 : P, (P <= 1 ? 1 : 0) | m->adapt_dbg, 1, m->aT[b] + qo * 2 * kQT, 0);
             if ((rc8 = fir_gallery_profile_end_(m->g, c.st, bytes8(P)))) return rc8;
             p0 += P;
         }
@@ -1858,6 +1895,7 @@
 extern "C" {
 
 void fir_gemm_set_int8_(fir_gemm* m, int32_t mode) { if (m) m->i8_mode = mode > 0 ? 1 : mode < 0 ? -1 : 0; }
+void fir_gemm_set_int8_tile_(fir_gemm* m, int32_t mode) { if (m) m->i8_tile = mode > 0 ? 1 : mode < 0 ? -1 : 0; }
 
 int fir_gemm_search_top1_keys_dev(fir_gemm* m, const float* d_queries, int32_t qb, uint64_t* d_keys, void* stream) {
     return gemm_search(m, d_queries, qb, 1, d_keys, stream);
diff --git a/fast-image-recognition_amd/csrc/fir_gemm_f16x.h b/fast-image-recognition_amd/csrc/fir_gemm_f16x.h
--- a/fast-image-recognition_amd/csrc/fir_gemm_f16x.h
+++ b/fast-image-recognition_amd/csrc/fir_gemm_f16x.h
@@ -70,7 +70,7 @@
 }
 
 constexpr int kXStage = 16;
-template <int MODE, int STREAMED, int ODD, int DBG = 0, int NJB = 8, int I8 = 0>
+template <int MODE, int STREAMED, int ODD, int DBG = 0, int NJB = 8, int I8 = 0, int QH = 1>
 __global__ void __launch_bounds__(kGemmBlock, 1) k_gemm_proxy_f16x(const uint4* __restrict__ gh, const float* __restrict__ gnorm, const uint4* qh,
                                                                     const float* __restrict__ qinv, int64_t n, int64_t row_begin, int64_t row_end,
                                                                     int dk16, const float* tau, unsigned long long* lists, int* counts,
@@ -79,7 +79,11 @@
     extern __shared__ __attribute__((aligned(16))) uint4 lqx[];
     if (MODE == 1 && smin != nullptr && (int)smin[0] - sub_stride <= 0) return;
     const int nt = nt_flags & 1;
-    __shared__ float tau_s[2 * kQT], qinv_s[2 * kQT];
+    static_assert(QH == 1 || (QH == 2 && MODE == 3 && !STREAMED && !ODD && NJB == 8 && I8 && !(DBG & (8 | 16 | 64 | 128 | 256 | 512))), "QH = 2: the int8 top-1 pass of two units only");
+    constexpr int kTQ = 2 * kQT * QH;
+    constexpr int kStage = QH == 2 ? kXStage / 2 : kXStage;
+    constexpr int kHalfImg = 4 * kRing * 2 * 64;
+    __shared__ float tau_s[kTQ], qinv_s[kTQ];
     constexpr bool kAdapt = MODE == 3 || MODE == 4;
     constexpr bool kSlots = MODE == 4;
     const int kth = kSlots ? sub_stride : 1;
@@ -97,11 +101,11 @@
         return res;
     };
     constexpr bool kAppend = MODE == 1 || kAdapt;
-    __shared__ unsigned long long skeys[kAppend ? 2 * kQT * kXStage : 1];
-    __shared__ int scnt[kAppend ? 2 * kQT : 1];
-    __shared__ float qn_s[kAdapt ? 2 * kQT : 1], win_s[kAdapt ? 2 * kQT : 1];
+    __shared__ unsigned long long skeys[kAppend ? kTQ * kStage : 1];
+    __shared__ int scnt[kAppend ? kTQ : 1];
+    __shared__ float qn_s[kAdapt ? kTQ : 1], win_s[kAdapt ? kTQ : 1];
     __shared__ __attribute__((aligned(16))) unsigned int slot_s[kSlots ? 2 * kQT * 8 : 8];
-    __shared__ float tq_s[kAdapt ? 2 * kQT : 1];
+    __shared__ float tq_s[kAdapt ? kTQ : 1];
     constexpr bool kDynForm = !STREAMED && kAdapt && !(DBG & 128);
     if (kDynForm && share <= 0) share = 1;
     __shared__ int next_blk;
@@ -123,7 +127,7 @@
     }
     const int dk32 = dk16 >> 1;
     {
-        const size_t pr = (size_t)pair_of_wg;
+        const size_t pr = (size_t)pair_of_wg * QH;
         qh += pr * 8 * dk32 * 64;
         qinv += pr * 2 * kQT;
         tau += pr * 2 * kQT;
@@ -137,7 +141,7 @@
     const int64_t rbs = MODE == 2 ? rb_stride : 1;
     const int lane = threadIdx.x & 63, wave = __builtin_amdgcn_readfirstlane(threadIdx.x >> 6);
     const int wpb = blockDim.x >> 6;
-    if (threadIdx.x < 2 * kQT) {
+    if (threadIdx.x < kTQ) {
         if (kSlots) {
             unsigned int v8[8];
 #pragma unroll
@@ -198,6 +202,12 @@
             const int jb = i / (dk32 * 64), r = i - jb * dk32 * 64;
             lqx[(size_t)((r >> 6) * 8 + jb) * 64 + (r & 63)] = qh[(size_t)jb * dk32 * 64 + r];
         }
+        if (QH == 2) {
+            for (int i = threadIdx.x; i < NJB * dk32 * 64; i += blockDim.x) {
+                const int jb = i / (dk32 * 64), r = i - jb * dk32 * 64;
+                lqx[kHalfImg + (size_t)((r >> 6) * 8 + jb) * 64 + (r & 63)] = qh[(size_t)(8 + jb) * dk32 * 64 + r];
+            }
+        }
         __syncthreads();
     }
     float smallest[NJB];
@@ -256,7 +266,7 @@
     };
     auto exchange_T = [&]() {
         __syncthreads();
-        if (threadIdx.x < 2 * kQT) {
+        if (threadIdx.x < kTQ) {
             if (kSlots) {
                 unsigned int mine[8], old[8];
 #pragma unroll
@@ -268,7 +278,9 @@
                 tau_s[threadIdx.x] = __uint_as_float(kth_of_slots(&slot_s[threadIdx.x * 8]));
             } else {
             const unsigned int mine = __float_as_uint(tau_s[threadIdx.x]);
-            const unsigned int old = (nt_flags & 8) ? mine : atomicMin(&smin[threadIdx.x], mine);
+            unsigned int zx = 0;
+            if (QH == 2) asm volatile("v_mov_b32 %0, 0" : "=v"(zx));
+            const unsigned int old = (nt_flags & 8) ? mine : atomicMin(&smin[threadIdx.x + zx], mine);
             tau_s[threadIdx.x] = __uint_as_float(old < mine ? old : mine);
             }
             tq_s[threadIdx.x] = tau_s[threadIdx.x] - qn_s[threadIdx.x];
@@ -284,13 +296,13 @@
         warm = false;
         rg_next = rg + rg_step;
         int tk = 0;
-        if (kDynForm && lane == 0) tk = (int)atomicInc((unsigned int*)&next_blk, 0xFFFFFFFFu);
+        if (kDynForm && lane == 0 && !(QH == 2 && warm_it)) tk = (int)atomicInc((unsigned int*)&next_blk, 0xFFFFFFFFu);
         const int64_t rbp = FIR_X_RBP(rg);
         const int64_t rb = rbp * rbs;
         const bool active = rbp < rb_end;
         const uint4* a_nxt = a_cur;
         auto next_block = [&]() {
-            if (kDynForm) rg_next = blk0 + __builtin_amdgcn_readfirstlane(tk);
+            if (kDynForm) rg_next = (QH == 2 && warm_it) ? rg : blk0 + __builtin_amdgcn_readfirstlane(tk);
             const int64_t rgn = rg_next;
             a_nxt = FIR_X_BLOCK(rgn < rg_end ? rgn : rg);
         };
@@ -299,10 +311,10 @@
         if (kAdapt) {
             if (!warm_it && wave < NJB && !(nt_flags & 4)) {
                 const int v = blk_no >> __builtin_ctz((unsigned)blk_no | 0x40000000u);
-                if ((v == 1 || v == 3) && lane < 16) {
+                if ((v == 1 || v == 3) && lane < 16 * QH) {
                     int zl;
                     asm volatile("v_mbcnt_lo_u32_b32 %0, -1, 0\n\tv_mbcnt_hi_u32_b32 %0, -1, %0" : "=v"(zl));
-                    const int ql = 16 * wave + zl;
+                    const int ql = QH == 2 ? 128 * (zl >> 4) + 16 * wave + (zl & 15) : 16 * wave + zl;
                     if (kSlots) {
                         unsigned int mine[8], old[8];
 #pragma unroll
@@ -327,8 +339,8 @@
         const float* gn_blk = n >= 32 ? gnorm + (rb * 32 < ((n - 32) & ~(int64_t)3) ? rb * 32 : ((n - 32) & ~(int64_t)3)) : (const float*)gh;
         const bool full_block = active && rbp * 32 >= row_begin && rbp * 32 + 32 <= row_end && rb * 32 + 32 <= n && (MODE != 0 || rb * 32 + 32 <= sample_rows);
         unsigned int* smin_blk = MODE == 2 ? smin + (size_t)(wave & 7) * sub_stride : nullptr;
-        auto check_jb = [&](int jb, int64_t rbq, const float4 g0, const float4 g1, float gminq) {
-            const int q = jb * 16 + (lane & 15);
+        auto check_jb = [&](int jb, int64_t rbq, const float4 g0, const float4 g1, float gminq, int half = 0) {
+            const int q = half * 2 * kQT + jb * 16 + (lane & 15);
             const float m2 = kDefer ? m2r[jb] : 2.0f * qinv_s[q];
             const float tq = kDefer ? tqr[jb] : kAdapt ? tq_s[q] : tau_s[q];
             float amax;
@@ -356,15 +368,15 @@
             if (mn < tq) {
                 int lz;
                 asm volatile("v_mbcnt_lo_u32_b32 %0, -1, 0\n\tv_mbcnt_hi_u32_b32 %0, -1, %0" : "=v"(lz));
-                const int qr = jb * 16 + (lz & 15);
+                const int qr = half * 2 * kQT + jb * 16 + (lz & 15);
 #pragma unroll
                 for (int i = 0; i < 8; ++i) {
                     if (pv[i] < tq) {
                         const int64_t row = rbq * 32 + 16 * (i >> 2) + 4 * (lz >> 4) + (i & 3);
                         const unsigned long long key = fir::key_pack(pv[i], (uint32_t)row);
                         const int st = atomicAdd(&scnt[qr], 1);
-                        if (st < kXStage) {
-                            skeys[qr * kXStage + st] = key;
+                        if (st < kStage) {
+                            skeys[qr * kStage + st] = key;
                         } else {
                             const int slot = atomicAdd(&counts[qr], 1);
                             if (slot < kListCap) lists[(size_t)qr * kListCap + slot] = key;
@@ -375,19 +387,72 @@
                 if (kAdapt) lower_T(qr, pv, mn);
             }
         };
-        auto unit = [&](uint4 (&C)[RING], uint4 (&N)[RING], int h, auto first_tag, auto last_tag) {
+        auto observe_half = [&](int half) __attribute__((always_inline)) {
+            int lw;
+            asm volatile("v_mbcnt_lo_u32_b32 %0, -1, 0\n\tv_mbcnt_hi_u32_b32 %0, -1, %0" : "=v"(lw));
+#pragma unroll
+            for (int jb = 0; jb < NJB; ++jb) {
+                const int q = half * 2 * kQT + jb * 16 + (lw & 15);
+                const float m2 = 2.0f * qinv_s[q];
+                const float gnv[8] = {gns[0].x, gns[0].y, gns[0].z, gns[0].w, gns[1].x, gns[1].y, gns[1].z, gns[1].w};
+                float mn = __builtin_huge_valf();
+#pragma unroll
+                for (int i = 0; i < 8; ++i) mn = fminf(mn, __builtin_fmaf(-m2, (float)acc[i >> 2][jb][i & 3], gnv[i]));
+                float o = __shfl_xor(mn, 16, 64);
+                mn = o < mn ? o : mn;
+                o = __shfl_xor(mn, 32, 64);
+                mn = o < mn ? o : mn;
+                const float tn = fmaxf((mn + qn_s[q]) + win_s[q], 0.f);
+                if (lw < 16 && tn < tau_s[q]) atomicMin((unsigned int*)&tau_s[q], __float_as_uint(tn));
+            }
+        };
+        auto straddle_half = [&](int half) __attribute__((always_inline)) {
+            int ls;
+            asm volatile("v_mbcnt_lo_u32_b32 %0, -1, 0\n\tv_mbcnt_hi_u32_b32 %0, -1, %0" : "=v"(ls));
+#pragma unroll
+            for (int jb = 0; jb < NJB; ++jb) {
+                const int q = half * 2 * kQT + jb * 16 + (ls & 15);
+                const float m2 = 2.0f * qinv_s[q];
+                const float tq = tq_s[q];
+#pragma unroll
+                for (int i = 0; i < 8; ++i) {
+                    const int64_t row = rb * 32 + 16 * (i >> 2) + 4 * (ls >> 4) + (i & 3);
+                    if (row >= n || row < row_begin || row >= row_end) continue;
+                    const float p = __builtin_fmaf(-m2, (float)acc[i >> 2][jb][i & 3], gnorm[row]);
+                    if (p < tq) {
+                        const int slot = atomicAdd(&counts[q], 1);
+                        if (slot < kListCap) lists[(size_t)q * kListCap + slot] = fir::key_pack(p, (uint32_t)row);
+                    }
+                }
+            }
+        };
+        auto unit = [&](uint4 (&C)[RING], uint4 (&N)[RING], int h, auto first_tag, auto last_tag, auto half_tag) {
             constexpr bool kFirst = decltype(first_tag)::value;
             constexpr bool kLast = decltype(last_tag)::value;
-            if (kLast && !kFirst && kDefer && kAdapt) {
+            constexpr int kHalf = decltype(half_tag)::value;
+            constexpr bool kBurst = QH == 1 || (kHalf == 0 ? kFirst : kLast);
+            constexpr bool kNorms = QH == 1 ? kLast : (kHalf == 0 && !kFirst);
+            if (QH == 1 && kLast && !kFirst && kDefer && kAdapt) {
 #pragma unroll
                 for (int jb = 0; jb < NJB; ++jb) tqr[jb] = tq_s[jb * 16 + (lane & 15)];
             }
             if (kLast && kNextLate) next_block();
             const uint4* src = kLast ? a_nxt : a_cur + (size_t)(h + 1) * RING * 64;
-            const uint4* bq = STREAMED ? lqx + lane + (size_t)(ring_c & 3) * 4 * RING * 64 : lqx + lane + (size_t)(h % kUnitsPerSlab) * RING * 4 * 64;
+            auto image_of_half = [&](int half) __attribute__((always_inline)) -> const uint4* {
+                uint32_t o = (uint32_t)(uintptr_t)(void __attribute__((address_space(3)))*)lqx + (uint32_t)(half * kHalfImg + lane) * 16u;
+                asm volatile("" : "+v"(o));
+#if defined(__HIP_DEVICE_COMPILE__)
+                return (const uint4*)(const uint4 __attribute__((address_space(3)))*)o;
+#else
+                return lqx + o;
+#endif
+            };
+            const uint4* bq = STREAMED ? lqx + lane + (size_t)(ring_c & 3) * 4 * RING * 64
+                              : QH == 2 ? image_of_half(kHalf) + (size_t)(h % kUnitsPerSlab) * RING * 4 * 64
+                                       : lqx + lane + (size_t)(h % kUnitsPerSlab) * RING * 4 * 64;
             unsigned long long t_burst0 = 0;
             if (DBG & 256) t_burst0 = __builtin_amdgcn_s_memtime();
-            if (!(DBG & 16) && !(DBG & 2) && !(DBG & 64)) {
+            if (kBurst && !(DBG & 16) && !(DBG & 2) && !(DBG & 64)) {
                 if (nt) {
 #pragma unroll
                     for (int u = 0; u < RING; ++u) N[u] = ld_nt(src + (size_t)u * 64 + lane);
@@ -410,7 +475,7 @@
                 }
                 ++dbg_units;
             }
-            if (kLast) {
+            if (kNorms) {
                 unsigned int zl;
                 asm volatile("v_mov_b32 %0, 0" : "=v"(zl));
                 const float* gb = gn_blk;
@@ -420,6 +485,7 @@
             }
             __builtin_amdgcn_sched_barrier(0);
             const uint4* bq_after = STREAMED ? lqx + lane + (size_t)((ring_c + 1) & 3) * 4 * RING * 64
+                                    : QH == 2 ? (kFirst ? image_of_half(kHalf) + (size_t)RING * 4 * 64 : image_of_half(kHalf ^ 1))
                                              : lqx + lane + (size_t)((kLast ? 0 : h + 1) % kUnitsPerSlab) * RING * 4 * 64;
 #pragma unroll
             for (int t = 0; t < RING / 2; ++t) {
@@ -428,7 +494,7 @@
 #pragma unroll
                 for (int j = 0; j < NJB; ++j) {
                     if (kDefer && kFirst && t == 0) {
-                        check_jb(j, p_rb, pg[0], pg[1], p_gmin);
+                        check_jb(j, p_rb, pg[0], pg[1], p_gmin, QH == 2 ? kHalf ^ 1 : 0);
                     }
                     const f16x8 b = as_f16x8(B[j]);
                     const acc_t zero = {0, 0, 0, 0};
@@ -468,24 +534,59 @@
         };
         const std::true_type yes;
         const std::false_type no;
+        const std::integral_constant<int, 0> h0;
+        const std::integral_constant<int, 1> h1;
+        float gmin_blk = 0.f;
+        if (QH == 2) {
+            auto bounds_of_half = [&](int half) __attribute__((always_inline)) {
+                if (!kDefer) return;
+#pragma unroll
+                for (int jb = 0; jb < NJB; ++jb) {
+                    tqr[jb] = tq_s[half * 2 * kQT + jb * 16 + (lane & 15)];
+                    m2r[jb] = 2.0f * qinv_s[half * 2 * kQT + jb * 16 + (lane & 15)];
+                }
+            };
+            unit(cur, nxt, 0, yes, no, h0);
+            bounds_of_half(0);
+            unit(nxt, cur, 1, no, no, h0);
+            gmin_blk = fminf(fminf(fminf(gns[0].x, gns[0].y), fminf(gns[0].z, gns[0].w)), fminf(fminf(gns[1].x, gns[1].y), fminf(gns[1].z, gns[1].w)));
+            p_rb = rb;
+            pg[0] = gns[0];
+            pg[1] = gns[1];
+            p_gmin = (full_block && !warm_it) ? gmin_blk : __builtin_huge_valf();
+            if (DBG & 1) {
+#pragma unroll
+                for (int jb = 0; jb < NJB; ++jb) asm volatile("" ::"v"(acc[0][jb]), "v"(acc[1][jb]));
+                if (DBG & 4) {
+#pragma unroll
+                    for (int jb = 0; jb < NJB; ++jb) asm volatile("" : "+v"(B[jb].x));
+                }
+            } else {
+                if (__builtin_expect(warm_it, 0)) { if (full_block) observe_half(0); }
+                else if (__builtin_expect(active && !full_block, 0)) straddle_half(0);
+            }
+            unit(cur, nxt, 0, yes, no, h1);
+            bounds_of_half(1);
+            unit(nxt, cur, 1, no, yes, h1);
+        } else
         if (!ODD) {
-            unit(cur, nxt, 0, yes, no);
+            unit(cur, nxt, 0, yes, no, h0);
             for (int h = 1; h + 1 < units; h += 2) {
-                unit(nxt, cur, h, no, no);
-                unit(cur, nxt, h + 1, no, no);
-            }
-            unit(nxt, cur, units - 1, no, yes);
+                unit(nxt, cur, h, no, no, h0);
+                unit(cur, nxt, h + 1, no, no, h0);
+            }
+            unit(nxt, cur, units - 1, no, yes, h0);
         } else {
             if (ODD == 2) {
-                unit(cur, nxt, 0, yes, yes);
+                unit(cur, nxt, 0, yes, yes, h0);
             } else {
-                unit(cur, nxt, 0, yes, no);
+                unit(cur, nxt, 0, yes, no, h0);
                 for (int h = 1; h + 2 < units; h += 2) {
-                    unit(nxt, cur, h, no, no);
-                    unit(cur, nxt, h + 1, no, no);
-                }
-                unit(nxt, cur, units - 2, no, no);
-                unit(cur, nxt, units - 1, no, yes);
+                    unit(nxt, cur, h, no, no, h0);
+                    unit(cur, nxt, h + 1, no, no, h0);
+                }
+                unit(nxt, cur, units - 2, no, no, h0);
+                unit(cur, nxt, units - 1, no, yes, h0);
             }
 #pragma unroll
             for (int u = 0; u < RING; ++u) cur[u] = nxt[u];
@@ -503,7 +604,7 @@
                 asm volatile("v_mbcnt_lo_u32_b32 %0, -1, 0\n\tv_mbcnt_hi_u32_b32 %0, -1, %0" : "=v"(lw));
 #pragma unroll
                 for (int jb = 0; jb < NJB; ++jb) {
-                    const int q = jb * 16 + (lw & 15);
+                    const int q = (QH - 1) * 2 * kQT + jb * 16 + (lw & 15);
                     const float m2 = 2.0f * qinv_s[q];
                     float pv[8];
                     float mn = __builtin_huge_valf();
@@ -533,6 +634,7 @@
                 }
             }
             exchange_T();
+            if (QH == 2) continue;
             if (kDefer) {
 #pragma unroll
                 for (int jb = 0; jb < NJB; ++jb) tqr[jb] = tq_s[jb * 16 + (lane & 15)];
@@ -542,7 +644,7 @@
         }
         if (!active) continue;
         if (full_block) {
-            const float gmin = fminf(fminf(fminf(gns[0].x, gns[0].y), fminf(gns[0].z, gns[0].w)), fminf(fminf(gns[1].x, gns[1].y), fminf(gns[1].z, gns[1].w)));
+            const float gmin = QH == 2 ? gmin_blk : fminf(fminf(fminf(gns[0].x, gns[0].y), fminf(gns[0].z, gns[0].w)), fminf(fminf(gns[1].x, gns[1].y), fminf(gns[1].z, gns[1].w)));
             if (kAppend) {
                 if (kDefer) {
                     pend = true;
@@ -597,7 +699,7 @@
         asm volatile("v_mbcnt_lo_u32_b32 %0, -1, 0\n\tv_mbcnt_hi_u32_b32 %0, -1, %0" : "=v"(ls));
 #pragma unroll
         for (int jb = 0; jb < NJB; ++jb) {
-            const int q = jb * 16 + (ls & 15);
+            const int q = (QH - 1) * 2 * kQT + jb * 16 + (ls & 15);
             const float m2 = 2.0f * qinv_s[q];
             const float tq = kAdapt ? tq_s[q] : tau_s[q];
             float mn = __builtin_huge_valf();
@@ -638,7 +740,7 @@
         int lt;
         asm volatile("v_mbcnt_lo_u32_b32 %0, -1, 0\n\tv_mbcnt_hi_u32_b32 %0, -1, %0" : "=v"(lt));
         auto last_jb = [&](int jb) {
-            const int q = jb * 16 + (lt & 15);
+            const int q = (QH - 1) * 2 * kQT + jb * 16 + (lt & 15);
             const float m2 = 2.0f * qinv_s[q];
             const float tq = kAdapt ? tq_s[q] : tau_s[q];
             const float gnv[8] = {pg[0].x, pg[0].y, pg[0].z, pg[0].w, pg[1].x, pg[1].y, pg[1].z, pg[1].w};
@@ -656,8 +758,8 @@
                         const int64_t row = p_rb * 32 + 16 * (i >> 2) + 4 * (lt >> 4) + (i & 3);
                         const unsigned long long key = fir::key_pack(pv[i], (uint32_t)row);
                         const int st = atomicAdd(&scnt[q], 1);
-                        if (st < kXStage) {
-                            skeys[q * kXStage + st] = key;
+                        if (st < kStage) {
+                            skeys[q * kStage + st] = key;
                         } else {
                             const int slot = atomicAdd(&counts[q], 1);
                             if (slot < kListCap) lists[(size_t)q * kListCap + slot] = key;
@@ -672,13 +774,13 @@
     }
     if (kAppend) {
         __syncthreads();
-        if (threadIdx.x < 2 * kQT) {
+        if (threadIdx.x < kTQ) {
             const int q = threadIdx.x;
-            const int cnt = scnt[q] < kXStage ? scnt[q] : kXStage;
+            const int cnt = scnt[q] < kStage ? scnt[q] : kStage;
             if (cnt > 0) {
                 const int base = atomicAdd(&counts[q], cnt);
                 for (int st = 0; st < cnt; ++st)
-                    if (base + st < kListCap) lists[(size_t)q * kListCap + base + st] = skeys[q * kXStage + st];
+                    if (base + st < kListCap) lists[(size_t)q * kListCap + base + st] = skeys[q * kStage + st];
             }
         }
     }
diff --git a/fast-image-recognition_amd/csrc/fir_internal.h b/fast-image-recognition_amd/csrc/fir_internal.h
--- a/fast-image-recognition_amd/csrc/fir_internal.h
+++ b/fast-image-recognition_amd/csrc/fir_internal.h
@@ -117,6 +117,7 @@
 extern "C" int fir_gemm_nominations_(fir_gemm* m, int32_t which, int32_t q0, int32_t nq, int32_t max_entries, int32_t* counts, float* tau, float* qnorm,
                                      uint64_t* lists, float* proxies, float* gmax, int32_t* qmap, int32_t* live);
 extern "C" void fir_gemm_set_int8_(fir_gemm* m, int32_t mode);
+extern "C" void fir_gemm_set_int8_tile_(fir_gemm* m, int32_t mode);
 extern "C" void fir_gemm_memory_bytes_(const fir_gemm* m, int64_t* fragments, int64_t* rowmajor, int64_t* scratch);
 
 struct fir_cls;
```

Result: faster. 2.711 million queries/s (median of 6 runs) (+8.9%).
